# iow-esm/components.flux_calculator

Measured on AMD Instinct MI355X. Metric: exchange-grid Mcells/s per coupling step; achieved HBM GB/s vs MI355X peak, higher is better.
Workload: dtype f64

## Files before the change

### components.flux_calculator_amd/csrc/fcx_engine.hip

```cpp
#include <hip/hip_runtime.h>

#include <algorithm>
#include <atomic>
#include <cctype>
#include <chrono>
#include <condition_variable>
#include <cstdarg>
#include <cstdio>
#include <cstdlib>
#include <cstring>
#include <deque>
#include <map>
#include <memory>
#include <mutex>
#include <set>
#include <string>
#include <thread>
#include <vector>

#include <sched.h>
#include <unistd.h>

#include "fcx_copy_pool.h"
#include "fcx_internal.h"
// ... 108 lines not shown
    return std::max(1, std::min(cpus, 16));
  }();
  return n;
}

}

struct FieldUploader {
  std::thread th;
  std::mutex mu;
  std::condition_variable cv, idle;
  std::deque<int> q;
  int busy = 0;
  bool stop = false;
  bool prepared = false;
  bool dma = false;
  int err = 0;
  std::string msg;
};

struct fcx_engine {
  int device = 0;
  int T = 0;
  int64_t n[3] = {0, 0, 0};
  hipStream_t stream = nullptr;
  bool own_stream = false;
  int8_t method[FCX_NUM_FLUXES][kMaxTypes] = {};
  int slot[kMaxTypes + 1][3][kNumVars];
  bool allocated[kMaxTypes + 1][3][kNumVars] = {};
  uint8_t put_to[kMaxTypes + 1][3][kNumVars] = {};
  std::vector<Buffer> bufs;
  std::map<const double *, int> by_ptr;
  bool committed = false;
  bool any_regrid = false;
  bool aligned16 = true;
  bool f32 = false;
  size_t esize = 8;
  bool lcorr = false;
  int32_t init_date = 0;
  std::vector<double> corr_mm;
  void *corr_dev = nullptr;
  Csr rg[4];
  std::vector<std::pair<int, std::pair<int, int>>> averages;
  std::map<std::pair<uint32_t, int>, Plan> plans;
  void *pool = nullptr;
  hipEvent_t ev0 = nullptr, ev1 = nullptr;
  bool timed = false;
  bool gpu_ready = false;
  bool user_stream = false;
  LaunchConfig launch;
  bool specialize = true;
  struct AtmosField {
    int phase, s, g, var;
    double *out_host = nullptr, *out_dev = nullptr;
    bool external = false;
    StageRef st;
  };
  int64_t n_atmos = -1;
  std::vector<int32_t> atm_row, atm_col;
  std::vector<double> atm_w;
  bool atm_contiguous = true;
  int32_t *d_atm_row = nullptr, *d_atm_col = nullptr, *d_atm_idx = nullptr;
  void *d_atm_seg = nullptr;
  int32_t *d_atm_tile_a0 = nullptr;
  int64_t atm_seg_words = 0, atm_segments = 0;
  std::vector<int32_t> atm_idx;
  std::vector<int32_t> atm_empty;
  int32_t *d_atm_empty = nullptr;
  int32_t atm_maxseg = 0;
  double *d_atm_xrec = nullptr;
  int64_t atm_crossings = 0;
  bool atm_halo = true;
  double *d_atm_w = nullptr;
  std::vector<AtmosField> atm_fields;
  double *atm_shared = nullptr;
  int32_t atm_nb = 0, atm_stride = 0, atm_left = -1, atm_right = -1;
  bool own_shared = false;
  double *atm_shared_own = nullptr;
  struct fcx_comm *comm = nullptr;
  bool atm_done = false;
  bool exchanged = false;
  void *atm_pool = nullptr;
  int64_t atm_out_tpad = 0;
  bool atmos_in_run = true;
  bool atm_done_fused = false;
  int group_members = 0;
  std::unique_ptr<FieldUploader> uploader;
  std::vector<char> field_sent;
  struct RemapField {
    int phase, s, g, var;
    double *out_host = nullptr, *out_dev = nullptr;
    bool external = false;
    StageRef st;
  };
  struct Remap {
    int64_t n_dst = 0, n_links = 0;
    int32_t max_src = -1;
    std::vector<int32_t> row, col;
    std::vector<double> w;
    int32_t *d_row = nullptr, *d_col = nullptr;
    double *d_w = nullptr;
    std::vector<RemapField> fields;
    void *pool = nullptr;
    size_t pool_bytes = 0;
    double scatter = 0.0;
  };
  std::vector<Remap> remaps;
  int remap_pack = 2;
  void *d_rec = nullptr;
  size_t rec_bytes = 0;
  const Plan *rec_plan = nullptr;
  bool rec_written = false;
  int chunks = 8;
  int64_t min_chunk = 256 * 1024;
  int zero_copy = 2;
  bool zc_active = false;
  int64_t zc_bytes = 0;
  bool timing = false;
  hipStream_t s_in = nullptr, s_out = nullptr;
  std::vector<hipEvent_t> ev_in, ev_comp, ev_out;
  bool staging = true;
  bool deferred_scatter = false;
#ifdef FCX_AB_BUILD
  bool ab_fixup_each = false;
  bool ab_no_head = false;
#endif
  int host_threads = 0;
  std::vector<StagePool> spools;
  std::vector<Xfer> pending_out;
  hipEvent_t ev_stage_in = nullptr;
  bool stage_in_live = false;
  size_t pool_bytes = 0, tiled_bytes = 0, atm_pool_bytes = 0;
  bool tiled_opt = true;
  int64_t tpad = 0;
  std::vector<void *> tiled_pools;
  bool plan_dry = false;
  bool lib_spans = true;
  std::vector<Span> spans;
  std::vector<char> written;

  fcx_engine() {
    for (auto &a : slot)
      for (auto &b : a)
        for (auto &c : b) c = -1;
  }
  int buf(int s, int g, int var) const { return slot[s][g - 1][var0(var)]; }
  double *dptr(int s, int g, int var) const {
    int b = buf(s, g, var);
    return b < 0 ? nullptr : bufs[b].dev;
  }
};

static void stage_free(fcx_engine *e);


extern "C" const char *fcx_last_error(void) { return g_err.c_str(); }
extern "C" int fcx_version(void) { return FCX_VERSION; }

static std::atomic<fcx_abort_handler> g_abort{nullptr};

extern "C" int fcx_set_abort_handler(fcx_abort_handler handler) {
  g_abort.store(handler);
  return FCX_OK;
}

extern "C" int fcx_abort(const char *message) {
  fcx_abort_handler h = g_abort.load();
  if (!h) return fail(FCX_E_STATE, "no abort handler registered");
  h(message ? message : "");
  return FCX_OK;
}

extern "C" int fcx_method_from_string(const char *s, size_t len) {
  if (!s) return -1;
  size_t e = len;
  while (e > 0 && (s[e - 1] == ' ' || s[e - 1] == '\0')) --e;
  std::string m(s, e);
  static const char *names[] = {"none", "zero", "copy", "CCLM", "MOM5", "RCO", "water", "ice", "StBo"};
  for (int i = 0; i < 9; ++i)
    if (m == names[i]) return i;
  return -1;
}

static int64_t days_from_civil(int64_t y, int m, int d) {
  y -= m <= 2;
  const int64_t era = (y >= 0 ? y : y - 399) / 400;
  const int64_t yoe = y - era * 400;
  const int64_t doy = (153 * (m + (m > 2 ? -3 : 9)) + 2) / 5 + d - 1;
  const int64_t doe = yoe * 365 + yoe / 4 - yoe / 100 + doy;
  return era * 146097 + doe - 719468;
}

extern "C" int fcx_current_month(int32_t init_date, int64_t seconds, int32_t *month) {
  if (!month) return fail(FCX_E_ARG, "month is NULL");
  const int64_t y = init_date / 10000;
  const int m = (init_date / 100) % 100, d = init_date % 100;
  if (y < 1 || m < 1 || m > 12 || d < 1 || d > 31)
    return fail(FCX_E_ARG, "init_date %d is not YYYYMMDD", (int)init_date);
  int64_t q = seconds / 86400;
  if (seconds % 86400 != 0 && seconds < 0) q -= 1;
  const int64_t z = days_from_civil(y, m, d) + q + 719468;
  const int64_t era = (z >= 0 ? z : z - 146096) / 146097;
  const int64_t doe = z - era * 146097;
  const int64_t yoe = (doe - doe / 1460 + doe / 36524 - doe / 146096) / 365;
  const int64_t doy = doe - (365 * yoe + yoe / 4 - yoe / 100);
  const int64_t mp = (5 * doy + 2) / 153;
  *month = (int32_t)(mp < 10 ? mp + 3 : mp - 9);
  return FCX_OK;
}


extern "C" int fcx_create(int device, int num_surface_types, const int32_t grid_size[3],
                          fcx_engine **out) {
  if (!out || !grid_size) return fail(FCX_E_ARG, "NULL argument");
  *out = nullptr;
  if (num_surface_types < 1 || num_surface_types > kMaxTypes)
    return fail(FCX_E_ARG, "num_surface_types=%d outside 1..%d", num_surface_types, kMaxTypes);
  for (int g = 0; g < 3; ++g)
    if (grid_size[g] < 0) return fail(FCX_E_ARG, "grid_size(%d)=%d < 0", g + 1, grid_size[g]);
  auto *e = new fcx_engine();
  e->device = device;
  e->T = num_surface_types;
  for (int g = 0; g < 3; ++g) e->n[g] = grid_size[g];
  *out = e;
  return FCX_OK;
}

static void uploader_stop(fcx_engine *e);
static int uploader_join(fcx_engine *e);

extern "C" int fcx_destroy(fcx_engine *e) {
  if (!e) return FCX_OK;
  uploader_stop(e);
  if (!e->gpu_ready) {
    delete e;
    return FCX_OK;
  }
  (void)hipSetDevice(e->device);
  if (e->stream) (void)hipStreamSynchronize(e->stream);
  for (auto &kv : e->plans) {
    (void)hipFree(kv.second.dev);
    (void)hipFree(kv.second.host.rec);
  }
  for (auto &r : e->rg) {
    (void)hipFree(r.d_row);
    (void)hipFree(r.d_col);
    (void)hipFree(r.d_w);
  }
  (void)hipFree(e->corr_dev);
  (void)hipFree(e->d_atm_row);
  (void)hipFree(e->d_atm_seg);
  (void)hipFree(e->d_atm_tile_a0);
  (void)hipFree(e->d_atm_idx);
  (void)hipFree(e->d_atm_empty);
  (void)hipFree(e->d_atm_xrec);
  (void)hipFree(e->d_atm_col);
  (void)hipFree(e->d_atm_w);
  (void)hipFree(e->atm_pool);
  (void)hipFree(e->atm_shared_own);
  for (auto &r : e->remaps) {
    (void)hipFree(r.d_row);
    (void)hipFree(r.d_col);
    (void)hipFree(r.d_w);
    (void)hipFree(r.pool);
  }
  (void)hipFree(e->d_rec);
  (void)hipFree(e->pool);
  for (void *p : e->tiled_pools) (void)hipFree(p);
  for (auto &sp : e->spans) (void)hipFree(sp.dev);
  if (e->ev0) (void)hipEventDestroy(e->ev0);
  if (e->ev1) (void)hipEventDestroy(e->ev1);
  for (hipEvent_t ev : e->ev_in) (void)hipEventDestroy(ev);
  for (hipEvent_t ev : e->ev_comp) (void)hipEventDestroy(ev);
  for (hipEvent_t ev : e->ev_out) (void)hipEventDestroy(ev);
  stage_free(e);
  if (e->s_in) (void)hipStreamDestroy(e->s_in);
  if (e->s_out) (void)hipStreamDestroy(e->s_out);
  if (e->own_stream && e->stream) (void)hipStreamDestroy(e->stream);
  delete e;
  return FCX_OK;
}

extern "C" int fcx_set_stream(fcx_engine *e, void *stream) {
  if (!e) return fail(FCX_E_ARG, "NULL engine");
  if (e->committed)
    if (int r = uploader_join(e)) return r;
  if (e->own_stream && e->stream) {
    (void)hipStreamSynchronize(e->stream);
    (void)hipStreamDestroy(e->stream);
  }
  e->stream = reinterpret_cast<hipStream_t>(stream);
  e->own_stream = false;
  e->user_stream = true;
  return FCX_OK;
}

static int gpu_init(fcx_engine *e) {
  if (e->gpu_ready) return FCX_OK;
  HIP_TRY(hipSetDevice(e->device));
  if (!e->user_stream) {
    HIP_TRY(hipStreamCreateWithFlags(&e->stream, hipStreamNonBlocking));
    e->own_stream = true;
  }
  HIP_TRY(hipEventCreate(&e->ev0));
  HIP_TRY(hipEventCreate(&e->ev1));
  e->gpu_ready = true;
  return FCX_OK;
}

extern "C" int fcx_set_method(fcx_engine *e, int flux, int s, int method) {
  if (!e) return fail(FCX_E_ARG, "NULL engine");
  if (e->committed) return fail(FCX_E_STATE, "engine already committed");
  if (flux < 0 || flux >= FCX_NUM_FLUXES) return fail(FCX_E_ARG, "flux %d unknown", flux);
  if (s < 1 || s > e->T) return fail(FCX_E_ARG, "surface_type %d outside 1..%d", s, e->T);
  if (method < FCX_NONE || method > FCX_STBO) return fail(FCX_E_ARG, "method %d unknown", method);
  e->method[flux][s - 1] = (int8_t)method;
  return FCX_OK;
}

extern "C" int fcx_bind_field(fcx_engine *e, int s, int g, int var, double *ptr, int64_t n,
                              int flags) {
  if (!e) return fail(FCX_E_ARG, "NULL engine");
  if (e->committed) return fail(FCX_E_STATE, "engine already committed");
  if (s < 0 || s > kMaxTypes || g < 1 || g > 3 || var < 1 || var > kNumVars)
    return fail(FCX_E_ARG, "slot (%d,%d,%d) out of range", s, g, var);
  if (!ptr) {
    e->slot[s][g - 1][var0(var)] = -1;
    return FCX_OK;
  }
  if (n < e->n[g - 1])
    return fail(FCX_E_ARG, "%s(%d,%s): array of %lld cells shorter than grid_size %lld",
                kVarNames[var0(var)], s, g == 1 ? "t" : g == 2 ? "u" : "v", (long long)n,
                (long long)e->n[g - 1]);
  const bool on_dev = flags & FCX_MEM_DEVICE;
  auto it = e->by_ptr.find(ptr);
  int b;
  if (it == e->by_ptr.end()) {
    Buffer bf;
    bf.n = n;
    if (on_dev) {
      bf.dev = ptr;
// ... 172 lines not shown
}


static bool is_compute(int m) { return m == FCX_ZERO || m == FCX_CCLM || m == FCX_MOM5 || m == FCX_RCO; }

static bool merge_ok(const fcx_engine *e) {
  if (e->n[0] != e->n[1] || e->n[0] != e->n[2]) return false;
  for (int s = 1; s <= e->T; ++s) {
    if (e->method[FCX_SPEC_VAPOR_SURFACE_U][s - 1] != e->method[FCX_SPEC_VAPOR_SURFACE_T][s - 1] ||
        e->method[FCX_SPEC_VAPOR_SURFACE_V][s - 1] != e->method[FCX_SPEC_VAPOR_SURFACE_T][s - 1])
      return false;
    for (int v : {FCX_TSUR, FCX_FICE, FCX_PSUR, FCX_UATM, FCX_VATM, FCX_QSUR})
      for (int g = 2; g <= 3; ++g)
        if (e->buf(s, g, v) >= 0 && e->buf(s, g, v) != e->buf(s, 1, v)) return false;
    for (int v : {FCX_AMOM, FCX_CMOM})
      if (e->buf(s, 3, v) != e->buf(s, 2, v)) return false;
  }
  return true;
}

static void plan_fused_atmos(fcx_engine *e, Plan &pl, uint32_t stages, int phase) {
  pl.atm_fused = false;
  const bool maps = (!compact_map(e->f32, true) || e->d_atm_seg) && (!compact_map(e->f32, false) || e->d_atm_seg) &&
                    (compact_map(e->f32, true) || e->d_atm_idx) && (compact_map(e->f32, false) || e->d_atm_idx);
  if (!pl.variant || !maps || e->atm_maxseg > kTile / 2 || e->any_regrid || phase <= 0 ||
      phase >= 1000 || !e->specialize || (e->f32 && e->T >= 2))
    return;
  const TypeParams &tp = pl.host.type[0];
  AtmosFused af{};
  int nf = 0;
  const bool multi = e->T >= 2;
  if (multi && !pl.host.ravg_on) return;
  for (size_t fi = 0; fi < e->atm_fields.size(); ++fi) {
    const auto &f = e->atm_fields[fi];
    if (!(f.phase & phase)) continue;
    const int b = e->buf(f.s, f.g, f.var);
    int k = -1;
    if (multi) {
      for (int slot = 0; slot < kFusedFields; ++slot)
        if (f.s == 0 && pl.host.ravg.out[slot] && b >= 0 && e->bufs[b].dev == pl.host.ravg.out[slot]) k = slot;
      if (k < 0 || af.out[k]) return;
      af.out[k] = f.out_dev;
      af.x[k] = e->bufs[b].dev;
      af.scol[k] = (int32_t)fi;
      ++nf;
      continue;
    }
    if (f.s == 1 && f.var == FCX_MEVA && (stages & S_MEVA) && b == e->buf(1, 1, FCX_MEVA)) k = 0;
    if (f.s == 1 && f.var == FCX_HLAT && (stages & S_HLAT) && b == e->buf(1, 1, FCX_HLAT) &&
        (tp.m_hlat == FCX_WATER || tp.m_hlat == FCX_ICE || tp.m_hlat == FCX_ZERO))
      k = 1;
    if (f.s == 1 && f.var == FCX_HSEN && (stages & S_HSEN) && b == e->buf(1, 1, FCX_HSEN)) k = 2;
    if (f.s == 1 && f.var == FCX_RBBR && (stages & S_RBBR) && b == e->buf(1, 1, FCX_RBBR) &&
        (tp.m_rbbr == FCX_STBO || tp.m_rbbr == FCX_ZERO))
      k = 3;
    if (f.s == 1 && f.var == FCX_UMOM && (stages & S_UMOM) && b == e->buf(1, 2, FCX_UMOM)) k = 4;
    if (f.s == 1 && f.var == FCX_VMOM && (stages & S_VMOM) && b == e->buf(1, 3, FCX_VMOM)) k = 5;
    if (k < 0 || af.out[k]) return;
    af.out[k] = f.out_dev;
    af.x[k] = e->bufs[b].dev;
    af.scol[k] = (int32_t)fi;
    ++nf;
  }
  if (nf == 0) return;
  if (e->d_atm_seg) {
    af.seg_bits = reinterpret_cast<const uint32_t *>(e->d_atm_seg);
    af.seg_pre = reinterpret_cast<const int32_t *>(af.seg_bits + e->atm_seg_words);
    af.seg_atm = af.seg_pre + e->atm_seg_words + 1;
  }
  af.tile_a0 = e->d_atm_tile_a0;
  af.idx = e->d_atm_idx;
  af.w = e->d_atm_w;
  af.xrec = e->d_atm_xrec;
  af.xrec_on = e->atm_crossings > 0;
#ifdef FCX_AB_BUILD
  if (e->ab_no_head) af.xrec_on = 0;
#endif
  af.n_atmos = e->n_atmos;
  af.shared = e->atm_shared;
  af.stride = e->atm_stride;
  af.left = e->atm_left;
  af.right = e->atm_right;
  af.tpad = e->tpad;
  af.out_tpad = e->atm_out_tpad;
  pl.af = af;
  pl.atm_nf = nf;
  pl.atm_phase = phase;
  pl.atm_fused = true;
}

static bool remap_packs(const fcx_engine *e, const fcx_engine::Remap &rm, int nf);
static int rec_width(const fcx_engine *e, int nf);

static int plan_fused_records(fcx_engine *e, Plan &pl, uint32_t stages, int phase) {
  pl.rec_remap = pl.rec_group = -1;
  Params &P = pl.host;
  for (int k = 0; k < 6; ++k) P.rec_pos[k] = -1;
#ifndef FCX_FUSE_RECORDS
#define FCX_FUSE_RECORDS 1
#endif
  if (!FCX_FUSE_RECORDS || !pl.variant || e->T != 1 || e->f32 || !e->specialize || e->any_regrid || phase <= 0 || phase >= 1000 ||
      e->remap_pack == 0 || e->launch.cells_per_thread != 2 || !e->aligned16 || !P.merged_uv || P.n_max <= 0)
    return FCX_OK;
  const TypeParams &tp = P.type[0];
  auto slot_of = [&](const fcx_engine::RemapField &f) -> int {
    const int b = e->buf(f.s, f.g, f.var);
    if (f.s != 1 || b < 0) return -1;
    if (f.var == FCX_MEVA && (stages & S_MEVA) && b == e->buf(1, 1, FCX_MEVA) && is_compute(tp.m_meva)) return 0;
    if (f.var == FCX_HLAT && (stages & S_HLAT) && b == e->buf(1, 1, FCX_HLAT) && tp.t.hlat &&
        (tp.m_hlat == FCX_WATER || tp.m_hlat == FCX_ICE || tp.m_hlat == FCX_ZERO))
      return 1;
    if (f.var == FCX_HSEN && (stages & S_HSEN) && b == e->buf(1, 1, FCX_HSEN) && tp.t.hsen && is_compute(tp.m_hsen))
      return 2;
    if (f.var == FCX_RBBR && (stages & S_RBBR) && b == e->buf(1, 1, FCX_RBBR) && tp.t.rbbr &&
        (tp.m_rbbr == FCX_STBO || tp.m_rbbr == FCX_ZERO))
      return 3;
    if (f.var == FCX_UMOM && (stages & S_UMOM) && b == e->buf(1, 2, FCX_UMOM) && tp.uv[0].mom && is_compute(tp.m_mom))
      return 4;
    if (f.var == FCX_VMOM && (stages & S_VMOM) && b == e->buf(1, 3, FCX_VMOM) && tp.uv[1].mom && is_compute(tp.m_mom))
      return 5;
    return -1;
  };
  for (size_t ri = 0; ri < e->remaps.size(); ++ri) {
    const auto &rm = e->remaps[ri];
    std::vector<const fcx_engine::RemapField *> grp;
    int gi = 0;
    auto try_group = [&]() -> bool {
      const int nf = (int)grp.size();
      if (!remap_packs(e, rm, nf) || nf > 6) return false;
      int8_t pos[6] = {-1, -1, -1, -1, -1, -1};
      for (int i = 0; i < nf; ++i) {
        const int k = slot_of(*grp[(size_t)i]);
        if (k < 0 || pos[k] >= 0) return false;
        pos[k] = (int8_t)i;
      }
      const int p = rec_width(e, nf);
      HIP_TRY(hipMalloc(&P.rec, (size_t)P.n_max * p * sizeof(double)));
      P.rec_p = p;
      for (int k = 0; k < 6; ++k) P.rec_pos[k] = pos[k];
      pl.rec_remap = (int)ri;
      pl.rec_group = gi;
      return true;
    };
    for (auto &f : rm.fields) {
      if (!(f.phase & phase)) continue;
      grp.push_back(&f);
      if ((int)grp.size() == kMaxAtmosFields) {
        if (try_group()) return FCX_OK;
        grp.clear();
        ++gi;
      }
    }
    if (!grp.empty() && try_group()) return FCX_OK;
  }
  return FCX_OK;
}

static int ravg_slot(const fcx_engine *e, const Params &P, uint32_t stages, int g, int var) {
  if (e->T < 2) return -1;
  int slot = -1;
  if (g == 1 && var == FCX_MEVA) slot = A_MEVA;
  if (g == 1 && var == FCX_HLAT) slot = A_HLAT;
  if (g == 1 && var == FCX_HSEN) slot = A_HSEN;
  if (g == 1 && var == FCX_RBBR) slot = A_RBBR;
  if (g == 1 && var == FCX_TSUR) slot = A_TSUR;
  if (P.merged_uv && g == 2 && var == FCX_UMOM) slot = A_UMOM;
  if (P.merged_uv && g == 3 && var == FCX_VMOM) slot = A_VMOM;
// ... 710 lines not shown
      at[b] = {cold_pool, fill[kCold]++};
    }
  }
  for (int k = 0; k < npools; ++k) {
    void *p = nullptr;
    hipError_t err = hipMalloc(&p, bytes);
    if (err != hipSuccess)
      return fail(FCX_E_NOMEM, "hipMalloc(%zu) for the tiled field mirrors: %s", bytes, hipGetErrorString(err));
    e->tiled_pools.push_back(p);
  }
  for (size_t b = 0; b < e->bufs.size(); ++b)
    e->bufs[b].dev = reinterpret_cast<double *>((char *)e->tiled_pools[at[b].first] +
                                                (size_t)at[b].second * kLayoutTile * e->esize);
  e->tpad = (S - 1) * kLayoutTile;
  return FCX_OK;
}

constexpr hipMemcpyKind kH2D = hipMemcpyDefault, kD2H = hipMemcpyDefault;

static hipError_t copy_cells(const fcx_engine *e, const Buffer &bf, int64_t a, int64_t z, bool h2d,
                             hipStream_t s) {
  const size_t es = e->esize;
  auto one = [&](int64_t lo, int64_t hi) {
    if (hi <= lo) return hipSuccess;
    char *dev = reinterpret_cast<char *>(bf.dev) + (size_t)tiled(lo, e->tpad) * es;
    char *host = reinterpret_cast<char *>(bf.host) + (size_t)lo * es;
    const size_t bytes = (size_t)(hi - lo) * es;
    return h2d ? hipMemcpyAsync(dev, host, bytes, kH2D, s) : hipMemcpyAsync(host, dev, bytes, kD2H, s);
  };
  if (z <= a) return hipSuccess;
  if (e->tpad == 0) return one(a, z);
  const int64_t t0 = (a + kLayoutTile - 1) / kLayoutTile, t1 = z / kLayoutTile;
  if (t1 <= t0) {
    const int64_t m = std::min(z, t0 * kLayoutTile);
    hipError_t r = one(a, m);
    return (r != hipSuccess || m >= z) ? r : one(m, z);
  }
  if (a < t0 * kLayoutTile)
    if (hipError_t r = one(a, t0 * kLayoutTile)) return r;
  const size_t row = (size_t)kLayoutTile * es, pitch = (size_t)(kLayoutTile + e->tpad) * es;
  char *dev = reinterpret_cast<char *>(bf.dev) + (size_t)t0 * pitch;
  char *host = reinterpret_cast<char *>(bf.host) + (size_t)t0 * row;
  hipError_t r = h2d ? hipMemcpy2DAsync(dev, pitch, host, row, row, (size_t)(t1 - t0), kH2D, s)
                     : hipMemcpy2DAsync(host, row, dev, pitch, row, (size_t)(t1 - t0), kD2H, s);
  if (r != hipSuccess || z == t1 * kLayoutTile) return r;
  return one(t1 * kLayoutTile, z);
}

static hipError_t zero_cells(const fcx_engine *e, double *dev, int64_t n, hipStream_t s) {
  if (n <= 0) return hipSuccess;
  if (e->tpad == 0) return hipMemsetAsync(dev, 0, (size_t)n * e->esize, s);
  const size_t row = (size_t)kLayoutTile * e->esize, pitch = (size_t)(kLayoutTile + e->tpad) * e->esize;
  const int64_t full = n / kLayoutTile;
  if (full)
    if (hipError_t r = hipMemset2DAsync(dev, pitch, 0, row, (size_t)full, s)) return r;
  if (n > full * kLayoutTile)
    return hipMemsetAsync(reinterpret_cast<char *>(dev) + full * pitch, 0, (size_t)(n - full * kLayoutTile) * e->esize, s);
  return hipSuccess;
}


static StageRef stage_ref(fcx_engine *e, const void *d) {
  StageRef r;
  const char *p = reinterpret_cast<const char *>(d);
  for (size_t i = 0; i < e->spools.size(); ++i) {
    const StagePool &q = e->spools[i];
    if (p >= q.dev && p < q.dev + q.bytes) {
      r.sp = (int)i;
      r.soff = (size_t)(p - q.dev);
      return r;
    }
  }
  return r;
}

static void stage_setup(fcx_engine *e) {
  if (!e->staging) return;
  const size_t es = e->esize;
  std::vector<StagePool> cand;
  for (void *p : e->tiled_pools)
    cand.push_back(StagePool{(char *)p, nullptr, e->tiled_bytes, true, (size_t)kLayoutTile * es,
                             (size_t)(kLayoutTile + e->tpad) * es});
  if (e->pool) cand.push_back(StagePool{(char *)e->pool, nullptr, e->pool_bytes, false, 0, 0});
  if (e->atm_pool) {
    const bool t = e->atm_out_tpad != 0;
    cand.push_back(StagePool{(char *)e->atm_pool, nullptr, e->atm_pool_bytes, t, t ? (size_t)kLayoutTile * es : 0,
                             t ? (size_t)(kLayoutTile + e->atm_out_tpad) * es : 0});
  }
  for (auto &rm : e->remaps)
    if (rm.pool) cand.push_back(StagePool{(char *)rm.pool, nullptr, rm.pool_bytes, false, 0, 0});
  auto heap = [&](const void *host, int64_t n) { return host && !lib_block_device_ptr(host, (size_t)std::max<int64_t>(n, 1) * es); };
  std::vector<char> used(cand.size(), 0);
  auto mark = [&](const void *dev) {
    for (size_t i = 0; i < cand.size(); ++i)
      if ((const char *)dev >= cand[i].dev && (const char *)dev < cand[i].dev + cand[i].bytes) used[i] = 1;
  };
  for (auto &bf : e->bufs)
    if (!bf.external && heap(bf.host, bf.n)) mark(bf.dev);
  for (auto &f : e->atm_fields)
    if (!f.external && heap(f.out_host, e->n_atmos)) mark(f.out_dev);
  for (auto &rm : e->remaps)
    for (auto &f : rm.fields)
      if (!f.external && heap(f.out_host, rm.n_dst)) mark(f.out_dev);
  for (size_t i = 0; i < cand.size(); ++i)
    if (used[i]) e->spools.push_back(cand[i]);
  for (auto &bf : e->bufs)
    if (!bf.external && heap(bf.host, bf.n)) bf.st = stage_ref(e, bf.dev);
  for (auto &f : e->atm_fields)
    if (!f.external && heap(f.out_host, e->n_atmos)) f.st = stage_ref(e, f.out_dev);
  for (auto &rm : e->remaps)
    for (auto &f : rm.fields)
      if (!f.external && heap(f.out_host, rm.n_dst)) f.st = stage_ref(e, f.out_dev);
}

static void stage_disable(fcx_engine *e, size_t i) {
  StagePool &p = e->spools[i];
  p.host = nullptr;
  p.disabled = true;
  auto drop = [&](StageRef &st) {
    if (st.sp == (int)i) st.sp = -1;
  };
  for (auto &bf : e->bufs) drop(bf.st);
  for (auto &f : e->atm_fields) drop(f.st);
  for (auto &rm : e->remaps)
    for (auto &f : rm.fields) drop(f.st);
}

static int pin_fail_mode() {
  const char *v = std::getenv("FCX_TEST_PIN_FAIL");
  return v && (*v == '1' || *v == '2') ? *v - '0' : 0;
}

static bool stage_pin(fcx_engine *e, size_t i, bool lazy) {
  StagePool &p = e->spools[i];
  if (p.host) return true;
  if (p.disabled) return false;
  const int inject = pin_fail_mode();
  if (!(inject == 1 || (inject == 2 && lazy)) &&
      hipHostMalloc((void **)&p.host, std::max<size_t>(p.bytes, 1), kHostPinFlags) == hipSuccess)
    return true;
  (void)hipGetLastError();
  stage_disable(e, i);
  return false;
}

static void stage_alloc_all(fcx_engine *e, const std::vector<char> &eager) {
  const bool fail_all = pin_fail_mode() == 1;
  for (size_t i = 0; i < e->spools.size(); ++i) {
    if (e->spools[i].host) continue;
    if (i < eager.size() && !eager[i] && !fail_all) continue;
    (void)stage_pin(e, i, false);
  }
}

static void stage_prepare_bufs(fcx_engine *e, const std::vector<int> &ids) {
  for (int b : ids) {
    const int sp = e->bufs[(size_t)b].st.sp;
    if (sp >= 0) (void)stage_pin(e, (size_t)sp, true);
  }
}
static void stage_prepare_outputs(fcx_engine *e) {
  for (auto &f : e->atm_fields)
    if (f.st.sp >= 0) (void)stage_pin(e, (size_t)f.st.sp, true);
  for (auto &rm : e->remaps)
    for (auto &f : rm.fields)
      if (f.st.sp >= 0) (void)stage_pin(e, (size_t)f.st.sp, true);
}

static int stage_alloc(fcx_engine *e, const std::vector<Xfer> &xs) {
  for (const Xfer &x : xs) {
    StagePool &p = e->spools[(size_t)x.sp];
    if (!p.host) return fail(FCX_E_STATE, "staging pool %d has no host image", x.sp);
  }
  return FCX_OK;
}

static void stage_free(fcx_engine *e) {
  for (auto &p : e->spools)
    if (p.host) (void)hipHostFree(p.host);
  e->spools.clear();
  if (e->ev_stage_in) (void)hipEventDestroy(e->ev_stage_in);
  e->ev_stage_in = nullptr;
}

static void stage_copy(fcx_engine *e, const std::vector<Xfer> &xs, int64_t a, int64_t z, bool gather) {
  constexpr size_t kPiece = size_t(64) << 10;
  const size_t es = e->esize;
  std::vector<CopyJob> jobs;
  auto add = [&](char *img, char *host, size_t bytes) {
    for (size_t o = 0; o < bytes; o += kPiece) {
      const size_t b = std::min(kPiece, bytes - o);
      jobs.push_back(gather ? CopyJob{img + o, host + o, b} : CopyJob{host + o, img + o, b});
// ... 265 lines not shown
  for (auto &c : e->rg) {
    if (!c.set) continue;
    HIP_TRY(hipMalloc(&c.d_row, c.row_ptr.size() * sizeof(int32_t)));
    HIP_TRY(hipMalloc(&c.d_col, std::max<size_t>(c.col.size(), 1) * sizeof(int32_t)));
    HIP_TRY(hipMalloc(&c.d_w, std::max<size_t>(c.w.size(), 1) * sizeof(double)));
    HIP_TRY(hipMemcpy(c.d_row, c.row_ptr.data(), c.row_ptr.size() * sizeof(int32_t), hipMemcpyHostToDevice));
    if (!c.col.empty()) {
      HIP_TRY(hipMemcpy(c.d_col, c.col.data(), c.col.size() * sizeof(int32_t), hipMemcpyHostToDevice));
      if (e->f32) {
        std::vector<float> wf(c.w.begin(), c.w.end());
        HIP_TRY(hipMemcpy(c.d_w, wf.data(), wf.size() * sizeof(float), hipMemcpyHostToDevice));
      } else {
        HIP_TRY(hipMemcpy(c.d_w, c.w.data(), c.w.size() * sizeof(double), hipMemcpyHostToDevice));
      }
    }
  }
  if (e->n_atmos >= 0) {
    HIP_TRY(hipMalloc(&e->d_atm_row, e->atm_row.size() * sizeof(int32_t)));
    HIP_TRY(hipMemcpy(e->d_atm_row, e->atm_row.data(), e->atm_row.size() * sizeof(int32_t),
                      hipMemcpyHostToDevice));
    HIP_TRY(hipMalloc(&e->d_atm_w, std::max<size_t>(e->atm_w.size(), 1) * sizeof(double)));
    if (!e->atm_w.empty())
      HIP_TRY(hipMemcpy(e->d_atm_w, e->atm_w.data(), e->atm_w.size() * sizeof(double), hipMemcpyHostToDevice));
    if (e->atm_contiguous && !e->atm_idx.empty() && !(compact_map(e->f32, true) && compact_map(e->f32, false))) {
      HIP_TRY(hipMalloc(&e->d_atm_idx, e->atm_idx.size() * sizeof(int32_t)));
      HIP_TRY(hipMemcpy(e->d_atm_idx, e->atm_idx.data(), e->atm_idx.size() * sizeof(int32_t),
                        hipMemcpyHostToDevice));
    }
    if (e->atm_contiguous && !e->atm_idx.empty() && (compact_map(e->f32, true) || compact_map(e->f32, false))) {
      const int64_t nx = (int64_t)e->atm_idx.size(), nw = (nx + 31) / 32;
      std::vector<uint32_t> seg((size_t)(2 * nw + 1), 0u);
      std::vector<int32_t> atm;
      for (int64_t x = 0; x < nx; ++x)
        if (x == 0 || e->atm_idx[(size_t)x] != e->atm_idx[(size_t)x - 1]) {
          seg[(size_t)(x >> 5)] |= 1u << (x & 31);
          atm.push_back(e->atm_idx[(size_t)x]);
        }
      int32_t run = 0;
      for (int64_t w = 0; w <= nw; ++w) {
        seg[(size_t)(nw + w)] = (uint32_t)run;
        if (w < nw) run += __builtin_popcount(seg[(size_t)w]);
      }
      e->atm_seg_words = nw;
      e->atm_segments = (int64_t)atm.size();
      const size_t head = seg.size() * sizeof(uint32_t);
      HIP_TRY(hipMalloc(&e->d_atm_seg, head + std::max<size_t>(atm.size(), 1) * sizeof(int32_t)));
      HIP_TRY(hipMemcpy(e->d_atm_seg, seg.data(), head, hipMemcpyHostToDevice));
      if (!atm.empty())
        HIP_TRY(hipMemcpy((char *)e->d_atm_seg + head, atm.data(), atm.size() * sizeof(int32_t), hipMemcpyHostToDevice));
      if (compact_map(e->f32, false)) {
        const int64_t tc = (int64_t)(e->f32 ? kF32Cpl : 2) * 64, nt = (nx + tc - 1) / tc;
        std::vector<int32_t> a0((size_t)nt);
        for (int64_t t = 0; t < nt; ++t) a0[(size_t)t] = e->atm_idx[(size_t)(t * tc)];
        HIP_TRY(hipMalloc(&e->d_atm_tile_a0, (size_t)std::max<int64_t>(nt, 1) * sizeof(int32_t)));
        if (nt) HIP_TRY(hipMemcpy(e->d_atm_tile_a0, a0.data(), a0.size() * sizeof(int32_t), hipMemcpyHostToDevice));
      }
    }
    if (e->atm_contiguous && !e->atm_idx.empty()) {
      const int64_t tiles = (e->n[0] + kTile - 1) / kTile;
      HIP_TRY(hipMalloc(&e->d_atm_xrec, (size_t)std::max<int64_t>(tiles, 1) * kXRec * sizeof(double)));
      e->atm_crossings = 0;
      for (size_t b = kTile; b < e->atm_idx.size(); b += kTile) e->atm_crossings += e->atm_idx[b - 1] == e->atm_idx[b];
      if (!e->atm_empty.empty()) {
        HIP_TRY(hipMalloc(&e->d_atm_empty, e->atm_empty.size() * sizeof(int32_t)));
        HIP_TRY(hipMemcpy(e->d_atm_empty, e->atm_empty.data(), e->atm_empty.size() * sizeof(int32_t),
                          hipMemcpyHostToDevice));
      }
    }
    if (!e->atm_contiguous) {
      HIP_TRY(hipMalloc(&e->d_atm_col, std::max<size_t>(e->atm_col.size(), 1) * sizeof(int32_t)));
      if (!e->atm_col.empty())
        HIP_TRY(hipMemcpy(e->d_atm_col, e->atm_col.data(), e->atm_col.size() * sizeof(int32_t),
                          hipMemcpyHostToDevice));
    }
    size_t need = 0;
    bool atm_ext = false;
    for (auto &f : e->atm_fields) {
      atm_ext = atm_ext || f.external;
      if (!f.external) need += ((size_t)std::max<int64_t>(e->n_atmos, 1) * e->esize + 255) / 256 * 256;
    }
    const int64_t nfa = (int64_t)e->atm_fields.size();
    if (FCX_TILED_ATM && e->tpad && !atm_ext && nfa >= 2 && e->n_atmos > 0) {
      const int64_t tiles = (e->n_atmos + kLayoutTile - 1) / kLayoutTile;
      e->atm_pool_bytes = (size_t)tiles * nfa * kLayoutTile * e->esize;
      HIP_TRY(hipMalloc(&e->atm_pool, e->atm_pool_bytes));
      for (int64_t k = 0; k < nfa; ++k)
        e->atm_fields[k].out_dev = reinterpret_cast<double *>((char *)e->atm_pool + (size_t)k * kLayoutTile * e->esize);
      e->atm_out_tpad = (nfa - 1) * kLayoutTile;
      need = 0;
    }
    if (need) {
      e->atm_pool_bytes = need;
      HIP_TRY(hipMalloc(&e->atm_pool, need));
      size_t off = 0;
      for (auto &f : e->atm_fields)
        if (!f.external) {
          f.out_dev = reinterpret_cast<double *>((char *)e->atm_pool + off);
          off += ((size_t)std::max<int64_t>(e->n_atmos, 1) * e->esize + 255) / 256 * 256;
        }
    }
  }
  if (e->own_shared && e->n_atmos >= 0) {
    const size_t stride = std::max<size_t>(e->atm_fields.size(), 1);
    const size_t cnt = std::max<size_t>((size_t)e->atm_nb * stride, 1);
    HIP_TRY(hipMalloc(&e->atm_shared_own, cnt * sizeof(double)));
    HIP_TRY(hipMemset(e->atm_shared_own, 0, cnt * sizeof(double)));
    if (e->atm_left >= 0 && e->atm_right >= 0 && e->n_atmos < 2 && e->atm_left != e->atm_right)
      return fail(FCX_E_ARG, "the one atmosphere cell is shared on both sides: it needs one boundary slot for all "
                             "its ranks (left == right), not %d and %d", e->atm_left, e->atm_right);
    e->atm_shared = e->atm_nb > 0 ? e->atm_shared_own : nullptr;
    e->atm_stride = (int32_t)stride;
  }
  for (auto &rm : e->remaps) {
    for (auto &f : rm.fields)
      if (rm.max_src >= e->n[f.g - 1])
        return fail(FCX_E_ARG, "remap link source %d outside the %lld cells of grid %d", rm.max_src,
                    (long long)e->n[f.g - 1], f.g);
    HIP_TRY(hipMalloc(&rm.d_row, rm.row.size() * sizeof(int32_t)));
    HIP_TRY(hipMemcpy(rm.d_row, rm.row.data(), rm.row.size() * sizeof(int32_t), hipMemcpyHostToDevice));
    HIP_TRY(hipMalloc(&rm.d_col, std::max<size_t>(rm.col.size(), 1) * sizeof(int32_t)));
    HIP_TRY(hipMalloc(&rm.d_w, std::max<size_t>(rm.w.size(), 1) * sizeof(double)));
    if (!rm.col.empty()) {
      HIP_TRY(hipMemcpy(rm.d_col, rm.col.data(), rm.col.size() * sizeof(int32_t), hipMemcpyHostToDevice));
      HIP_TRY(hipMemcpy(rm.d_w, rm.w.data(), rm.w.size() * sizeof(double), hipMemcpyHostToDevice));
    }
    const size_t one = ((size_t)std::max<int64_t>(rm.n_dst, 1) * e->esize + 255) / 256 * 256;
    size_t need = 0;
    for (auto &f : rm.fields) need += f.external ? 0 : one;
    if (need) {
      rm.pool_bytes = need;
      HIP_TRY(hipMalloc(&rm.pool, need));
      size_t off = 0;
      for (auto &f : rm.fields)
        if (!f.external) {
          f.out_dev = reinterpret_cast<double *>((char *)rm.pool + off);
          off += one;
        }
    }
    size_t nf_max = 0;
    for (int ph = 1; ph <= 3; ++ph) {
      size_t c = 0;
      for (auto &f : rm.fields) c += (f.phase & ph) ? 1 : 0;
      nf_max = std::max(nf_max, std::min<size_t>(c, kMaxAtmosFields));
    }
    rm.scatter = remap_scatter(rm);
    if (remap_packs(e, rm, (int)nf_max))
      e->rec_bytes = std::max(e->rec_bytes, (size_t)(rm.max_src + 1) * rec_width(e, (int)nf_max) * e->esize);
  }
  if (e->rec_bytes) HIP_TRY(hipMalloc(&e->d_rec, e->rec_bytes));
  stage_setup(e);
  e->committed = true;
  std::vector<char> eager(e->spools.size(), e->any_regrid ? 1 : 0);
  if (!e->any_regrid) {
    Plan *pl = nullptr;
    if (get_plan(e, phase_stages(FCX_PHASE_ALL), FCX_PHASE_ALL, &pl) == FCX_OK && pl) {
      for (const std::vector<int> *ids : {&pl->reads, &pl->writes})
        for (int b : *ids)
          if (e->bufs[(size_t)b].st.sp >= 0) eager[(size_t)e->bufs[(size_t)b].st.sp] = 1;
    } else {
      std::fill(eager.begin(), eager.end(), 1);
    }
    for (auto &f : e->atm_fields)
      if (f.st.sp >= 0) eager[(size_t)f.st.sp] = 1;
    for (auto &rm : e->remaps)
      for (auto &f : rm.fields)
        if (f.st.sp >= 0) eager[(size_t)f.st.sp] = 1;
  }
  stage_alloc_all(e, eager);
  return FCX_OK;
}


// ... 40 lines not shown
    direct = true;
  }
  if (!spanned.empty()) {
    if (int r = span_copy(e, spanned, h2d, e->stream)) return r;
    direct = true;
  }
  if (h2d) return stage_in(e, xs, e->stream);
  if (xs.empty() && direct && !e->deferred_scatter) {
    HIP_TRY(hipStreamSynchronize(e->stream));
    return stage_flush(e);
  }
  return stage_out(e, xs, e->stream);
}

#ifndef FCX_ZC_ONE_CELL
#define FCX_ZC_ONE_CELL 1
#endif

static int full_range_halo(const fcx_engine *e, const Plan *pl) {
  const int cpl = e->f32 ? kF32Cpl : 2;
  const int h = (e->atm_maxseg - 1 + cpl - 1) / cpl;
  if (e->atm_halo && e->atm_crossings > 0 &&
      (pl->host.num_types == 1 || (FCX_HALO_RAVG && pl->host.ravg_on)) && h >= 1 && h <= (cpl == 4 ? 2 : 4))
    return h;
  return 0;
}

static LaunchConfig plan_launch(fcx_engine *e, Plan *pl, int64_t lo, int64_t hi, bool *fused) {
  LaunchConfig lc = e->launch;
  lc.lo = lo;
  lc.hi = hi;
  if (e->zc_active) lc.nontemporal = false;
  if (!e->aligned16) lc.cells_per_thread = 1;
  if (FCX_ZC_ONE_CELL && e->zc_active && !pl->atm_fused && pl->host.rec == nullptr) lc.cells_per_thread = 1;
  lc.merged = pl->host.merged_uv != 0;
  lc.variant = (e->specialize && lc.merged) ? pl->variant : 0;
  lc.f32 = e->f32;
  lc.ravg = pl->host.ravg_on != 0;
  lc.rec = pl->host.rec != nullptr && lc.variant && lc.cells_per_thread == 2 && !lc.f32;
  *fused = pl->atm_fused && lc.variant && lc.cells_per_thread == 2;
  if (*fused) {
    pl->af.shared = e->atm_shared;
    pl->af.stride = e->atm_stride;
    pl->af.left = e->atm_left;
    pl->af.right = e->atm_right;
    lc.halo = lo == 0 && (hi < 0 || hi >= pl->host.n_max) ? full_range_halo(e, pl) : 0;
    pl->af.halo = lc.halo;
  }
  return lc;
}

static int launch_empty_cells(fcx_engine *e, Plan *pl, const LaunchConfig &lc) {
  if (e->atm_empty.empty()) return FCX_OK;
  const int r = launch_atmos_zero(pl->af, e->d_atm_empty, (int64_t)e->atm_empty.size(), lc.f32, e->stream);
  if (r) return fail(FCX_E_HIP, "atmos_zero launch: %s", hipGetErrorString((hipError_t)r));
  return FCX_OK;
}

static int launch_fixup(fcx_engine *e, Plan *pl, const LaunchConfig &lc) {
  if (int r = launch_empty_cells(e, pl, lc)) return r;
  if (e->atm_crossings <= 0 || lc.halo) return FCX_OK;
  const int r = launch_atmos_fixup(pl->af, pl->host.n_max, lc.f32, e->stream);
  if (r) return fail(FCX_E_HIP, "atmos_fixup launch: %s", hipGetErrorString((hipError_t)r));
  return FCX_OK;
}

static int launch_plan(fcx_engine *e, Plan *pl, const double *corr_m, int64_t lo = 0, int64_t hi = -1,
                       bool fixup = true) {
  if (pl->host.n_max <= 0) return FCX_OK;
  bool fused = false;
  const LaunchConfig lc = plan_launch(e, pl, lo, hi, &fused);
  e->rec_written = lc.rec;
  const int r = launch_cells(&pl->host, pl->dev, corr_m, lc, e->stream, fused ? &pl->af : nullptr);
  if (r) return fail(FCX_E_HIP, "cells_kernel launch: %s", hipGetErrorString((hipError_t)r));
  if (fused && fixup)
    if (int r2 = launch_fixup(e, pl, lc)) return r2;
  if (fused) e->atm_done_fused = true;
  return FCX_OK;
}

static int regrid_var(fcx_engine *e, int var, int surface_type);
static int comm_exchange(fcx_engine *e);
static hipError_t get_atm(const fcx_engine *e, double *host, const double *dev, hipStream_t s);
static int run_remaps(fcx_engine *e, int phase);
static int download_remaps(fcx_engine *e, int phase, hipStream_t s, std::vector<Xfer> *xs);

static int staged_sequence(int phase, std::vector<std::pair<uint32_t, int>> &seq) {
  if (phase & FCX_PHASE_EARLY) seq.push_back({S_RBBR, FCX_RBBR});
  if (phase & FCX_PHASE_NORMAL) {
    seq.push_back({S_QSUR_T | S_QSUR_U | S_QSUR_V, FCX_QSUR});
    seq.push_back({S_MEVA, FCX_MEVA});
    seq.push_back({S_HLAT, FCX_HLAT});
    seq.push_back({S_HSEN, FCX_HSEN});
    seq.push_back({S_UMOM, FCX_UMOM});
    seq.push_back({S_VMOM, FCX_VMOM});
    seq.push_back({S_RSDR, 0});
  }
  return FCX_OK;
}

static uint32_t phase_stages(int phase) {
  uint32_t st = S_AVG;
  if (phase & FCX_PHASE_EARLY) st |= kEarly;
  if (phase & FCX_PHASE_NORMAL) st |= kNormal;
  return st;
}


static int upload_one(fcx_engine *e, int b) {
  FieldUploader &u = *e->uploader;
  const Buffer &bf = e->bufs[(size_t)b];
  if (bf.n == 0) return FCX_OK;
  if (bf.st.sp >= 0) (void)stage_pin(e, (size_t)bf.st.sp, true);
  if (bf.st.sp >= 0) {
    if (!u.prepared) {
      bool mapped = false;
      for (const StagePool &p : e->spools) mapped = mapped || p.mapped;
      if (!e->pending_out.empty() || mapped) {
        HIP_TRY(hipStreamSynchronize(e->stream));
        if (int r = stage_flush(e)) return r;
      }
      if (e->stage_in_live) HIP_TRY(hipEventSynchronize(e->ev_stage_in));
      u.prepared = true;
    }
    const std::vector<Xfer> xs{xfer_of(bf.st, bf.host, bf.n)};
    if (int r = stage_alloc(e, xs)) return r;
    stage_copy(e, xs, 0, -1, true);
    if (!e->spools[(size_t)bf.st.sp].mapped) {
      HIP_TRY(stage_dma(e, xs, 0, -1, true, e->stream));
      u.dma = true;
    }
  } else if (!bf.external || bf.span >= 0) {
    HIP_TRY(copy_cells(e, bf, 0, bf.n, true, e->stream));
  }
  return FCX_OK;
}

static void uploader_loop(fcx_engine *e) {
  FieldUploader &u = *e->uploader;
  (void)hipSetDevice(e->device);
  std::unique_lock<std::mutex> lk(u.mu);
  for (;;) {
    u.cv.wait(lk, [&] { return u.stop || !u.q.empty(); });
    if (u.q.empty()) return;
    const int b = u.q.front();
    u.q.pop_front();
    u.busy = 1;
    lk.unlock();
    const int r = upload_one(e, b);
    lk.lock();
    if (r && !u.err) {
      u.err = r;
      u.msg = g_err;
    }
    u.busy = 0;
    if (u.q.empty()) u.idle.notify_all();
  }
}

static int uploader_join(fcx_engine *e) {
  if (!e->uploader) return FCX_OK;
  FieldUploader &u = *e->uploader;
  std::unique_lock<std::mutex> lk(u.mu);
  u.idle.wait(lk, [&] { return u.q.empty() && u.busy == 0; });
  if (u.dma) {
    u.dma = false;
    if (!e->ev_stage_in) HIP_TRY(hipEventCreateWithFlags(&e->ev_stage_in, hipEventDisableTiming));
    HIP_TRY(hipEventRecord(e->ev_stage_in, e->stream));
    e->stage_in_live = true;
  }
  if (u.err) {
    const int r = u.err;
    u.err = 0;
    std::fill(e->field_sent.begin(), e->field_sent.end(), 0);
    u.prepared = false;
    return fail(r, "fcx_upload_field: %s", u.msg.c_str());
  }
  return FCX_OK;
}

static void uploader_stop(fcx_engine *e) {
  if (!e->uploader) return;
  {
    std::lock_guard<std::mutex> lk(e->uploader->mu);
    e->uploader->stop = true;
  }
  e->uploader->cv.notify_all();
  if (e->uploader->th.joinable()) e->uploader->th.join();
  e->uploader.reset();
}

static void fields_taken(fcx_engine *e) {
  std::fill(e->field_sent.begin(), e->field_sent.end(), 0);
  if (e->uploader) e->uploader->prepared = false;
}

extern "C" int fcx_upload_field(fcx_engine *e, int s, int g, int var) {
  if (!e) return fail(FCX_E_ARG, "NULL engine");
  if (!e->committed) return fail(FCX_E_STATE, "fcx_commit has not been called");
  if (s < 0 || s > kMaxTypes || g < 1 || g > 3 || var < 1 || var > kNumVars)
    return fail(FCX_E_ARG, "field (%d, %d, %d) outside the data model", s, g, var);
  const int b = e->buf(s, g, var);
  if (b < 0) return fail(FCX_E_ARG, "local_field(%d,%d)%%var(%s) is not bound", s, g, kVarNames[var - 1]);
  if (e->field_sent.size() != e->bufs.size()) e->field_sent.assign(e->bufs.size(), 0);
  if (e->field_sent[(size_t)b]) return FCX_OK;
  e->field_sent[(size_t)b] = 1;
  if (!e->uploader) {
    e->uploader.reset(new FieldUploader());
    e->uploader->th = std::thread(uploader_loop, e);
  }
  {
    std::lock_guard<std::mutex> lk(e->uploader->mu);
    e->uploader->q.push_back(b);
  }
  e->uploader->cv.notify_one();
  return FCX_OK;
}

extern "C" int fcx_upload(fcx_engine *e, int phase) {
  if (int r = check(e)) return r;
  if (phase < 1 || phase > 3) return fail(FCX_E_ARG, "phase %d unknown", phase);
  Plan *pl;
  if (int r = get_plan(e, phase_stages(phase), phase, &pl)) return r;
  return copy_bufs(e, pl->reads, true);
}

extern "C" int fcx_download(fcx_engine *e, int phase) {
  if (int r = check(e)) return r;
  if (phase < 1 || phase > 3) return fail(FCX_E_ARG, "phase %d unknown", phase);
  Plan *pl;
  if (int r = get_plan(e, phase_stages(phase), phase, &pl)) return r;
  stage_prepare_outputs(e);
  std::vector<Xfer> xs;
  std::vector<int> ids = pl->writes;
  for (auto &f : e->atm_fields)
    if ((f.phase & phase) && e->n_atmos > 0) {
      if (f.st.sp >= 0)
        xs.push_back(xfer_of(f.st, f.out_host, e->n_atmos));
      else if (!f.external)
        HIP_TRY(get_atm(e, f.out_host, f.out_dev, e->stream));
    }
  if (int r = download_remaps(e, phase, e->stream, &xs)) return r;
  if (e->any_regrid) {
    std::vector<int> extra;
    std::vector<int> vars;
    if (phase & FCX_PHASE_EARLY) vars = {FCX_RBBR};
    if (phase & FCX_PHASE_NORMAL)
      for (int v : {FCX_QSUR, FCX_MEVA, FCX_HLAT, FCX_HSEN, FCX_UMOM, FCX_VMOM}) vars.push_back(v);
    for (int s = 1; s <= e->T; ++s)
      for (int g = 1; g <= 3; ++g)
        for (int v : vars)
          if (e->put_to[s][g - 1][v - 1])
            for (int k = 0; k < 3; ++k)
              if ((e->put_to[s][g - 1][v - 1] >> k) & 1)
                if (e->buf(s, k + 1, v) >= 0) extra.push_back(e->buf(s, k + 1, v));
    ids.insert(ids.end(), extra.begin(), extra.end());
  }
  std::sort(ids.begin(), ids.end());
  ids.erase(std::unique(ids.begin(), ids.end()), ids.end());
  return copy_bufs(e, ids, false, &xs);
}

static hipError_t get_atm(const fcx_engine *e, double *host, const double *dev, hipStream_t s) {
  const size_t es = e->esize, n = (size_t)e->n_atmos;
  if (!e->atm_out_tpad) return hipMemcpyAsync(host, dev, n * es, kD2H, s);
  const size_t row = (size_t)kLayoutTile * es, pitch = (size_t)(kLayoutTile + e->atm_out_tpad) * es;
  const size_t full = n / kLayoutTile;
  if (full)
    if (hipError_t r = hipMemcpy2DAsync(host, row, dev, pitch, row, full, kD2H, s)) return r;
  if (n > full * kLayoutTile)
    return hipMemcpyAsync((char *)host + full * row, (const char *)dev + full * pitch, (n - full * kLayoutTile) * es,
                          kD2H, s);
  return hipSuccess;
}

static AtmosArgs atmos_args(fcx_engine *e, int phase) {
  AtmosArgs a{};
  a.f32 = e->f32 ? 1 : 0;
  a.row_ptr = e->d_atm_row;
  a.col = e->atm_contiguous ? nullptr : e->d_atm_col;
  a.w = e->d_atm_w;
  a.n_atmos = e->n_atmos;
  a.stride = e->atm_stride;
  a.left = e->atm_left;
  a.right = e->atm_right;
  a.shared = e->atm_shared;
  a.tpad = e->tpad;
  a.out_tpad = e->atm_out_tpad;
  a.vec = a.col == nullptr && e->aligned16;
  for (size_t i = 0; i < e->atm_fields.size(); ++i) {
    const auto &f = e->atm_fields[i];
    if (!(f.phase & phase) || a.nf >= kMaxAtmosFields) continue;
    a.x[a.nf] = e->dptr(f.s, f.g, f.var);
    a.out[a.nf] = f.out_dev;
    a.scol[a.nf] = (int32_t)i;
    ++a.nf;
  }
  return a;
}

static int run_atmos(fcx_engine *e, int phase) {
  if (e->n_atmos < 0 || e->atm_fields.empty()) return FCX_OK;
  const AtmosArgs a = atmos_args(e, phase);
  if (a.nf == 0) return FCX_OK;
  const int r = launch_atmos(a, e->stream);
  if (r) return fail(FCX_E_HIP, "atmos_kernel launch: %s", hipGetErrorString((hipError_t)r));
  return FCX_OK;
}

static int run_remaps(fcx_engine *e, int phase) {
  for (size_t ri = 0; ri < e->remaps.size(); ++ri) {
    auto &rm = e->remaps[ri];
    int gi = 0;
    AtmosArgs a{};
    a.f32 = e->f32 ? 1 : 0;
    a.row_ptr = rm.d_row;
    a.col = rm.d_col;
    a.w = rm.d_w;
    a.n_atmos = rm.n_dst;
    a.left = a.right = -1;
    a.tpad = e->tpad;
    auto flush = [&]() -> int {
      if (!a.nf) return FCX_OK;
      a.rec = nullptr;
      a.rec_p = 0;
      const Plan *rp = e->rec_plan;
      if (rp && rp->rec_remap == (int)ri && rp->rec_group == gi) {
        a.rec = rp->host.rec;
        a.rec_p = rp->host.rec_p;
      } else if (e->d_rec && remap_packs(e, rm, a.nf)) {
        a.rec_p = rec_width(e, a.nf);
        const int r = launch_pack_records(a, (int64_t)rm.max_src + 1, e->aligned16, !e->zc_active && e->launch.nontemporal,
                                          e->d_rec, e->stream);
        if (r) return fail(FCX_E_HIP, "remap pack launch: %s", hipGetErrorString((hipError_t)r));
        a.rec = e->d_rec;
      }
      const int r = launch_atmos(a, e->stream);
      if (r) return fail(FCX_E_HIP, "remap launch: %s", hipGetErrorString((hipError_t)r));
      a.nf = 0;
      ++gi;
      return FCX_OK;
    };
    for (auto &f : rm.fields) {
      if (!(f.phase & phase)) continue;
      a.x[a.nf] = e->dptr(f.s, f.g, f.var);
      a.out[a.nf] = f.out_dev;
      if (!a.x[a.nf]) return fail(FCX_E_MISSING, "remap field %s(%d) is not bound", kVarNames[var0(f.var)], f.s);
      if (++a.nf == kMaxAtmosFields)
        if (int r = flush()) return r;
    }
    if (int r = flush()) return r;
  }
  return FCX_OK;
}

static int download_remaps(fcx_engine *e, int phase, hipStream_t s, std::vector<Xfer> *xs) {
  for (auto &rm : e->remaps)
    for (auto &f : rm.fields)
      if ((f.phase & phase) && rm.n_dst > 0) {
        if (f.st.sp >= 0)
          xs->push_back(xfer_of(f.st, f.out_host, rm.n_dst));
        else if (!f.external)
          HIP_TRY(hipMemcpyAsync(f.out_host, f.out_dev, rm.n_dst * e->esize, kD2H, s));
      }
  return FCX_OK;
}

static int run_tail(fcx_engine *e, int phase) {
  if (e->atmos_in_run && !e->atm_done_fused)
    if (int r = run_atmos(e, phase)) return r;
  e->atm_done = e->atmos_in_run || e->atm_done_fused;
  if (e->atm_done)
    if (int r = comm_exchange(e)) return r;
  if (int r = run_remaps(e, phase)) return r;
  if (e->timing) HIP_TRY(hipEventRecord(e->ev1, e->stream));
  e->timed = e->timing;
  return FCX_OK;
}

extern "C" int fcx_run(fcx_engine *e, int phase, int32_t t) {
  if (int r = check(e)) return r;
  if (phase < 1 || phase > 3) return fail(FCX_E_ARG, "phase %d unknown", phase);
  int rc;
  const double *corr_m = month_slice(e, t, &rc);
  if (rc) return rc;
  if (e->timing) HIP_TRY(hipEventRecord(e->ev0, e->stream));
  e->atm_done_fused = false;
  e->atm_done = e->exchanged = false;
  e->rec_plan = nullptr;
  e->group_members = 0;
  fields_taken(e);
  if (!e->any_regrid) {
    Plan *pl;
    if (int r = get_plan(e, phase_stages(phase), phase, &pl)) return r;
    if (int r = launch_plan(e, pl, corr_m)) return r;
    e->rec_plan = e->rec_written ? pl : nullptr;
  } else {
    std::vector<std::pair<uint32_t, int>> seq;
    staged_sequence(phase, seq);
    for (auto &st : seq) {
      Plan *pl;
      if (int r = get_plan(e, st.first, 0, &pl)) return r;
      if (int r = launch_plan(e, pl, corr_m)) return r;
      if (st.second)
// ... 145 lines not shown
    HIP_TRY(hipEventCreateWithFlags(&b, hipEventDisableTiming));
    HIP_TRY(hipEventCreateWithFlags(&c, hipEventDisableTiming));
    e->ev_in.push_back(a);
    e->ev_comp.push_back(b);
    e->ev_out.push_back(c);
  }
  stage_prepare_bufs(e, pl->reads);
  stage_prepare_bufs(e, pl->writes);
  stage_prepare_outputs(e);
  std::vector<Xfer> xin, xout;
  std::vector<int> din, dout;
  for (int b : pl->reads) {
    const Buffer &bf = e->bufs[b];
    if (bf.n == 0) continue;
    if (bf.st.sp >= 0) xin.push_back(xfer_of(bf.st, bf.host, bf.n));
    else if (!bf.external || bf.span >= 0) din.push_back(b);
  }
  for (int b : pl->writes) {
    const Buffer &bf = e->bufs[b];
    if (bf.n == 0) continue;
    if (bf.st.sp >= 0) xout.push_back(xfer_of(bf.st, bf.host, bf.n));
    else if (!bf.external || bf.span >= 0) dout.push_back(b);
  }
  if (!xin.empty() || !xout.empty()) {
    if (int r = stage_alloc(e, xin)) return r;
    if (int r = stage_alloc(e, xout)) return r;
    bool mapped = false;
    for (const Xfer &x : xin) mapped = mapped || e->spools[(size_t)x.sp].mapped;
    if (!e->pending_out.empty() || mapped) {
      HIP_TRY(hipStreamSynchronize(e->stream));
      if (int r = stage_flush(e)) return r;
    }
    if (e->stage_in_live) HIP_TRY(hipEventSynchronize(e->ev_stage_in));
  }
  auto range = [&](int k, int64_t *lo, int64_t *hi) {
    *lo = k * per;
    *hi = k == K - 1 ? -1 : std::min(n, *lo + per);
  };
  int scattered = 0;
  auto scatter_upto = [&](int k_end) -> int {
    for (; scattered < k_end; ++scattered) {
      int64_t lo, hi;
      range(scattered, &lo, &hi);
      HIP_TRY(hipEventSynchronize(e->ev_out[scattered]));
      stage_copy(e, xout, lo, hi, false);
    }
    return FCX_OK;
  };
  if (e->timing) HIP_TRY(hipEventRecord(e->ev0, e->s_in));
  e->atm_done_fused = false;
  e->atm_done = e->exchanged = false;
  e->rec_plan = pl;
  for (int k = 0; k < K; ++k) {
    const int64_t lo = k * per, hi = std::min(n, lo + per);
    const bool last = k == K - 1;
    if (!xin.empty()) {
      stage_copy(e, xin, lo, last ? -1 : hi, true);
      HIP_TRY(stage_dma(e, xin, lo, last ? -1 : hi, true, e->s_in));
    }
    for (int b : din)
      if (int r = copy_slice(e, e->bufs[b], lo, hi, last, true, e->s_in)) return r;
    HIP_TRY(hipEventRecord(e->ev_in[k], e->s_in));
    HIP_TRY(hipStreamWaitEvent(e->stream, e->ev_in[k], 0));
    if (int r = launch_plan(e, pl, corr_m, lo, hi, last)) return r;
    if (!e->rec_written) e->rec_plan = nullptr;
    HIP_TRY(hipEventRecord(e->ev_comp[k], e->stream));
    HIP_TRY(hipStreamWaitEvent(e->s_out, e->ev_comp[k], 0));
    if (!xout.empty()) HIP_TRY(stage_dma(e, xout, lo, last ? -1 : hi, false, e->s_out));
    for (int b : dout)
      if (int r = copy_slice(e, e->bufs[b], lo, hi, last, false, e->s_out)) return r;
    HIP_TRY(hipEventRecord(e->ev_out[k], e->s_out));
    if (!xout.empty() && k >= 2)
      if (int r = scatter_upto(k - 1)) return r;
  }
  if (e->atmos_in_run && !e->atm_done_fused)
    if (int r = run_atmos(e, phase)) return r;
  e->atm_done = e->atmos_in_run || e->atm_done_fused;
  if (e->atm_done)
    if (int r = comm_exchange(e)) return r;
  if (int r = run_remaps(e, phase)) return r;
  HIP_TRY(hipEventRecord(e->ev_comp[K - 1], e->stream));
  HIP_TRY(hipStreamWaitEvent(e->s_out, e->ev_comp[K - 1], 0));
  std::vector<Xfer> xa;
  if (e->atmos_in_run || e->atm_done_fused)
    for (auto &f : e->atm_fields)
      if ((f.phase & phase) && e->n_atmos > 0) {
        if (f.st.sp >= 0)
          xa.push_back(xfer_of(f.st, f.out_host, e->n_atmos));
        else if (!f.external)
          HIP_TRY(get_atm(e, f.out_host, f.out_dev, e->s_out));
      }
  if (int r = download_remaps(e, phase, e->s_out, &xa)) return r;
  if (!xa.empty()) {
    if (int r = stage_alloc(e, xa)) return r;
    HIP_TRY(stage_dma(e, xa, 0, -1, false, e->s_out));
  }
  if (e->timing) HIP_TRY(hipEventRecord(e->ev1, e->s_out));
  e->timed = e->timing;
  if (!xout.empty())
    if (int r = scatter_upto(K)) return r;
  HIP_TRY(hipStreamSynchronize(e->s_out));
  HIP_TRY(hipStreamSynchronize(e->stream));
  if (!xa.empty()) stage_copy(e, xa, 0, -1, false);
  return FCX_OK;
}

static bool host_bound(const fcx_engine *e, const Plan *pl) {
  for (int b : pl->reads)
    if (!e->bufs[b].external || e->bufs[b].st.sp >= 0 || e->bufs[b].span >= 0) return true;
  for (int b : pl->writes)
    if (!e->bufs[b].external || e->bufs[b].st.sp >= 0 || e->bufs[b].span >= 0) return true;
  return false;
}

extern "C" int fcx_step(fcx_engine *e, int phase, int32_t t) {
  if (int r = check(e)) return r;
  if (phase < 1 || phase > 3) return fail(FCX_E_ARG, "phase %d unknown", phase);
  const bool handed = std::find(e->field_sent.begin(), e->field_sent.end(), 1) != e->field_sent.end();
  if (e->chunks > 1 && !e->any_regrid && !handed) {
    Plan *pl;
    if (int r = get_plan(e, phase_stages(phase), phase, &pl)) return r;
    if (host_bound(e, pl) && pl->host.n_max >= 2 * e->min_chunk) return step_pipelined(e, phase, t, pl);
  }
  if (int r = fcx_upload(e, phase)) return r;
  if (int r = fcx_run(e, phase, t)) return r;
  if (int r = fcx_download(e, phase)) return r;
  return fcx_synchronize(e);
}

extern "C" int fcx_step_async(fcx_engine *e, int phase, int32_t t) {
  if (int r = check(e)) return r;
  if (phase < 1 || phase > 3) return fail(FCX_E_ARG, "phase %d unknown", phase);
  const bool handed = std::find(e->field_sent.begin(), e->field_sent.end(), 1) != e->field_sent.end();
  if (e->chunks > 1 && !e->any_regrid && !handed) {
    Plan *pl;
    if (int r = get_plan(e, phase_stages(phase), phase, &pl)) return r;
    if (host_bound(e, pl) && pl->host.n_max >= 2 * e->min_chunk) return step_pipelined(e, phase, t, pl);
  }
  if (int r = fcx_upload(e, phase)) return r;
  if (int r = fcx_run(e, phase, t)) return r;
  const bool keep = e->deferred_scatter;
  e->deferred_scatter = true;
  const int r = fcx_download(e, phase);
  e->deferred_scatter = keep;
  return r;
}

extern "C" int fcx_synchronize(fcx_engine *e) {
  if (!e) return fail(FCX_E_ARG, "NULL engine");
  if (e->committed)
    if (int r = uploader_join(e)) return r;
  HIP_TRY(hipStreamSynchronize(e->stream));
  return stage_flush(e);
}

static int per_call(fcx_engine *e, uint32_t stages, int avg_phases, int32_t t) {
  if (int r = check(e)) return r;
  Plan *pl;
  if (int r = get_plan(e, stages, avg_phases, &pl)) return r;
  int rc;
  const double *corr_m = (stages & S_MEVA) ? month_slice(e, t, &rc) : nullptr;
  if ((stages & S_MEVA) && rc) return rc;
  if (int r = copy_bufs(e, pl->reads, true)) return r;
  fields_taken(e);
  if (e->timing) HIP_TRY(hipEventRecord(e->ev0, e->stream));
  if (int r = launch_plan(e, pl, corr_m)) return r;
  if (e->timing) HIP_TRY(hipEventRecord(e->ev1, e->stream));
  e->timed = e->timing;
  if (int r = copy_bufs(e, pl->writes, false)) return r;
  return fcx_synchronize(e);
}

extern "C" int fcx_calc_spec_vapor_surface(fcx_engine *e, int g) {
  if (g < 1 || g > 3) return fail(FCX_E_ARG, "which_grid %d", g);
// ... 184 lines not shown
                                      : hipMemcpyDefault;
  if (kind < 1 || kind > 3) return fail(FCX_E_ARG, "memcpy kind %d", kind);
  HIP_TRY(hipMemcpy(dst, src, bytes, k));
  return FCX_OK;
}


static int drop_plans(fcx_engine *e) {
  if (e->plans.empty()) return FCX_OK;
  if (e->stream) HIP_TRY(hipStreamSynchronize(e->stream));
  for (auto &kv : e->plans) {
    (void)hipFree(kv.second.dev);
    (void)hipFree(kv.second.host.rec);
  }
  e->plans.clear();
  e->rec_plan = nullptr;
  return FCX_OK;
}

extern "C" int fcx_set_option(fcx_engine *e, int option, int64_t value) {
  if (!e) return fail(FCX_E_ARG, "NULL engine");
  switch (option) {
    case FCX_OPT_CELLS_PER_THREAD:
      if (value != 1 && value != 2) return fail(FCX_E_ARG, "cells per thread must be 1 or 2");
      if (e->launch.cells_per_thread != (int)value)
        if (int r = drop_plans(e)) return r;
      e->launch.cells_per_thread = (int)value;
      return FCX_OK;
    case FCX_OPT_MAX_BLOCKS:
      if (value < -1 || value > (1 << 30)) return fail(FCX_E_ARG, "max blocks %lld", (long long)value);
      e->launch.max_blocks = (int)value;
      return FCX_OK;
    case FCX_OPT_NONTEMPORAL:
      e->launch.nontemporal = value != 0;
      return FCX_OK;
    case FCX_OPT_SPECIALIZE:
      if (e->specialize != (value != 0))
        if (int r = drop_plans(e)) return r;
      e->specialize = value != 0;
      return FCX_OK;
    case FCX_OPT_ATMOS_IN_RUN:
      e->atmos_in_run = value != 0;
      return FCX_OK;
    case FCX_OPT_TIMING:
      e->timing = value != 0;
      if (!e->timing) e->timed = false;
      return FCX_OK;
    case FCX_OPT_LIB_SPANS:
      if (e->committed) return fail(FCX_E_STATE, "lib_spans is applied at fcx_commit");
      if (value < 0 || value > 1) return fail(FCX_E_ARG, "lib_spans: 0 or 1");
      e->lib_spans = value != 0;
      return FCX_OK;
    case FCX_OPT_ZERO_COPY:
      if (e->committed) return fail(FCX_E_STATE, "zero_copy is applied at fcx_commit");
      if (value < 0 || value > 2) return fail(FCX_E_ARG, "zero_copy: 0 off, 1 on, 2 auto");
      e->zero_copy = (int)value;
      return FCX_OK;
    case FCX_OPT_PIPELINE_MIN_CHUNK:
      if (value < kChunkAlign || value % kChunkAlign)
        return fail(FCX_E_ARG, "pipeline min chunk %lld: a positive multiple of %lld cells", (long long)value,
                    (long long)kChunkAlign);
      e->min_chunk = value;
      return FCX_OK;
    case FCX_OPT_PIPELINE_CHUNKS:
      if (value < 1 || value > 1024) return fail(FCX_E_ARG, "pipeline chunks %lld outside 1..1024", (long long)value);
      e->chunks = (int)value;
      return FCX_OK;
    case FCX_OPT_ATMOS_HALO:
      e->atm_halo = value != 0;
      return FCX_OK;
    case FCX_OPT_HOST_STAGING:
      if (e->committed) return fail(FCX_E_STATE, "host_staging is applied at fcx_commit");
      e->staging = value != 0;
      return FCX_OK;
    case FCX_OPT_HOST_THREADS:
      if (value < 0 || value > 64) return fail(FCX_E_ARG, "host threads %lld outside 0..64", (long long)value);
      e->host_threads = (int)value;
      return FCX_OK;
    case FCX_OPT_REMAP_PACK:
      if (e->committed) return fail(FCX_E_STATE, "remap_pack is applied at fcx_commit");
      if (value < 0 || value > 2) return fail(FCX_E_ARG, "remap_pack: 0 never, 1 always, 2 auto");
      e->remap_pack = (int)value;
      return FCX_OK;
    case FCX_OPT_TILED_LAYOUT:
      if (e->committed) return fail(FCX_E_STATE, "tiled_layout is applied at fcx_commit");
      e->tiled_opt = value != 0;
      return FCX_OK;
    case FCX_OPT_DEFERRED_SCATTER:
      e->deferred_scatter = value != 0;
      return FCX_OK;
    case FCX_OPT_RETIRED_PIN_HOST:
    case FCX_OPT_RETIRED_12:
    case FCX_OPT_RETIRED_CARRY_HANDOFF:
      return FCX_OK;
#ifdef FCX_AB_BUILD
    case 98:
      e->ab_no_head = value != 0;
      for (auto &kv : e->plans) kv.second.af.xrec_on = !e->ab_no_head && e->atm_crossings > 0;
      return FCX_OK;
    case 99:
      e->ab_fixup_each = value != 0;
      return FCX_OK;
#endif
    default:
      return fail(FCX_E_ARG, "option %d unknown", option);
  }
}


extern "C" int fcx_set_atmos_map(fcx_engine *e, int64_t n_atmos, const int32_t *idx, const double *w) {
  if (!e) return fail(FCX_E_ARG, "NULL engine");
  if (e->committed) return fail(FCX_E_STATE, "engine already committed");
  const int64_t n = e->n[0];
  if (n_atmos < 0 || (n > 0 && (!idx || !w))) return fail(FCX_E_ARG, "bad atmosphere map");
  std::vector<int32_t> count((size_t)n_atmos + 1, 0);
  bool sorted = true;
  for (int64_t x = 0; x < n; ++x) {
    if (idx[x] < 0 || idx[x] >= n_atmos)
      return fail(FCX_E_ARG, "atmosphere index %d of exchange cell %lld outside 0..%lld", idx[x],
                  (long long)x, (long long)n_atmos - 1);
    if (x > 0 && idx[x] < idx[x - 1]) sorted = false;
    count[(size_t)idx[x] + 1]++;
  }
  e->n_atmos = n_atmos;
  e->atm_idx.assign(idx, idx + n);
  e->atm_maxseg = 0;
  e->atm_empty.clear();
  for (int64_t a = 0; a < n_atmos; ++a) {
    e->atm_maxseg = std::max(e->atm_maxseg, count[(size_t)a + 1]);
    if (count[(size_t)a + 1] == 0) e->atm_empty.push_back((int32_t)a);
  }
  e->atm_row.assign((size_t)n_atmos + 1, 0);
  for (int64_t a = 0; a < n_atmos; ++a) e->atm_row[(size_t)a + 1] = e->atm_row[(size_t)a] + count[(size_t)a + 1];
  e->atm_contiguous = sorted;
  e->atm_w.assign((size_t)n, 0.0);
  e->atm_col.clear();
  if (sorted) {
    for (int64_t x = 0; x < n; ++x) e->atm_w[(size_t)x] = w[x];
  } else {
    e->atm_col.assign((size_t)n, 0);
    std::vector<int32_t> fill(e->atm_row.begin(), e->atm_row.end() - 1);
    for (int64_t x = 0; x < n; ++x) {
      const int32_t at = fill[(size_t)idx[x]]++;
      e->atm_col[(size_t)at] = (int32_t)x;
      e->atm_w[(size_t)at] = w[x];
    }
  }
  return FCX_OK;
}

extern "C" int fcx_add_atmos_field(fcx_engine *e, int phase, int s, int g, int var, double *out, int flags) {
  if (!e) return fail(FCX_E_ARG, "NULL engine");
  if (e->committed) return fail(FCX_E_STATE, "engine already committed");
  if (e->n_atmos < 0) return fail(FCX_E_STATE, "fcx_set_atmos_map first");
  if (phase < 1 || phase > 3 || s < 0 || s > kMaxTypes || g < 1 || g > 3 || var < 1 || var > kNumVars || !out)
    return fail(FCX_E_ARG, "bad atmosphere field arguments");
  if (e->n[g - 1] != e->n[0]) return fail(FCX_E_UNSUPPORTED, "atmosphere fields must live on the t grid cells");
  if ((int)e->atm_fields.size() >= kMaxAtmosFields)
    return fail(FCX_E_UNSUPPORTED, "more than %d atmosphere fields", kMaxAtmosFields);
  fcx_engine::AtmosField f;
  f.phase = phase;
  f.s = s;
  f.g = g;
  f.var = var;
  if (flags & FCX_MEM_DEVICE) {
    f.out_dev = out;
    f.external = true;
  } else {
    f.out_host = out;
  }
  e->atm_fields.push_back(f);
  return FCX_OK;
}

extern "C" int fcx_set_atmos_shared(fcx_engine *e, double *shared, int32_t nb, int32_t stride, int32_t left,
                                    int32_t right) {
  if (!e) return fail(FCX_E_ARG, "NULL engine");
  if (nb < 0 || stride < 0 || left >= nb || right >= nb || (nb > 0 && !shared))
    return fail(FCX_E_ARG, "bad shared boundary buffer");
  if ((left >= 0 || right >= 0) && stride < (int32_t)e->atm_fields.size())
    return fail(FCX_E_ARG, "stride %d < %zu atmosphere fields", stride, e->atm_fields.size());
  if (left >= 0 && right >= 0 && e->n_atmos == 1 && left != right)
    return fail(FCX_E_ARG, "the one atmosphere cell is shared on both sides: it needs one boundary slot for all "
                           "its ranks (left == right), not %d and %d", left, right);
  if (e->own_shared) return fail(FCX_E_STATE, "boundary slots already owned by the engine (fcx_set_atmos_boundaries)");
  e->atm_shared = shared;
  e->atm_nb = nb;
  e->atm_stride = stride;
  e->atm_left = left;
  e->atm_right = right;
  return FCX_OK;
}

extern "C" int fcx_atmos_finish(fcx_engine *e) {
  if (int r = check(e)) return r;
  if (!e->atm_shared) return FCX_OK;
  if (e->n_atmos <= 0) {
    if (e->atm_nb > 0 && e->atm_stride > 0)
      HIP_TRY(hipMemsetAsync(e->atm_shared, 0, (size_t)e->atm_nb * e->atm_stride * sizeof(double), e->stream));
    return FCX_OK;
  }
  const AtmosArgs a = atmos_args(e, FCX_PHASE_ALL);
  const int r = launch_atmos_finish(a, e->atm_nb, e->stream);
  if (r) return fail(FCX_E_HIP, "atmos_finish launch: %s", hipGetErrorString((hipError_t)r));
  return FCX_OK;
}

extern "C" int fcx_run_atmos(fcx_engine *e, int phase) {
  if (int r = check(e)) return r;
  if (phase < 1 || phase > 3) return fail(FCX_E_ARG, "phase %d unknown", phase);
  if (!e->atm_done) {
    if (int r = run_atmos(e, phase)) return r;
    e->atm_done = true;
  }
  return comm_exchange(e);
}

extern "C" int fcx_last_group_size(fcx_engine *e, int32_t *members) {
  if (!e || !members) return fail(FCX_E_ARG, "NULL argument");
  *members = e->group_members;
  return FCX_OK;
}


extern "C" int fcx_add_remap(fcx_engine *e, int64_t n_dst, int64_t n_links, const int32_t *src,
                             const int32_t *dst, const double *w, int32_t *remap_id) {
  if (!e || !remap_id) return fail(FCX_E_ARG, "NULL argument");
  if (e->committed) return fail(FCX_E_STATE, "engine already committed");
  if (n_dst < 0 || n_links < 0 || (n_links > 0 && (!src || !dst || !w))) return fail(FCX_E_ARG, "bad remap");
  fcx_engine::Remap rm;
  rm.n_dst = n_dst;
  rm.n_links = n_links;
  rm.row.assign((size_t)n_dst + 1, 0);
  for (int64_t k = 0; k < n_links; ++k) {
    if (dst[k] < 0 || dst[k] >= n_dst || src[k] < 0)
      return fail(FCX_E_ARG, "remap link %lld (%d -> %d) outside the grids", (long long)k, src[k], dst[k]);
    rm.row[(size_t)dst[k] + 1]++;
    rm.max_src = std::max(rm.max_src, src[k]);
  }
  for (int64_t d = 0; d < n_dst; ++d) rm.row[(size_t)d + 1] += rm.row[(size_t)d];
  rm.col.assign((size_t)n_links, 0);
  rm.w.assign((size_t)n_links, 0.0);
  std::vector<int32_t> fill(rm.row.begin(), rm.row.end() - 1);
  for (int64_t k = 0; k < n_links; ++k) {
    const int32_t at = fill[(size_t)dst[k]]++;
    rm.col[(size_t)at] = src[k];
    rm.w[(size_t)at] = w[k];
  }
  *remap_id = (int32_t)e->remaps.size();
  e->remaps.push_back(std::move(rm));
  return FCX_OK;
}

extern "C" int fcx_add_remap_field(fcx_engine *e, int32_t remap_id, int phase, int s, int g, int var, double *out,
                                   int flags) {
  if (!e) return fail(FCX_E_ARG, "NULL engine");
  if (e->committed) return fail(FCX_E_STATE, "engine already committed");
  if (remap_id < 0 || remap_id >= (int32_t)e->remaps.size()) return fail(FCX_E_ARG, "remap %d unknown", remap_id);
  if (phase < 1 || phase > 3 || s < 0 || s > kMaxTypes || g < 1 || g > 3 || var < 1 || var > kNumVars || !out)
    return fail(FCX_E_ARG, "bad remap field arguments");
  fcx_engine::RemapField f;
  f.phase = phase;
  f.s = s;
  f.g = g;
  f.var = var;
  if (flags & FCX_MEM_DEVICE) {
    f.out_dev = out;
    f.external = true;
  } else {
    f.out_host = out;
  }
  e->remaps[(size_t)remap_id].fields.push_back(f);
  return FCX_OK;
}

extern "C" int fcx_remap_info(const fcx_engine *e, int32_t remap_id, double *scatter, int32_t *packed) {
  if (!e || !scatter || !packed) return fail(FCX_E_ARG, "NULL argument");
  if (!e->committed) return fail(FCX_E_STATE, "remap info is known after fcx_commit");
  if (remap_id < 0 || remap_id >= (int32_t)e->remaps.size()) return fail(FCX_E_ARG, "remap %d unknown", remap_id);
  const auto &rm = e->remaps[(size_t)remap_id];
  int nf_max = 0;
  for (int ph = 1; ph <= 3; ++ph) {
    int c = 0;
    for (auto &f : rm.fields) c += (f.phase & ph) ? 1 : 0;
    nf_max = std::max(nf_max, std::min(c, kMaxAtmosFields));
  }
  *scatter = rm.scatter;
  *packed = e->d_rec && remap_packs(e, rm, nf_max) ? 1 : 0;
  if (e->rec_plan && e->rec_plan->rec_remap == remap_id) *packed = 2;
  return FCX_OK;
}

#include <dlfcn.h>
#include <rccl/rccl.h>

namespace {

struct RcclApi {
  bool ok = false;
  std::string why;
// ... 274 lines not shown
```

### components.flux_calculator_amd/csrc/fcx_internal.h

```cpp
#pragma once
#include <cstdint>
#include "../../include/fcx.h"

#if !defined(FCX_AB_BUILD)
#if defined(FCX_TRIVIAL_MATH) || defined(FCX_DBG_ATM_NOLDS) || defined(FCX_DBG_ATM_NOSTORE) || \
    defined(FCX_DBG_NO_HEAD)
#error "FCX_TRIVIAL_MATH / FCX_DBG_*: wrong-result measurement builds need FCX_AB_BUILD"
#endif
#endif
#ifndef FCX_TRIVIAL_MATH
#define FCX_TRIVIAL_MATH 0
#endif
#ifndef FCX_DBG_ATM_NOLDS
#define FCX_DBG_ATM_NOLDS 0
#endif
#ifndef FCX_DBG_ATM_NOSTORE
#define FCX_DBG_ATM_NOSTORE 0
#endif
#ifndef FCX_DBG_NO_HEAD
#define FCX_DBG_NO_HEAD 0
#endif
#if !defined(FCX_AB_BUILD) && defined(FCX_WAVE_TRACE)
#error "FCX_WAVE_TRACE is a measurement build (FCX_AB_BUILD)"
#endif
#ifndef FCX_WAVE_TRACE
#define FCX_WAVE_TRACE 0
#endif
#ifndef FCX_HALO_RAVG
#define FCX_HALO_RAVG 0
#endif
#ifndef FCX_F64_COMPACT
#define FCX_F64_COMPACT 1
#endif

namespace fcx {

constexpr int kMaxTypes = FCX_MAX_SURFACE_TYPES;
constexpr int kNumVars = FCX_NUM_VARS;
constexpr int kMaxAvg = 24;

enum Stage : uint32_t {
  S_RBBR = 1u << 0,
  S_QSUR_T = 1u << 1,
  S_QSUR_U = 1u << 2,
  S_QSUR_V = 1u << 3,
  S_MEVA = 1u << 4,
  S_HLAT = 1u << 5,
  S_HSEN = 1u << 6,
  S_UMOM = 1u << 7,
  S_VMOM = 1u << 8,
  S_RSDR = 1u << 9,
  S_AVG = 1u << 10,
};

struct TGridPtrs {
  const double *tsur, *fice, *psur, *patm, *qatm, *tatm, *uatm, *vatm;
  const double *amoi, *cmoi, *chea;
  const double *qsur_in;
  const double *meva_in;
  double *qsur, *meva, *hlat, *hsen, *rbbr, *rsdr;
};
struct UVGridPtrs {
  const double *tsur, *fice, *psur, *uatm, *vatm, *amom, *cmom;
  const double *qsur_in;
  double *qsur, *mom;
};
struct TypeParams {
  TGridPtrs t;
  UVGridPtrs uv[2];
  int8_t m_qsur[3], m_meva, m_hlat, m_hsen, m_mom, m_rbbr;
  int8_t bias_adds;
  int8_t pad[7];
};
struct AvgEntry {
  double *x0;
  int32_t grid;
  int32_t pad;
  const double *x[kMaxTypes];
  const double *fare[kMaxTypes];
};
enum AvgSlot : int { A_MEVA = 0, A_HLAT = 1, A_HSEN = 2, A_RBBR = 3, A_UMOM = 4, A_VMOM = 5, A_TSUR = 6 };
constexpr int kAvgSlots = 7;
struct AvgRegs {
  double *out[kAvgSlots];
  const double *fare[kMaxTypes];
};

#ifndef FCX_LAYOUT_SHIFT
#define FCX_LAYOUT_SHIFT 12
#endif
constexpr int kLayoutShift = FCX_LAYOUT_SHIFT;
constexpr int64_t kLayoutTile = int64_t(1) << kLayoutShift;
__host__ __device__ inline int64_t tiled(int64_t j, int64_t tpad) { return j + (j >> kLayoutShift) * tpad; }

struct Params {
  int64_t n[3];
  int64_t n_max;
  int32_t num_types;
  uint32_t stages;
  const double *rsdd0;
  int32_t merged_uv;
  int32_t num_avg;
  TypeParams type[kMaxTypes];
  AvgEntry avg[kMaxAvg];
  AvgRegs ravg;
  int32_t ravg_on;
  int32_t pad2;
  int64_t tpad;
  double *rec;
  int32_t rec_p;
  int8_t rec_pos[6];
  int8_t pad3[2];
};

struct LaunchConfig {
  int cells_per_thread = 2;
  int max_blocks = -1;
  bool nontemporal = true;
  bool merged = false;
  int variant = 0;
  bool f32 = false;
  bool ravg = false;
  int64_t lo = 0, hi = -1;
  bool rec = false;
  int halo = 0;
};
constexpr int64_t kChunkAlign = 1024;

struct AtmosFused;
int launch_cells(const Params *host_params, const Params *dev_params, const double *corr_m,
                 const LaunchConfig &lc, void *stream, const AtmosFused *atm = nullptr);
constexpr int kMaxAtmosFields = 16;
struct AtmosArgs {
  const int32_t *row_ptr;
  const int32_t *col;
  const double *w;
  int64_t n_atmos;
  int32_t nf;
  int32_t stride;
  int32_t left, right;
  double *shared;
  const double *x[kMaxAtmosFields];
  double *out[kMaxAtmosFields];
  int32_t f32;
  int64_t tpad;
  int64_t out_tpad;
  int32_t vec;
  int32_t rec_p;
  const void *rec;
  int32_t scol[kMaxAtmosFields];
};
int launch_atmos(const AtmosArgs &a, void *stream);
struct FinishGroup;
int launch_atmos_finish_group(const AtmosArgs *as, const int32_t *n_boundaries, int n, void *stream);
int launch_pack_records(const AtmosArgs &a, int64_t n, bool aligned16, bool nontemporal, void *rec, void *stream);

constexpr int kFusedFields = 6;
constexpr int kRecHead = 4;
constexpr int kXRec = 32;
constexpr int kTile = 128;
constexpr bool compact_map(bool f32, bool halo) {
  return f32 || FCX_F64_COMPACT == 2 || (FCX_F64_COMPACT == 1 && halo);
}
struct AtmosFused {
  const uint32_t *seg_bits;
  const int32_t *seg_pre;
  const int32_t *seg_atm;
  const int32_t *tile_a0;
  const int32_t *idx;
  const double *w;
  double *out[kFusedFields];
  const double *x[kFusedFields];
  double *xrec;
  int32_t xrec_on;
  int32_t halo;
  int64_t n_atmos;
  double *shared;
  int32_t stride, left, right;
  int64_t tpad;
  int64_t out_tpad;
  int32_t scol[kFusedFields];
  int64_t n_tiles;
#if FCX_WAVE_TRACE
  uint64_t *trace;
#endif
};
constexpr int kMaxGroup = 4;
struct FinishGroup {
  int32_t n;
  int32_t nb[kMaxGroup];
  AtmosArgs a[kMaxGroup];
};
#ifndef FCX_F32_CPL
#define FCX_F32_CPL 4
#endif
constexpr int kF32Cpl = FCX_F32_CPL;
struct GroupMember {
  const Params *P;
  const double *corr_m;
  int64_t tile0;
  int32_t var;
  int32_t pad;
  AtmosFused af;
};
constexpr int kMaxGroupRanges = kMaxGroup;
struct GroupRange {
  int64_t t0;
  int64_t first;
  int32_t member;
  int32_t pad;
};
struct GroupArgs {
  int32_t n;
  int32_t n_ranges;
  int64_t total_tiles;
  GroupMember m[kMaxGroup];
  GroupRange r[kMaxGroupRanges];
};
int launch_cells_group(GroupMember *members, int n, const LaunchConfig &lc, void *stream);

int launch_atmos_fixup(const AtmosFused &af, int64_t n_cells, bool f32, void *stream);
int launch_atmos_zero(const AtmosFused &af, const int32_t *cells, int64_t n, bool f32, void *stream);
struct FixupGroup {
  int32_t n;
  int32_t pad;
  int64_t first[kMaxGroup + 1];
  AtmosFused af[kMaxGroup];
};
int launch_atmos_fixup_group(const AtmosFused *afs, const int64_t *n_cells, int n, bool f32, void *stream);
int launch_atmos_finish(const AtmosArgs &a, int32_t n_boundaries, void *stream);

int launch_regrid_csr(const int32_t *row_ptr, const int32_t *col, const double *w,
                      const double *src, double *dst, int64_t n_dst, void *stream, bool f32 = false,
                      int64_t tpad = 0);
int launch_zero(double *x, int64_t n, void *stream);

}
```

### components.flux_calculator_amd/csrc/fcx_kernels.hip

```cpp
#include <hip/hip_runtime.h>

#include <algorithm>
#include <type_traits>
#include "fcx_internal.h"
#include "fcx_physics.h"

#pragma clang fp contract(off)

namespace fcx {

template <int C, class R = double>
struct Vec {
  R v[C];
};

typedef double d2 __attribute__((ext_vector_type(2)));
#if FCX_WAVE_TRACE
typedef unsigned long long u64x2 __attribute__((ext_vector_type(2)));
#endif
typedef float f4 __attribute__((ext_vector_type(4)));
typedef float f2v __attribute__((ext_vector_type(2)));
typedef int i2v __attribute__((ext_vector_type(2)));
typedef int i4v __attribute__((ext_vector_type(4)));

// ... 557 lines not shown
constexpr int tile_cells() { return 64 * C; }
template <int C>
constexpr int row_len() { return tile_cells<C>() + 2 * (tile_cells<C>() / 16); }
__device__ __forceinline__ int lds_slot(int e) { return e + 2 * (e >> 4); }

template <int C>
constexpr int xrows_doubles() { return kFusedFields * tile_cells<C>() / 2; }
#ifndef FCX_F32_SEG_ORDINAL
#define FCX_F32_SEG_ORDINAL 1
#endif
constexpr int kSegCap = 192;
template <class R, int C>
constexpr bool seg_ordinal() { return FCX_F32_SEG_ORDINAL && sizeof(R) == 4 && C == 4; }
template <class R, int C>
constexpr int wave_lds_doubles(int rows) {
  return sizeof(R) == 4 ? xrows_doubles<C>() + row_len<C>() + (seg_ordinal<R, C>() ? kSegCap : 0)
                        : rows * row_len<C>();
}

template <int C>
struct LdsEmitT {
  double *p;
  double w[C];
  int s;
  template <int CC, class R>
  __device__ __forceinline__ void operator()(int k, const Vec<CC, R> &x) const {
    static_assert(CC == C, "one emitter per cell width");
    if (FCX_DBG_ATM_NOLDS) return;
    if constexpr (sizeof(R) == 4 && C == 4) {
      const int lane = threadIdx.x & 63;
      *reinterpret_cast<f4 *>(reinterpret_cast<float *>(p) + k * tile_cells<C>() + C * lane) =
          f4{x.v[0], x.v[1], x.v[2], x.v[3]};
      return;
    } else if constexpr (sizeof(R) == 4 && C == 2) {
      const int lane = threadIdx.x & 63;
      *reinterpret_cast<f2v *>(reinterpret_cast<float *>(p) + k * tile_cells<C>() + C * lane) = f2v{x.v[0], x.v[1]};
      return;
    }
#pragma unroll
    for (int h = 0; h < C / 2; ++h) {
      const d2 q = {w[2 * h] * (double)x.v[2 * h], w[2 * h + 1] * (double)x.v[2 * h + 1]};
      *reinterpret_cast<d2 *>(p + k * row_len<C>() + s + 2 * h) = q;
    }
  }
};

__device__ __forceinline__ void wave_sync() {
  __builtin_amdgcn_fence(__ATOMIC_RELEASE, "wavefront");
  __builtin_amdgcn_wave_barrier();
  __builtin_amdgcn_fence(__ATOMIC_ACQUIRE, "wavefront");
}

__device__ __forceinline__ int first_bit(uint64_t m) { return m ? __builtin_ctzll(m) : 64; }

constexpr uint32_t kXcds = 8;
#ifndef FCX_XCD_CHUNK
#define FCX_XCD_CHUNK 64
#endif
#ifndef FCX_XCD_CHUNK_F32
#define FCX_XCD_CHUNK_F32 32
#endif
template <uint32_t K>
__device__ __forceinline__ uint32_t xcd_block(uint32_t b, uint32_t nb) {
  constexpr uint32_t row = K * kXcds;
  const uint32_t full = nb / row * row;
  if (b >= full) return b;
  const uint32_t x = b % kXcds, i = b / kXcds;
  return i / K * row + x * K + i % K;
}

template <class R>
__device__ __forceinline__ void segment_done(const AtmosFused &af, int64_t tile, int32_t a, const double *acc,
                                             bool cont) {
  if (cont) {
#pragma unroll
    for (int q = 0; q < kFusedFields / 2; ++q)
      gptr(reinterpret_cast<d2 *>(af.xrec + (tile + 1) * kXRec))[q] = d2{acc[2 * q], acc[2 * q + 1]};
    return;
  }
  if (FCX_DBG_ATM_NOSTORE) return;
#pragma unroll
  for (int k = 0; k < kFusedFields; ++k) {
    if (!af.out[k]) continue;
    FCX_GLOBAL R *o = gptr(reinterpret_cast<R *>(af.out[k]) + tiled(a, af.out_tpad));
    if constexpr (sizeof(R) == 8)
      __builtin_nontemporal_store((R)acc[k], o);
    else
      *o = (R)acc[k];
    if (a == 0 && af.left >= 0) gptr(af.shared)[(int64_t)af.left * af.stride + af.scol[k]] = acc[k];
    if (a == af.n_atmos - 1 && af.right >= 0) gptr(af.shared)[(int64_t)af.right * af.stride + af.scol[k]] = acc[k];
  }
}

#ifndef FCX_RAVG_ATMOS_BLOCKS
#define FCX_RAVG_ATMOS_BLOCKS 3
#endif
#ifndef FCX_T1_ATMOS_BLOCKS
#define FCX_T1_ATMOS_BLOCKS 1
#endif
#ifndef FCX_F32_ATMOS_BLOCKS
#define FCX_F32_ATMOS_BLOCKS 4
#endif
#ifndef FCX_ATMOS_WAVES
#define FCX_ATMOS_WAVES 4
#endif
#ifndef FCX_F32_ATMOS_WAVES
#define FCX_F32_ATMOS_WAVES 4
#endif
template <int C>
constexpr int atmos_waves() { return C == 4 ? FCX_F32_ATMOS_WAVES : FCX_ATMOS_WAVES; }
template <int C, class R, int VAR, bool NT, int TM, bool RAVG, bool REC, bool HALO>
__device__ __forceinline__ void atmos_tile(const Params *__restrict__ P, const double *__restrict__ corr_m,
                                           const AtmosFused &af, int64_t tile, double *wp) {
  constexpr int kT = tile_cells<C>();
  constexpr int kR = row_len<C>();
  constexpr bool kXF = sizeof(R) == 4;
  const int64_t n = P->n_max;
  const int own_lanes = HALO ? 64 - af.halo : 64;
  const int64_t kO = (int64_t)C * own_lanes;
  const int lane = threadIdx.x & 63;
  const uint64_t at_or_above = ~0ull << lane;
  const uint64_t above = lane == 63 ? 0ull : (~0ull << (lane + 1));
    const int64_t t0 = tile * kO;
    const int64_t j0 = t0 + C * lane;
    LdsEmitT<C> emit{wp, {}, lds_slot(C * lane)};
    constexpr bool kCompact = compact_map(sizeof(R) == 4, HALO);
    const int sh = (int)(j0 & 31);
    uint32_t word = 0;
    int32_t before = 0;
    int32_t a[C];
#pragma unroll
    for (int i = 0; i < C; ++i) a[i] = -1;
    int32_t a0_tile = 0;
    if constexpr (kCompact) {
      if (j0 < n) {
        word = gptr(af.seg_bits)[j0 >> 5];
        before = gptr(af.seg_pre)[j0 >> 5];
      }
      if (!HALO && af.xrec_on) a0_tile = gptr(af.tile_a0)[tile];
    } else if (j0 + C <= n) {
      const i2v ii = *gptr(reinterpret_cast<const i2v *>(af.idx + j0));
      a[0] = ii.x;
      a[1] = ii.y;
    } else {
#pragma unroll
      for (int i = 0; i < C; ++i)
        if (j0 + i < n) a[i] = gptr(af.idx)[j0 + i];
    }
    if (j0 + C <= n) {
#pragma unroll
      for (int h = 0; h < C / 2; ++h) {
        const d2 ww = __builtin_nontemporal_load(gptr(reinterpret_cast<const d2 *>(af.w + j0) + h));
        emit.w[2 * h] = ww[0];
        emit.w[2 * h + 1] = ww[1];
      }
    } else {
#pragma unroll
      for (int i = 0; i < C; ++i)
        if (j0 + i < n) emit.w[i] = gptr(af.w)[j0 + i];
    }
    const int64_t tend = t0 + kT;
    bool next_cont;
    int32_t prev_tile = -2;
    if constexpr (kCompact) {
      next_cont = tend < n && !((gptr(af.seg_bits)[tend >> 5] >> (tend & 31)) & 1u);
    } else {
      prev_tile = t0 > 0 ? gptr(af.idx)[t0 - 1] : -2;
      next_cont = tend < n && gptr(af.idx)[tend] == gptr(af.idx)[tend - 1];
    }
    if (j0 < n)
      process<C, true, VAR, NT, R, TM, RAVG, LdsEmitT<C>, REC, HALO>(
          P, corr_m, j0, emit, AccLds<C, R>{reinterpret_cast<R *>(wp + emit.s), kR}, t0 + kO);
    if constexpr (kXF) {
#pragma unroll
      for (int h = 0; h < C / 2; ++h)
        *reinterpret_cast<d2 *>(wp + xrows_doubles<C>() + emit.s + 2 * h) = d2{emit.w[2 * h], emit.w[2 * h + 1]};
    }
    auto add_cell = [&](double *acc, int e) {
      if constexpr (kXF) {
        const float *xr = reinterpret_cast<const float *>(wp);
        const double we = wp[xrows_doubles<C>() + lds_slot(e)];
#pragma unroll
        for (int k = 0; k < kFusedFields; ++k) acc[k] = acc[k] + we * (double)xr[k * kT + e];
      } else {
        const double *q = wp + lds_slot(e);
#pragma unroll
        for (int k = 0; k < kFusedFields; ++k) acc[k] = acc[k] + q[k * kR];
      }
    };
    bool st[C];
    uint64_t m[C];
    if constexpr (kCompact) {
      before += __builtin_popcount(word & ((1u << sh) - 1u));
      int32_t ord = before;
#pragma unroll
      for (int i = 0; i < C; ++i) {
        const bool valid = j0 + i < n;
        st[i] = !valid || ((word >> (sh + i)) & 1u);
        if (valid && st[i]) a[i] = gptr(af.seg_atm)[ord++];
        m[i] = __ballot(st[i]);
      }
    } else {
      int32_t prev = __shfl_up(a[C - 1], 1);
      if (lane == 0) prev = prev_tile;
#pragma unroll
      for (int i = 0; i < C; ++i) {
        st[i] = a[i] != (i ? a[i - 1] : prev);
        m[i] = __ballot(st[i]);
      }
    }
    wave_sync();
    uint32_t rem = 0;
#pragma unroll
    for (int i = 0; i < C; ++i)
      if (st[i] && j0 + i < n && (!HALO || lane < own_lanes)) rem |= 1u << i;
    auto seg_end = [&](int i) {
      int e_end = kT;
#pragma unroll
      for (int q = 0; q < C; ++q) e_end = min(e_end, C * first_bit(m[q] & (q > i ? at_or_above : above)) + q);
      return min(e_end, kT);
    };
    auto seg_end_of = [&](int c) {
      const int l = c / C, i = c % C;
      const uint64_t ge = ~0ull << l, gt = l == 63 ? 0ull : (~0ull << (l + 1));
      int e_end = kT;
#pragma unroll
      for (int q = 0; q < C; ++q) e_end = min(e_end, C * first_bit(m[q] & (q > i ? ge : gt)) + q);
      return min(e_end, kT);
    };
    if constexpr (seg_ordinal<R, C>()) {
      static_assert(kT == 256 && kSegCap * 8 == kT * 6, "one list entry per cell of the tile");
      uint16_t *seg = reinterpret_cast<uint16_t *>(wp + xrows_doubles<C>() + row_len<C>());
      int32_t *seg_a = reinterpret_cast<int32_t *>(seg + kT);
      const uint64_t lower = (1ull << lane) - 1;
      int total = 0, o = 0;
#pragma unroll
      for (int q = 0; q < C; ++q) {
        const uint64_t b = __ballot((rem >> q) & 1u);
        total += __popcll(b);
        o += __popcll(b & lower);
      }
#pragma unroll
      for (int i = 0; i < C; ++i)
        if ((rem >> i) & 1u) {
          seg[o] = (uint16_t)(C * lane + i);
          seg_a[o] = a[i];
          ++o;
        }
      wave_sync();
      for (int base = 0; base < total; base += 64) {
        const int sg = base + lane;
        if (sg < total) {
          const int c = seg[sg];
          const int end = seg_end_of(c);
          const int32_t ai = seg_a[sg];
          double acc[kFusedFields];
#pragma unroll
          for (int k = 0; k < kFusedFields; ++k) acc[k] = 0.0;
          for (int e = c; e < end; ++e) add_cell(acc, e);
          segment_done<R>(af, tile, ai, acc, !HALO && end == kT && next_cont);
        }
      }
      rem = 0;
    }
    while (__ballot(rem != 0)) {
      if (rem) {
        const int i = __builtin_ctz(rem);
        rem &= rem - 1;
        int32_t ai = a[0];
#pragma unroll
        for (int q = 1; q < C; ++q)
          if (q == i) ai = a[q];
        const int c = C * lane + i;
        const int end = seg_end(i);
        double acc[kFusedFields];
#pragma unroll
        for (int k = 0; k < kFusedFields; ++k) acc[k] = 0.0;
        for (int e = c; e < end; ++e) add_cell(acc, e);
        segment_done<R>(af, tile, ai, acc, !HALO && end == kT && next_cont);
      }
    }
    if (!HALO && af.xrec_on) {
      int head = kT;
#pragma unroll
      for (int q = 0; q < C; ++q) head = min(head, C * first_bit(m[q]) + q);
      if (FCX_DBG_NO_HEAD >= 2) head = 0;
      double *xr0 = af.xrec + tile * kXRec;
      if (lane == 0 && FCX_DBG_NO_HEAD < 2) {
        const int32_t a0 = kCompact ? a0_tile : a[0];
        *gptr(reinterpret_cast<i2v *>(xr0 + 30)) = i2v{head, a0};
      }
      if (FCX_DBG_NO_HEAD) head = 0;
      if (lane < min(head, kRecHead)) {
        double hp[kFusedFields];
        if constexpr (kXF) {
          const float *xr = reinterpret_cast<const float *>(wp);
          const double we = wp[xrows_doubles<C>() + lds_slot(lane)];
#pragma unroll
          for (int k = 0; k < kFusedFields; ++k) hp[k] = we * (double)xr[k * kT + lane];
        } else {
#pragma unroll
          for (int k = 0; k < kFusedFields; ++k) hp[k] = wp[k * kR + lds_slot(lane)];
        }
#pragma unroll
        for (int q = 0; q < kFusedFields / 2; ++q)
          gptr(reinterpret_cast<d2 *>(xr0 + kFusedFields + lane * kFusedFields))[q] = d2{hp[2 * q], hp[2 * q + 1]};
      }
    }
    wave_sync();
}

template <int C, class R, int VAR, bool NT, int TM, bool RAVG, bool REC = false, bool HALO = false>
__global__ __launch_bounds__(64 * atmos_waves<C>(), RAVG  ? FCX_RAVG_ATMOS_BLOCKS
                                                  : REC ? 4
                                                  : (C == 4 && VAR != 3) ? FCX_F32_ATMOS_BLOCKS
                                                                         : FCX_T1_ATMOS_BLOCKS) void cells_atmos_kernel(const Params *__restrict__ P,
                                                          const double *__restrict__ corr_m,
                                                          const AtmosFused af, int64_t lo, int64_t hi) {
  static_assert(!RAVG || (C == 2 && sizeof(R) == 8), "register averages: fp64 engine only");
  static_assert(sizeof(R) == 8 || C == 4 || C == 2, "fp32 flux rows: 4 or 2 cells per lane");
  constexpr int kRows = RAVG ? kAvgSlots : kFusedFields;
  __shared__ double s_p[atmos_waves<C>()][wave_lds_doubles<R, C>(kRows)];
  static_assert(!HALO || (TM == 1 && !RAVG) || (FCX_HALO_RAVG && RAVG), "halo tiles: the T=1 launch");
  const int own_lanes = HALO ? 64 - af.halo : 64;
  const int64_t kO = (int64_t)C * own_lanes;
  const int64_t n_tiles = af.n_tiles;
  const int wv = threadIdx.x >> 6;
  double *wp = s_p[wv];
  const int64_t waves = (int64_t)gridDim.x * (blockDim.x >> 6);
  const int64_t wave0 =
      (int64_t)xcd_block<C == 4 ? FCX_XCD_CHUNK_F32 : FCX_XCD_CHUNK>(blockIdx.x, gridDim.x) * (blockDim.x >> 6) + wv;
#if FCX_WAVE_TRACE
  const int lane = threadIdx.x & 63;
  const uint64_t trace_start = (uint64_t)wall_clock64();
  uint64_t trace_loop = 0;
#endif
  for (int64_t tile = lo / kO + wave0; tile < n_tiles; tile += waves) {
#if FCX_WAVE_TRACE
    if (!trace_loop) trace_loop = (uint64_t)wall_clock64();
#endif
    atmos_tile<C, R, VAR, NT, TM, RAVG, REC, HALO>(P, corr_m, af, tile, wp);
  }
#if FCX_WAVE_TRACE
  if (af.trace) {
    __builtin_amdgcn_s_waitcnt(0);
    const uint64_t trace_end = (uint64_t)wall_clock64();
    if (lane == 0) {
      const uint64_t hw = __builtin_amdgcn_s_getreg((31 << 11) | 4);
      const uint64_t xcc = __builtin_amdgcn_s_getreg((31 << 11) | 20);
      u64x2 *t = reinterpret_cast<u64x2 *>(af.trace + ((int64_t)blockIdx.x * (blockDim.x >> 6) + wv) * 4);
      t[0] = u64x2{trace_start, trace_end};
      t[1] = u64x2{hw | (xcc << 32), trace_loop};
    }
  }
#endif
}


#ifndef FCX_GROUP_BLOCKS
#define FCX_GROUP_BLOCKS 4
#endif
template <int C, class R, bool NT, bool HALO, int TM = 1, bool RAVG = false>
__global__ __launch_bounds__(64 * atmos_waves<C>(), RAVG ? FCX_RAVG_ATMOS_BLOCKS
                                                    : C == 4 ? FCX_F32_ATMOS_BLOCKS : FCX_GROUP_BLOCKS) void
cells_atmos_group_kernel(const GroupArgs g, const Params *__restrict__ P0, const Params *__restrict__ P1,
                         const Params *__restrict__ P2, const Params *__restrict__ P3) {
  constexpr int kRows = RAVG ? kAvgSlots : kFusedFields;
  __shared__ double s_p[atmos_waves<C>()][wave_lds_doubles<R, C>(kRows)];
  const int wv = threadIdx.x >> 6;
  double *wp = s_p[wv];
  const int64_t waves = (int64_t)gridDim.x * (blockDim.x >> 6);
  const int64_t wave0 =
      (int64_t)xcd_block<C == 4 ? FCX_XCD_CHUNK_F32 : FCX_XCD_CHUNK>(blockIdx.x, gridDim.x) * (blockDim.x >> 6) + wv;
  for (int64_t t = wave0; t < g.total_tiles; t += waves) {
    int q = 0;
    for (int j = 1; j < g.n_ranges; ++j)
      if (t >= g.r[j].t0) q = j;
    q = __builtin_amdgcn_readfirstlane(q);
    const GroupRange &rg = g.r[q];
    const int k = __builtin_amdgcn_readfirstlane(rg.member);
    const GroupMember &m = g.m[k];
    const Params *__restrict__ P = k == 0 ? P0 : k == 1 ? P1 : k == 2 ? P2 : P3;
    const int64_t tile = t - rg.t0 + rg.first;
    switch (m.var) {
      case 1: atmos_tile<C, R, 1, NT, TM, RAVG, false, HALO>(P, m.corr_m, m.af, tile, wp); break;
      case 2: atmos_tile<C, R, 2, NT, TM, RAVG, false, HALO>(P, m.corr_m, m.af, tile, wp); break;
      default: atmos_tile<C, R, 3, NT, TM, RAVG, false, HALO>(P, m.corr_m, m.af, tile, wp); break;
    }
  }
}

template <class R, int kT>
__device__ __forceinline__ void fixup_one(const AtmosFused &af, int64_t t, int k) {
  const int64_t x0 = t * kT;
  const double *rec = af.xrec + t * kXRec;
  const int2 ha = *reinterpret_cast<const int2 *>(rec + 30);
  double acc = rec[k];
  double p[kRecHead];
#pragma unroll
  for (int e = 0; e < kRecHead; ++e) p[e] = rec[kFusedFields + e * kFusedFields + k];
  const int h = ha.x;
  const int32_t a = ha.y;
  if (h == 0) return;
#pragma unroll
  for (int e = 0; e < kRecHead; ++e)
    if (e < h) acc = acc + p[e];
  const R *xk = reinterpret_cast<const R *>(af.x[k]);
  for (int e = kRecHead; e < h; ++e) acc = acc + af.w[x0 + e] * (double)xk[tiled(x0 + e, af.tpad)];
  reinterpret_cast<R *>(af.out[k])[tiled(a, af.out_tpad)] = (R)acc;
  if (a == 0 && af.left >= 0) af.shared[(int64_t)af.left * af.stride + af.scol[k]] = acc;
  if (a == af.n_atmos - 1 && af.right >= 0) af.shared[(int64_t)af.right * af.stride + af.scol[k]] = acc;
}

template <class R, int kT>
__global__ __launch_bounds__(256) void atmos_fixup_kernel(const AtmosFused af, int64_t n_tiles) {
  const int64_t i = (int64_t)blockIdx.x * blockDim.x + threadIdx.x;
  const int64_t t = 1 + i / kFusedFields;
  const int k = (int)(i % kFusedFields);
  if (t >= n_tiles || !af.out[k]) return;
  fixup_one<R, kT>(af, t, k);
}

template <class R, int kT>
__global__ __launch_bounds__(256) void atmos_fixup_group_kernel(const FixupGroup g) {
  const int64_t i = (int64_t)blockIdx.x * blockDim.x + threadIdx.x;
  if (i >= g.first[g.n]) return;
  int m = 0;
  for (int q = 1; q < g.n; ++q)
    if (i >= g.first[q]) m = q;
  const int64_t j = i - g.first[m];
  const int64_t t = 1 + j / kFusedFields;
  const int k = (int)(j % kFusedFields);
  if (!g.af[m].out[k]) return;
  fixup_one<R, kT>(g.af[m], t, k);
}

template <class R>
__global__ __launch_bounds__(256) void regrid_csr_kernel(const int32_t *__restrict__ row_ptr,
                                                         const int32_t *__restrict__ col,
                                                         const R *__restrict__ w,
                                                         const R *__restrict__ src,
                                                         R *__restrict__ dst, int64_t n_dst, int64_t tpad) {
  const int64_t d = (int64_t)blockIdx.x * blockDim.x + threadIdx.x;
  if (d >= n_dst) return;
  R acc = R(0);
  for (int32_t k = row_ptr[d]; k < row_ptr[d + 1]; ++k) acc = acc + src[tiled(col[k], tpad)] * w[k];
  dst[tiled(d, tpad)] = acc;
}

#ifndef FCX_ATM_CHUNK
#define FCX_ATM_CHUNK 512
#endif
constexpr int kAtmChunk = FCX_ATM_CHUNK;

template <class R>
__global__ __launch_bounds__(256) void atmos_kernel(const AtmosArgs a) {
  extern __shared__ double lds[];
  const int64_t a0 = (int64_t)blockIdx.x * blockDim.x;
  const int64_t c = a0 + threadIdx.x;
  const int64_t a_end = min(a0 + (int64_t)blockDim.x, a.n_atmos);
  const int32_t K0 = a.row_ptr[a0], K1 = a.row_ptr[a_end];
  constexpr int V = 16 / sizeof(R);
  using VecT = typename std::conditional<sizeof(R) == 8, d2, f4>::type;
  const int32_t n_links = a.vec ? a.row_ptr[a.n_atmos] : 0;
  const bool mine = c < a.n_atmos;
  const int32_t k_lo = mine ? a.row_ptr[c] : 0, k_hi = mine ? a.row_ptr[c + 1] : 0;
  double acc[kMaxAtmosFields];
#pragma unroll
  for (int f = 0; f < kMaxAtmosFields; ++f) acc[f] = 0.0;
  for (int32_t C0 = K0; C0 < K1; C0 += kAtmChunk) {
    const int32_t len = min(kAtmChunk, K1 - C0);
    __syncthreads();
    if (a.vec) {
      const int32_t hi_k = C0 + len;
      for (int32_t v = (C0 & ~(V - 1)) + (int32_t)threadIdx.x * V; v < hi_k; v += (int32_t)blockDim.x * V) {
        const bool full = v + V <= n_links;
        double wv[V];
        if (full) {
#pragma unroll
          for (int h = 0; h < V / 2; ++h) {
            const d2 t = __builtin_nontemporal_load(reinterpret_cast<const d2 *>(a.w + v) + h);
            wv[2 * h] = t[0];
            wv[2 * h + 1] = t[1];
          }
        } else {
#pragma unroll
          for (int i = 0; i < V; ++i) wv[i] = v + i < n_links ? a.w[v + i] : 0.0;
        }
        const int64_t xo = tiled(v, a.tpad);
        for (int f = 0; f < a.nf; ++f) {
          const R *xf = reinterpret_cast<const R *>(a.x[f]) + xo;
          R xv[V];
          if (full) {
            const VecT t = __builtin_nontemporal_load(reinterpret_cast<const VecT *>(xf));
#pragma unroll
            for (int i = 0; i < V; ++i) xv[i] = t[i];
          } else {
#pragma unroll
            for (int i = 0; i < V; ++i) xv[i] = v + i < n_links ? xf[i] : R(0);
          }
#pragma unroll
          for (int i = 0; i < V; ++i)
            if (v + i >= C0 && v + i < hi_k) lds[f * kAtmChunk + (v + i - C0)] = wv[i] * (double)xv[i];
        }
      }
    } else if (a.rec) {
      for (int32_t i = threadIdx.x; i < len; i += blockDim.x) {
        const int32_t k = C0 + i;
        const int32_t xi = __builtin_nontemporal_load(a.col + k);
        const double wk = __builtin_nontemporal_load(a.w + k);
        const VecT *r = reinterpret_cast<const VecT *>(reinterpret_cast<const R *>(a.rec) + (int64_t)xi * a.rec_p);
#pragma unroll
        for (int q = 0; q < kMaxAtmosFields / V; ++q) {
          if (q * V >= a.nf) break;
          const VecT t = r[q];
#pragma unroll
          for (int h = 0; h < V; ++h)
            if (q * V + h < a.nf) lds[(q * V + h) * kAtmChunk + i] = wk * (double)t[h];
        }
      }
    } else {
      for (int32_t i = threadIdx.x; i < len; i += blockDim.x) {
        const int32_t k = C0 + i;
        const int32_t xi = a.col ? a.col[k] : k;
        const double wk = __builtin_nontemporal_load(a.w + k);
#pragma unroll
        for (int f = 0; f < kMaxAtmosFields; ++f)
          if (f < a.nf) lds[f * kAtmChunk + i] = wk * (double)reinterpret_cast<const R *>(a.x[f])[tiled(xi, a.tpad)];
      }
    }
    __syncthreads();
    const int32_t lo = max(k_lo, C0), hi = min(k_hi, C0 + len);
    for (int32_t k = lo; k < hi; ++k) {
#pragma unroll
      for (int f = 0; f < kMaxAtmosFields; ++f)
        if (f < a.nf) acc[f] = acc[f] + lds[f * kAtmChunk + (k - C0)];
    }
  }
  if (!mine) return;
#pragma unroll
  for (int f = 0; f < kMaxAtmosFields; ++f) {
    if (f >= a.nf) break;
    reinterpret_cast<R *>(a.out[f])[tiled(c, a.out_tpad)] = (R)acc[f];
    if (c == 0 && a.left >= 0) a.shared[(int64_t)a.left * a.stride + a.scol[f]] = acc[f];
    if (c == a.n_atmos - 1 && a.right >= 0) a.shared[(int64_t)a.right * a.stride + a.scol[f]] = acc[f];
  }
}

template <class R>
__global__ __launch_bounds__(256) void pack_records_kernel(const AtmosArgs a, int64_t n, int32_t flags, R *rec) {
  constexpr int V = 16 / sizeof(R);
  constexpr int CB = 256 * V;
  using VecT = typename std::conditional<sizeof(R) == 8, d2, f4>::type;
  extern __shared__ unsigned char lds_raw[];
  R *lds = reinterpret_cast<R *>(lds_raw);
  const int64_t c0 = (int64_t)blockIdx.x * CB;
  const int64_t cn = min((int64_t)CB, n - c0);
  const int t = threadIdx.x;
  for (int f = 0; f < a.nf; ++f) {
    const R *x = reinterpret_cast<const R *>(a.x[f]) + tiled(c0, a.tpad);
    const int64_t j = (int64_t)t * V;
    if ((flags & 1) && j + V <= cn) {
      const VecT *p = reinterpret_cast<const VecT *>(x + j);
      const VecT v = (flags & 2) ? __builtin_nontemporal_load(p) : *p;
#pragma unroll
      for (int h = 0; h < V; ++h) lds[f * CB + j + h] = v[h];
    } else {
#pragma unroll
      for (int h = 0; h < V; ++h)
        if (j + h < cn) lds[f * CB + j + h] = x[j + h];
    }
  }
  __syncthreads();
  const int P = a.rec_p;
  const int64_t nvec = cn * P / V;
  VecT *out = reinterpret_cast<VecT *>(rec + c0 * P);
  for (int64_t q = t; q < nvec; q += 256) {
    const int64_t e = q * V;
    const int64_t cell = e / P;
    const int f0 = (int)(e - cell * P);
    VecT v;
#pragma unroll
    for (int h = 0; h < V; ++h) v[h] = f0 + h < a.nf ? lds[(f0 + h) * CB + cell] : R(0);
    __builtin_nontemporal_store(v, out + q);
  }
}

template <class R>
__global__ void atmos_finish_kernel(const AtmosArgs a, int32_t n_boundaries) {
  const int t = threadIdx.x;
  if (t < a.nf) {
    R *out = reinterpret_cast<R *>(a.out[t]);
    if (a.left >= 0) out[0] = (R)a.shared[(int64_t)a.left * a.stride + a.scol[t]];
    if (a.right >= 0) out[tiled(a.n_atmos - 1, a.out_tpad)] = (R)a.shared[(int64_t)a.right * a.stride + a.scol[t]];
  }
  __syncthreads();
  for (int64_t i = t; i < (int64_t)n_boundaries * a.stride; i += blockDim.x) a.shared[i] = 0.0;
}

template <class R>
__global__ void atmos_finish_group_kernel(const FinishGroup g) {
  const AtmosArgs &a = g.a[blockIdx.x];
  const int32_t n_boundaries = g.nb[blockIdx.x];
  const int t = threadIdx.x;
  if (t < a.nf) {
    R *out = reinterpret_cast<R *>(a.out[t]);
    if (a.left >= 0) out[0] = (R)a.shared[(int64_t)a.left * a.stride + a.scol[t]];
    if (a.right >= 0) out[tiled(a.n_atmos - 1, a.out_tpad)] = (R)a.shared[(int64_t)a.right * a.stride + a.scol[t]];
  }
  __syncthreads();
  for (int64_t i = t; i < (int64_t)n_boundaries * a.stride; i += blockDim.x) a.shared[i] = 0.0;
}

__global__ void zero_kernel(double *x, int64_t n) {
  const int64_t stride = (int64_t)gridDim.x * blockDim.x;
  for (int64_t j = (int64_t)blockIdx.x * blockDim.x + threadIdx.x; j < n; j += stride) x[j] = 0.0;
}

static int grid_for(int64_t units, int max_blocks = 256 * 8) {
  int64_t blocks = (units + 255) / 256;
  if (max_blocks > 0 && blocks > max_blocks) blocks = max_blocks;
  if (blocks < 1) blocks = 1;
  return (int)blocks;
}

template <int C, bool MERGED, int VAR, bool NT, class R, int TM, bool RAVG>
static void launch_one(int blocks, hipStream_t s, const Params *dp, const double *corr_m, int64_t lo,
                       int64_t hi) {
  hipLaunchKernelGGL((cells_kernel<C, MERGED, VAR, NT, R, TM, RAVG>), dim3(blocks), dim3(256), 0, s, dp,
                     corr_m, lo, hi);
}

template <int C, bool MERGED, int VAR, class R, int TM, bool RAVG>
static void launch_nt(bool nt, int blocks, hipStream_t s, const Params *dp, const double *corr_m,
                      int64_t lo, int64_t hi) {
  if (nt)
    launch_one<C, MERGED, VAR, true, R, TM, RAVG>(blocks, s, dp, corr_m, lo, hi);
  else
    launch_one<C, MERGED, VAR, false, R, TM, RAVG>(blocks, s, dp, corr_m, lo, hi);
}

template <int C, class R, int TM, bool RAVG>
static void launch_c(const LaunchConfig &lc, int blocks, hipStream_t s, const Params *dp,
                     const double *corr_m, int64_t lo, int64_t hi) {
  if (!lc.merged) {
    launch_nt<C, false, 0, R, TM, RAVG>(lc.nontemporal, blocks, s, dp, corr_m, lo, hi);
    return;
  }
  switch (lc.variant) {
    case 1: launch_nt<C, true, 1, R, TM, RAVG>(lc.nontemporal, blocks, s, dp, corr_m, lo, hi); break;
    case 2: launch_nt<C, true, 2, R, TM, RAVG>(lc.nontemporal, blocks, s, dp, corr_m, lo, hi); break;
    case 3: launch_nt<C, true, 3, R, TM, RAVG>(lc.nontemporal, blocks, s, dp, corr_m, lo, hi); break;
    default: launch_nt<C, true, 0, R, TM, RAVG>(lc.nontemporal, blocks, s, dp, corr_m, lo, hi); break;
  }
}

template <int VAR>
static void launch_rec(bool nt, int blocks, hipStream_t s, const Params *dp, const double *corr_m, int64_t lo,
                       int64_t hi) {
  if (nt)
    hipLaunchKernelGGL((cells_kernel<2, true, VAR, true, double, 1, false, true>), dim3(blocks), dim3(256), 0, s, dp,
                       corr_m, lo, hi);
  else
    hipLaunchKernelGGL((cells_kernel<2, true, VAR, false, double, 1, false, true>), dim3(blocks), dim3(256), 0, s, dp,
                       corr_m, lo, hi);
}

template <int C, class R>
static void launch_r(const Params *hp, const LaunchConfig &lc, int blocks, hipStream_t s, const Params *dp,
                     const double *corr_m, int64_t lo, int64_t hi) {
  if (hp->num_types == 1)
    launch_c<C, R, 1, false>(lc, blocks, s, dp, corr_m, lo, hi);
  else if (lc.ravg)
    launch_c<C, R, 0, true>(lc, blocks, s, dp, corr_m, lo, hi);
  else
    launch_c<C, R, 0, false>(lc, blocks, s, dp, corr_m, lo, hi);
}

template <int C, class R, int VAR, int TM, bool RAVG, bool REC = false, bool HALO = false>
static void launch_atm(bool nt, int blocks, hipStream_t s, const Params *dp, const double *corr_m,
                       const AtmosFused &af, int64_t lo, int64_t hi) {
  if (nt)
    hipLaunchKernelGGL((cells_atmos_kernel<C, R, VAR, true, TM, RAVG, REC, HALO>), dim3(blocks),
                       dim3(64 * atmos_waves<C>()), 0, s, dp, corr_m, af, lo, hi);
  else
    hipLaunchKernelGGL((cells_atmos_kernel<C, R, VAR, false, TM, RAVG, REC, HALO>), dim3(blocks),
                       dim3(64 * atmos_waves<C>()), 0, s, dp, corr_m, af, lo, hi);
}

template <int VAR>
static int launch_atm_r(const Params *hp, const LaunchConfig &lc, int blocks, hipStream_t s, const Params *dp,
                        const double *corr_m, const AtmosFused &af, int64_t lo, int64_t hi) {
  const bool halo = lc.halo > 0;
  if (halo && ((hp->num_types != 1 && !(FCX_HALO_RAVG && lc.ravg)) || lo != 0)) return (int)hipErrorInvalidValue;
  if (hp->num_types == 1 && lc.f32) {
    if (halo)
      launch_atm<kF32Cpl, float, VAR, 1, false, false, true>(lc.nontemporal, blocks, s, dp, corr_m, af, lo, hi);
    else
      launch_atm<kF32Cpl, float, VAR, 1, false>(lc.nontemporal, blocks, s, dp, corr_m, af, lo, hi);
  } else if (lc.f32) {
    return (int)hipErrorInvalidValue;
  } else if (hp->num_types == 1 && lc.rec) {
    if (halo)
      launch_atm<2, double, VAR, 1, false, true, true>(lc.nontemporal, blocks, s, dp, corr_m, af, lo, hi);
    else
      launch_atm<2, double, VAR, 1, false, true>(lc.nontemporal, blocks, s, dp, corr_m, af, lo, hi);
  } else if (hp->num_types == 1) {
    if (halo)
      launch_atm<2, double, VAR, 1, false, false, true>(lc.nontemporal, blocks, s, dp, corr_m, af, lo, hi);
    else
      launch_atm<2, double, VAR, 1, false>(lc.nontemporal, blocks, s, dp, corr_m, af, lo, hi);
  }
  else if (lc.ravg) {
    if constexpr (FCX_HALO_RAVG) {
      if (halo) {
        launch_atm<2, double, VAR, 0, true, false, true>(lc.nontemporal, blocks, s, dp, corr_m, af, lo, hi);
        return 0;
      }
    }
    launch_atm<2, double, VAR, 0, true>(lc.nontemporal, blocks, s, dp, corr_m, af, lo, hi);
  } else
    return (int)hipErrorInvalidValue;
  return 0;
}

#if FCX_WAVE_TRACE
static struct {
  uint64_t *base = nullptr;
  int64_t stride = 0;
  int64_t slots = 1;
  int64_t launches = 0;
} g_trace;
}
extern "C" int fcx_debug_wave_trace(uint64_t *base, int64_t stride_words, int64_t slots, int64_t *wall_khz) {
  fcx::g_trace.base = base;
  fcx::g_trace.stride = stride_words;
  fcx::g_trace.slots = slots > 0 ? slots : 1;
  fcx::g_trace.launches = 0;
  int rate = 0, dev = 0;
  if (hipGetDevice(&dev) != hipSuccess || hipDeviceGetAttribute(&rate, hipDeviceAttributeWallClockRate, dev) != hipSuccess)
    return 1;
  if (wall_khz) *wall_khz = rate;
  return 0;
}
namespace fcx {
#endif

int launch_cells(const Params *hp, const Params *dp, const double *corr_m, const LaunchConfig &lc,
                 void *stream, const AtmosFused *atm) {
  hipStream_t s = reinterpret_cast<hipStream_t>(stream);
  const int64_t lo = lc.lo, hi = lc.hi < 0 ? hp->n_max : std::min<int64_t>(lc.hi, hp->n_max);
  if (lo % kChunkAlign || lo < 0) return (int)hipErrorInvalidValue;
  if (hi <= lo) return 0;
  AtmosFused afl;
  if (atm) {
    afl = *atm;
    const int64_t own = (lc.f32 ? kF32Cpl : 2) * (64 - lc.halo);
    afl.n_tiles = (hi + own - 1) / own;
#if FCX_WAVE_TRACE
    afl.trace = g_trace.base ? g_trace.base + (g_trace.launches++ % g_trace.slots) * g_trace.stride : nullptr;
#endif
    atm = &afl;
  }
  if (atm) {
    const int64_t kt = (lc.f32 ? kF32Cpl : 2) * (64 - lc.halo);
    const int64_t kw = lc.f32 ? atmos_waves<kF32Cpl>() : atmos_waves<2>();
    const int64_t tiles = (hi - lo + kt - 1) / kt;
    const int64_t full = (tiles + kw - 1) / kw;
    const int blocks = (int)std::max<int64_t>(1, lc.max_blocks > 0 ? std::min<int64_t>(full, lc.max_blocks) : full);
    int r = 0;
    switch (lc.variant) {
      case 1: r = launch_atm_r<1>(hp, lc, blocks, s, dp, corr_m, *atm, lo, hi); break;
      case 2: r = launch_atm_r<2>(hp, lc, blocks, s, dp, corr_m, *atm, lo, hi); break;
      case 3: r = launch_atm_r<3>(hp, lc, blocks, s, dp, corr_m, *atm, lo, hi); break;
      default: return (int)hipErrorInvalidValue;
    }
    if (r) return r;
    return (int)hipGetLastError();
  }
  const int c = lc.cells_per_thread == 1 ? 1 : lc.f32 ? 4 : 2;
  const int64_t units = (hi - lo + c - 1) / c;
  const int blocks = grid_for(units, lc.max_blocks < 0 ? 8192 : lc.max_blocks);
  if (lc.rec) {
    if (lc.f32 || c != 2 || hp->num_types != 1 || !lc.merged || lc.variant < 1 || lc.variant > 3)
      return (int)hipErrorInvalidValue;
    switch (lc.variant) {
      case 1: launch_rec<1>(lc.nontemporal, blocks, s, dp, corr_m, lo, hi); break;
      case 2: launch_rec<2>(lc.nontemporal, blocks, s, dp, corr_m, lo, hi); break;
      default: launch_rec<3>(lc.nontemporal, blocks, s, dp, corr_m, lo, hi); break;
    }
    return (int)hipGetLastError();
  }
  if (lc.f32) {
    if (c == 4)
      launch_r<4, float>(hp, lc, blocks, s, dp, corr_m, lo, hi);
    else
      launch_r<1, float>(hp, lc, blocks, s, dp, corr_m, lo, hi);
  } else if (c == 2) {
    launch_r<2, double>(hp, lc, blocks, s, dp, corr_m, lo, hi);
  } else {
    launch_r<1, double>(hp, lc, blocks, s, dp, corr_m, lo, hi);
  }
  return (int)hipGetLastError();
}

template <int C, class R, bool NT>
static void launch_group_h(bool halo, bool ravg, int blocks, hipStream_t s, const GroupArgs &g) {
  const Params *p[kMaxGroup];
  for (int k = 0; k < kMaxGroup; ++k) p[k] = g.m[k < g.n ? k : 0].P;
  if constexpr (C == 2 && sizeof(R) == 8) {
    if (ravg) {
      hipLaunchKernelGGL((cells_atmos_group_kernel<C, R, NT, false, 0, true>), dim3(blocks),
                         dim3(64 * atmos_waves<C>()), 0, s, g, p[0], p[1], p[2], p[3]);
      return;
    }
  }
  if (halo)
    hipLaunchKernelGGL((cells_atmos_group_kernel<C, R, NT, true>), dim3(blocks), dim3(64 * atmos_waves<C>()), 0, s, g,
                       p[0], p[1], p[2], p[3]);
  else
    hipLaunchKernelGGL((cells_atmos_group_kernel<C, R, NT, false>), dim3(blocks), dim3(64 * atmos_waves<C>()), 0, s,
                       g, p[0], p[1], p[2], p[3]);
}

int launch_cells_group(GroupMember *members, int n, const LaunchConfig &lc, void *stream) {
  if (n < 1 || n > kMaxGroup) return (int)hipErrorInvalidValue;
  hipStream_t s = reinterpret_cast<hipStream_t>(stream);
  GroupArgs g{};
  g.n = n;
  int64_t total = 0;
  for (int k = 0; k < n; ++k) {
    GroupMember &m = members[k];
    if (m.var < 1 || m.var > 3 || (m.af.halo > 0) != (lc.halo > 0) || m.af.n_tiles < 0)
      return (int)hipErrorInvalidValue;
    m.tile0 = total;
    g.m[k] = m;
    g.r[k] = GroupRange{total, 0, k, 0};
    total += m.af.n_tiles;
  }
  g.n_ranges = n;
  g.total_tiles = total;
  if (total == 0) return 0;
  const int64_t kw = lc.f32 ? atmos_waves<kF32Cpl>() : atmos_waves<2>();
  const int blocks = (int)std::max<int64_t>(1, (total + kw - 1) / kw);
  if (lc.ravg && (lc.f32 || lc.halo > 0)) return (int)hipErrorInvalidValue;
  if (lc.f32) {
    if (lc.nontemporal) launch_group_h<kF32Cpl, float, true>(lc.halo > 0, false, blocks, s, g);
    else launch_group_h<kF32Cpl, float, false>(lc.halo > 0, false, blocks, s, g);
  } else {
    if (lc.nontemporal) launch_group_h<2, double, true>(lc.halo > 0, lc.ravg, blocks, s, g);
    else launch_group_h<2, double, false>(lc.halo > 0, lc.ravg, blocks, s, g);
  }
  return (int)hipGetLastError();
}

int launch_regrid_csr(const int32_t *row_ptr, const int32_t *col, const double *w,
                      const double *src, double *dst, int64_t n_dst, void *stream, bool f32, int64_t tpad) {
  if (n_dst <= 0) return 0;
  const int blocks = (int)((n_dst + 255) / 256);
  hipStream_t s = reinterpret_cast<hipStream_t>(stream);
  if (f32)
    hipLaunchKernelGGL(regrid_csr_kernel<float>, dim3(blocks), dim3(256), 0, s, row_ptr, col,
                       reinterpret_cast<const float *>(w), reinterpret_cast<const float *>(src),
                       reinterpret_cast<float *>(dst), n_dst, tpad);
  else
    hipLaunchKernelGGL(regrid_csr_kernel<double>, dim3(blocks), dim3(256), 0, s, row_ptr, col, w, src, dst, n_dst, tpad);
  return (int)hipGetLastError();
}

int launch_atmos(const AtmosArgs &a, void *stream) {
  if (a.n_atmos <= 0 || a.nf <= 0) return 0;
  const int blocks = (int)((a.n_atmos + 255) / 256);
  const size_t lds = (size_t)a.nf * kAtmChunk * sizeof(double);
  if (a.f32)
    hipLaunchKernelGGL(atmos_kernel<float>, dim3(blocks), dim3(256), lds, reinterpret_cast<hipStream_t>(stream), a);
  else
    hipLaunchKernelGGL(atmos_kernel<double>, dim3(blocks), dim3(256), lds, reinterpret_cast<hipStream_t>(stream), a);
  return (int)hipGetLastError();
}

int launch_pack_records(const AtmosArgs &a, int64_t n, bool aligned16, bool nontemporal, void *rec, void *stream) {
  if (n <= 0 || a.nf <= 0) return 0;
  const int V = a.f32 ? 4 : 2;
  if (a.rec_p < a.nf || a.rec_p % V || a.nf > kMaxAtmosFields) return (int)hipErrorInvalidValue;
  const int64_t cb = 256 * V;
  const int blocks = (int)((n + cb - 1) / cb);
  const size_t lds = (size_t)a.nf * cb * (a.f32 ? 4 : 8);
  const int32_t flags = (aligned16 ? 1 : 0) | (nontemporal ? 2 : 0);
  hipStream_t s = reinterpret_cast<hipStream_t>(stream);
  if (a.f32)
    hipLaunchKernelGGL(pack_records_kernel<float>, dim3(blocks), dim3(256), lds, s, a, n, flags,
                       reinterpret_cast<float *>(rec));
  else
    hipLaunchKernelGGL(pack_records_kernel<double>, dim3(blocks), dim3(256), lds, s, a, n, flags,
                       reinterpret_cast<double *>(rec));
  return (int)hipGetLastError();
}

int launch_atmos_finish(const AtmosArgs &a, int32_t n_boundaries, void *stream) {
  if (!a.shared) return 0;
  if (a.f32)
    hipLaunchKernelGGL(atmos_finish_kernel<float>, dim3(1), dim3(256), 0, reinterpret_cast<hipStream_t>(stream),
                       a, n_boundaries);
  else
    hipLaunchKernelGGL(atmos_finish_kernel<double>, dim3(1), dim3(256), 0, reinterpret_cast<hipStream_t>(stream),
                       a, n_boundaries);
  return (int)hipGetLastError();
}

int launch_atmos_finish_group(const AtmosArgs *as, const int32_t *nbs, int n, void *stream) {
  if (n < 1 || n > kMaxGroup) return (int)hipErrorInvalidValue;
  FinishGroup g{};
  g.n = n;
  for (int k = 0; k < n; ++k) {
    if (!as[k].shared || as[k].f32 != as[0].f32) return (int)hipErrorInvalidValue;
    g.a[k] = as[k];
    g.nb[k] = nbs[k];
  }
  hipStream_t s = reinterpret_cast<hipStream_t>(stream);
  if (as[0].f32)
    hipLaunchKernelGGL(atmos_finish_group_kernel<float>, dim3(n), dim3(256), 0, s, g);
  else
    hipLaunchKernelGGL(atmos_finish_group_kernel<double>, dim3(n), dim3(256), 0, s, g);
  return (int)hipGetLastError();
}

int launch_atmos_fixup(const AtmosFused &af, int64_t n, bool f32, void *stream) {
  const int64_t kt = f32 ? tile_cells<kF32Cpl>() : tile_cells<2>();
  const int64_t tiles = (n + kt - 1) / kt;
  if (tiles < 2) return 0;
  const int blocks = (int)(((tiles - 1) * kFusedFields + 255) / 256);
  hipStream_t s = reinterpret_cast<hipStream_t>(stream);
  if (f32)
    hipLaunchKernelGGL((atmos_fixup_kernel<float, tile_cells<kF32Cpl>()>), dim3(blocks), dim3(256), 0, s, af, tiles);
  else
    hipLaunchKernelGGL((atmos_fixup_kernel<double, tile_cells<2>()>), dim3(blocks), dim3(256), 0, s, af, tiles);
  return (int)hipGetLastError();
}

template <class R>
__global__ __launch_bounds__(256) void atmos_zero_kernel(const AtmosFused af, const int32_t *cells, int64_t n) {
  const int64_t i = (int64_t)blockIdx.x * blockDim.x + threadIdx.x;
  if (i >= n) return;
  const int32_t a = cells[i];
#pragma unroll
  for (int k = 0; k < kFusedFields; ++k)
    if (af.out[k]) reinterpret_cast<R *>(af.out[k])[tiled(a, af.out_tpad)] = R(0);
}

int launch_atmos_zero(const AtmosFused &af, const int32_t *cells, int64_t n, bool f32, void *stream) {
  if (n <= 0) return 0;
  const int blocks = (int)((n + 255) / 256);
  hipStream_t s = reinterpret_cast<hipStream_t>(stream);
  if (f32)
    hipLaunchKernelGGL(atmos_zero_kernel<float>, dim3(blocks), dim3(256), 0, s, af, cells, n);
  else
    hipLaunchKernelGGL(atmos_zero_kernel<double>, dim3(blocks), dim3(256), 0, s, af, cells, n);
  return (int)hipGetLastError();
}

int launch_atmos_fixup_group(const AtmosFused *afs, const int64_t *n_cells, int n, bool f32, void *stream) {
  if (n < 1 || n > kMaxGroup) return (int)hipErrorInvalidValue;
  const int64_t kt = f32 ? tile_cells<kF32Cpl>() : tile_cells<2>();
  FixupGroup g{};
  g.n = n;
  for (int m = 0; m < n; ++m) {
    g.af[m] = afs[m];
    const int64_t tiles = (n_cells[m] + kt - 1) / kt;
    g.first[m + 1] = g.first[m] + std::max<int64_t>(tiles - 1, 0) * kFusedFields;
  }
  if (g.first[n] == 0) return 0;
  const int blocks = (int)((g.first[n] + 255) / 256);
  hipStream_t s = reinterpret_cast<hipStream_t>(stream);
  if (f32)
    hipLaunchKernelGGL((atmos_fixup_group_kernel<float, tile_cells<kF32Cpl>()>), dim3(blocks), dim3(256), 0, s, g);
  else
    hipLaunchKernelGGL((atmos_fixup_group_kernel<double, tile_cells<2>()>), dim3(blocks), dim3(256), 0, s, g);
  return (int)hipGetLastError();
}

int launch_zero(double *x, int64_t n, void *stream) {
  if (n <= 0) return 0;
  hipLaunchKernelGGL(zero_kernel, dim3(grid_for(n)), dim3(256), 0,
                     reinterpret_cast<hipStream_t>(stream), x, n);
  return (int)hipGetLastError();
}

}
```

### components.flux_calculator_amd/python/fcx/_lib.py

```python
import ctypes
import os

_HERE = os.path.dirname(os.path.abspath(__file__))
LIB_PATH = os.path.normpath(os.path.join(_HERE, "..", "..", "lib", "libfcx.so"))
if os.environ.get("FCX_LIBRARY"):
    LIB_PATH = os.path.abspath(os.environ["FCX_LIBRARY"])

FCX_OK = 0
FCX_MEM_HOST = 0x0
FCX_MEM_DEVICE = 0x1
FCX_ALLOCATED = 0x2
FCX_CORR_CELL_MAJOR = 0
FCX_CORR_MONTH_MAJOR = 1
FCX_PRECISION_F64 = 0
FCX_PRECISION_F32 = 1
FCX_COMM_ID_BYTES = 128

_c = ctypes
_P = _c.c_void_p
_I = _c.c_int
_I32 = _c.c_int32
_I64 = _c.c_int64
_DP = _c.POINTER(_c.c_double)
SIGNATURES = [
    ("fcx_last_error", _c.c_char_p, []),
    ("fcx_version", _I, []),
    ("fcx_method_from_string", _I, [_c.c_char_p, _c.c_size_t]),
    ("fcx_current_month", _I, [_I32, _I64, _c.POINTER(_I32)]),
    ("fcx_create", _I, [_I, _I, _c.POINTER(_I32), _c.POINTER(_P)]),
    ("fcx_destroy", _I, [_P]),
    ("fcx_set_stream", _I, [_P, _P]),
    ("fcx_set_method", _I, [_P, _I, _I, _I]),
    ("fcx_bind_field", _I, [_P, _I, _I, _I, _P, _I64, _I]),
    ("fcx_set_corrections", _I, [_P, _I, _I32, _P, _I64, _I]),
    ("fcx_set_regrid_matrix", _I, [_P, _I, _I64, _P, _P, _P]),
    ("fcx_set_put_to", _I, [_P, _I, _I, _I, _I]),
    ("fcx_add_average", _I, [_P, _I, _I, _I]),
    ("fcx_set_precision", _I, [_P, _I]),
    ("fcx_commit", _I, [_P]),
    ("fcx_plan_check", _I, [_P]),
    ("fcx_upload", _I, [_P, _I]),
    ("fcx_run", _I, [_P, _I, _I32]),
    ("fcx_download", _I, [_P, _I]),
    ("fcx_step", _I, [_P, _I, _I32]),
    ("fcx_synchronize", _I, [_P]),
    ("fcx_calc_spec_vapor_surface", _I, [_P, _I]),
    ("fcx_calc_flux_mass_evap", _I, [_P, _I32]),
    ("fcx_calc_flux_heat_latent", _I, [_P]),
    ("fcx_calc_flux_heat_sensible", _I, [_P]),
    ("fcx_calc_flux_momentum_east", _I, [_P, _I]),
    ("fcx_calc_flux_momentum_north", _I, [_P, _I]),
    ("fcx_calc_flux_radiation_blackbody", _I, [_P]),
    ("fcx_distribute_shortwave_radiation_flux", _I, [_P]),
    ("fcx_average_across_surface_types", _I, [_P, _I, _I]),
    ("fcx_do_regridding", _I, [_P, _I, _I]),
    ("fcx_device_ptr", _I, [_P, _I, _I, _I, _c.POINTER(_DP)]),
    ("fcx_device_layout", _I, [_P, _c.POINTER(_I64), _c.POINTER(_I64)]),
    ("fcx_last_kernel_ms", _I, [_P, _c.POINTER(_c.c_float)]),
    ("fcx_staging_bytes", _I, [_P, _c.POINTER(_I64)]),
    ("fcx_algorithmic_bytes", _I, [_P, _I, _c.POINTER(_I64)]),
    ("fcx_span_runs", _I, [_P, _I, _c.POINTER(_I32), _c.POINTER(_I32)]),
    ("fcx_zero_copy_bytes", _I, [_P, _c.POINTER(_I64)]),
    ("fcx_run_group", _I, [_P, _I, _I, _I32]),
    ("fcx_pinned_bytes", _I, [_P, _c.POINTER(_I64)]),
    ("fcx_handoff_recoveries", _I, [_P, _c.POINTER(_I64)]),
    ("fcx_host_malloc", _I, [_c.c_size_t, _c.POINTER(_P)]),
    ("fcx_set_atmos_boundaries", _I, [_P, _I32, _I32, _I32]),
    ("fcx_comm_unique_id", _I, [_P]),
    ("fcx_comm_create", _I, [_I, _I, _I, _P, _c.POINTER(_P)]),
    ("fcx_comm_destroy", _I, [_P]),
    ("fcx_comm_allreduce_sum", _I, [_P, _P, _c.c_size_t, _P]),
    ("fcx_set_comm", _I, [_P, _P]),
    ("fcx_atmos_allreduce", _I, [_P, _c.POINTER(_P), _I]),
    ("fcx_host_free", _I, [_P]),
    ("fcx_add_remap", _I, [_P, _I64, _I64, _P, _P, _P, _P]),
    ("fcx_add_remap_field", _I, [_P, _I32, _I, _I, _I, _I, _P, _I]),
    ("fcx_remap_info", _I, [_P, _I32, _c.POINTER(_c.c_double), _c.POINTER(_I32)]),
    ("fcx_set_option", _I, [_P, _I, _I64]),
    ("fcx_set_atmos_map", _I, [_P, _I64, _P, _P]),
    ("fcx_add_atmos_field", _I, [_P, _I, _I, _I, _I, _P, _I]),
    ("fcx_set_atmos_shared", _I, [_P, _P, _I32, _I32, _I32, _I32]),
    ("fcx_atmos_finish", _I, [_P]),
    ("fcx_run_atmos", _I, [_P, _I]),
    ("fcx_device_malloc", _I, [_I, _c.c_size_t, _c.POINTER(_P)]),
    ("fcx_device_free", _I, [_P]),
    ("fcx_memcpy", _I, [_P, _P, _c.c_size_t, _I]),
    ("fcx_last_group_size", _I, [_P, _c.POINTER(_I32)]),
    ("fcx_step_async", _I, [_P, _I, _I32]),
    ("fcx_upload_field", _I, [_P, _I, _I, _I]),
    ("fcx_comm_verify", _I, [_P, _I]),
    ("fcx_set_abort_handler", _I, [_P]),
    ("fcx_abort", _I, [_c.c_char_p]),
]


class FcxError(RuntimeError):

    def __init__(self, status, message):
        super().__init__(f"fcx status {status}: {message}")
        self.status = status


_lib = None


def load():
    global _lib
    if _lib is None:
        if not os.environ.get("FCX_NO_TORCH"):
            try:
                import torch
            except ImportError:
                pass
        if not os.path.exists(LIB_PATH):
            raise FcxError(-1, f"{LIB_PATH} is not built (run __graft_entry__.build())")
        lib = ctypes.CDLL(LIB_PATH)
        _bind(lib, strict=not os.environ.get("FCX_LIBRARY"))
        _lib = lib
    return _lib


def load_path(path):
    load()
    lib = ctypes.CDLL(os.path.abspath(path))
    _bind(lib, strict=False)
    return lib


def _bind(lib, strict=True):
    for name, res, args in SIGNATURES:
        try:
            fn = getattr(lib, name)
        except AttributeError:
            if strict:
                raise
            continue
        fn.restype = res
        fn.argtypes = args


def check(status):
    if status != FCX_OK:
        raise FcxError(status, load().fcx_last_error().decode(errors="replace"))
    return status
```

### components.flux_calculator_amd/python/fcx/engine.py

```python
import ctypes

import numpy as np

from . import _lib
from .basic import FLUX_ID, IDX, METHOD_ID, PHASE_ALL, PHASE_EARLY, PHASE_NORMAL
from .local_field import LocalFields, data_ptr, dtype_name, is_device


class Engine:

    def __init__(self, lf: LocalFields, num_surface_types, methods, corrections=None,
                 averages=(), regrid=None, device=0, stream=None, atmos=None, options=None, remaps=None,
                 lib=None, commit=True):
        self.lib = lib if lib is not None else _lib.load()
        self.lf = lf
        self.T = int(num_surface_types)
        self.methods = {k: list(v) for k, v in methods.items()}
        self._keep = []
        h = ctypes.c_void_p()
        gs = (ctypes.c_int32 * 3)(*lf.grid_size)
        _lib.check(self.lib.fcx_create(device, self.T, gs, ctypes.byref(h)))
        self.h = h
        try:
            if stream is not None:
# ... 67 lines not shown
                _lib.check(self.lib.fcx_add_remap(h, int(rm["n_dst"]), src.shape[0], ctypes.c_void_p(src.ctypes.data),
                                                  ctypes.c_void_p(dst.ctypes.data), ctypes.c_void_p(w.ctypes.data),
                                                  ctypes.byref(rid)))
                for phase, s, g, name, out in rm["fields"]:
                    if dtype_name(out) != dtype:
                        raise TypeError(f"remap output {name}: {dtype_name(out)} array in a {dtype} engine")
                    flags = _lib.FCX_MEM_DEVICE if is_device(out) else _lib.FCX_MEM_HOST
                    self._keep.append(out)
                    _lib.check(self.lib.fcx_add_remap_field(h, rid.value, phase, s, g, IDX[name],
                                                            ctypes.c_void_p(data_ptr(out)), flags))
            for name, value in (options or {}).items():
                _lib.check(self.lib.fcx_set_option(h, self._option_id(name), int(value)))
            if commit:
                _lib.check(self.lib.fcx_commit(h))
        except Exception:
            self.lib.fcx_destroy(h)
            self.h = None
            raise

    def plan_check(self):
        _lib.check(self.lib.fcx_plan_check(self.h))

    def commit(self):
        _lib.check(self.lib.fcx_commit(self.h))

    def upload(self, phase=PHASE_ALL):
        _lib.check(self.lib.fcx_upload(self.h, phase))

    def run(self, phase=PHASE_ALL, current_step_time=0):
        _lib.check(self.lib.fcx_run(self.h, phase, int(current_step_time)))

    def download(self, phase=PHASE_ALL):
        _lib.check(self.lib.fcx_download(self.h, phase))

    def step(self, phase=PHASE_ALL, current_step_time=0):
        _lib.check(self.lib.fcx_step(self.h, phase, int(current_step_time)))

    def step_async(self, phase=PHASE_ALL, current_step_time=0):
        _lib.check(self.lib.fcx_step_async(self.h, phase, int(current_step_time)))

    def upload_field(self, surface_type, grid, name):
        _lib.check(self.lib.fcx_upload_field(self.h, int(surface_type), int(grid), IDX[name]))

    def set_stream(self, stream):
        _lib.check(self.lib.fcx_set_stream(self.h, ctypes.c_void_p(stream)))

    def do_regridding(self, name, surface_type=0):
        _lib.check(self.lib.fcx_do_regridding(self.h, IDX[name], int(surface_type)))

    def synchronize(self):
        _lib.check(self.lib.fcx_synchronize(self.h))

    def last_kernel_ms(self):
        ms = ctypes.c_float()
        _lib.check(self.lib.fcx_last_kernel_ms(self.h, ctypes.byref(ms)))
        return ms.value

    def algorithmic_bytes(self, phase=PHASE_ALL):
        b = ctypes.c_int64()
        _lib.check(self.lib.fcx_algorithmic_bytes(self.h, phase, ctypes.byref(b)))
        return b.value

    def staging_bytes(self):
        b = ctypes.c_int64()
        _lib.check(self.lib.fcx_staging_bytes(self.h, ctypes.byref(b)))
        return b.value

    def zero_copy_bytes(self):
        b = ctypes.c_int64()
        _lib.check(self.lib.fcx_zero_copy_bytes(self.h, ctypes.byref(b)))
        return b.value

    def span_runs(self, phase=PHASE_ALL):
        a, b = ctypes.c_int32(), ctypes.c_int32()
        _lib.check(self.lib.fcx_span_runs(self.h, phase, ctypes.byref(a), ctypes.byref(b)))
        return a.value, b.value

    def zero_copy_active(self):
        return self.zero_copy_bytes() > 0

    OPTIONS = {"cells_per_thread": 1, "max_blocks": 2, "nontemporal": 3, "specialize": 4,
               "atmos_in_run": 5, "pipeline_chunks": 7, "pipeline_min_chunk": 8, "zero_copy": 9,
               "timing": 10, "tiled_layout": 11, "remap_pack": 13, "host_staging": 15, "host_threads": 16,
               "atmos_halo": 17, "deferred_scatter": 18, "lib_spans": 19}

    def run_atmos(self, phase=PHASE_ALL):
        _lib.check(self.lib.fcx_run_atmos(self.h, phase))

    def atmos_finish(self):
        _lib.check(self.lib.fcx_atmos_finish(self.h))

    def remap_info(self, remap_id=0):
        sc, pk = ctypes.c_double(), ctypes.c_int32()
        _lib.check(self.lib.fcx_remap_info(self.h, remap_id, ctypes.byref(sc), ctypes.byref(pk)))
        return sc.value, pk.value

    @classmethod
    def _option_id(cls, name):
        if isinstance(name, int) or (isinstance(name, str) and name.isdigit()):
            return int(name)
        return cls.OPTIONS[name]

    def set_option(self, name, value):
        _lib.check(self.lib.fcx_set_option(self.h, self._option_id(name), int(value)))

    def device_ptr(self, s, g, name):
        p = ctypes.POINTER(ctypes.c_double)()
        _lib.check(self.lib.fcx_device_ptr(self.h, s, g, IDX[name], ctypes.byref(p)))
        return ctypes.cast(p, ctypes.c_void_p).value

    def device_layout(self):
        tile, stride = ctypes.c_int64(), ctypes.c_int64()
        _lib.check(self.lib.fcx_device_layout(self.h, ctypes.byref(tile), ctypes.byref(stride)))
        return tile.value, stride.value

    def last_group_size(self):
        m = ctypes.c_int32()
        _lib.check(self.lib.fcx_last_group_size(self.h, ctypes.byref(m)))
        return m.value

    def close(self):
        if self.h is not None:
            self.lib.fcx_destroy(self.h)
            self.h = None

    def __del__(self):
        try:
            self.close()
        except Exception:
            pass


def run_group(engines, phase=PHASE_ALL, current_step_time=0):
    if not engines:
        return
    lib = engines[0].lib
    arr = (ctypes.c_void_p * len(engines))(*[e.h.value for e in engines])
    _lib.check(lib.fcx_run_group(arr, len(engines), phase, int(current_step_time)))


def current_month(init_date, seconds):
    lib = _lib.load()
    m = ctypes.c_int32()
    _lib.check(lib.fcx_current_month(int(init_date), int(seconds), ctypes.byref(m)))
    return m.value


__all__ = ["Engine", "run_group", "current_month", "PHASE_EARLY", "PHASE_NORMAL", "PHASE_ALL"]
```

### include/fcx.h

```cpp
#ifndef FCX_H
#define FCX_H
#include <stddef.h>
#include <stdint.h>

#ifdef __cplusplus
extern "C" {
#endif

#define FCX_VERSION 1
#define FCX_MAX_SURFACE_TYPES 10
#define FCX_NUM_VARS 35

enum fcx_var {
  FCX_ALBE = 1, FCX_ALBA, FCX_AMOI, FCX_AMOM, FCX_FARE, FCX_FICE, FCX_PATM, FCX_PSUR,
  FCX_QATM, FCX_TATM, FCX_TSUR, FCX_UATM, FCX_VATM, FCX_U10M, FCX_V10M,
  FCX_CMOM, FCX_CMOI, FCX_CHEA, FCX_QSUR, FCX_HLAT, FCX_HSEN,
  FCX_MEVA, FCX_MPRE, FCX_MRAI, FCX_MSNO,
  FCX_RBBR, FCX_RLWD, FCX_RLWU, FCX_RSID, FCX_RSIU, FCX_RSIN, FCX_RSDD, FCX_RSDR,
  FCX_UMOM, FCX_VMOM
};

enum fcx_grid { FCX_T_GRID = 1, FCX_U_GRID = 2, FCX_V_GRID = 3 };

enum fcx_method {
  FCX_NONE = 0, FCX_ZERO, FCX_COPY, FCX_CCLM, FCX_MOM5, FCX_RCO, FCX_WATER, FCX_ICE, FCX_STBO
};

enum fcx_flux {
  FCX_SPEC_VAPOR_SURFACE_T = 0, FCX_SPEC_VAPOR_SURFACE_U, FCX_SPEC_VAPOR_SURFACE_V,
  FCX_FLUX_MASS_EVAP, FCX_FLUX_HEAT_LATENT, FCX_FLUX_HEAT_SENSIBLE, FCX_FLUX_MOMENTUM,
  FCX_FLUX_RADIATION_BLACKBODY, FCX_NUM_FLUXES
};

enum fcx_phase { FCX_PHASE_EARLY = 1, FCX_PHASE_NORMAL = 2, FCX_PHASE_ALL = 3 };

enum fcx_regrid { FCX_U_TO_T = 0, FCX_V_TO_T, FCX_T_TO_U, FCX_T_TO_V };

enum fcx_status {
  FCX_OK = 0, FCX_E_ARG = 1, FCX_E_STATE = 2, FCX_E_UNSUPPORTED = 3, FCX_E_HIP = 4,
  FCX_E_MISSING = 5, FCX_E_NOMEM = 6
};

#define FCX_MEM_HOST   0x0
#define FCX_MEM_DEVICE 0x1
#define FCX_ALLOCATED  0x2

#define FCX_CORR_CELL_MAJOR  0
#define FCX_CORR_MONTH_MAJOR 1

typedef struct fcx_engine fcx_engine;

const char *fcx_last_error(void);
int fcx_version(void);

typedef void (*fcx_abort_handler)(const char *message);
int fcx_set_abort_handler(fcx_abort_handler handler);
int fcx_abort(const char *message);

int fcx_method_from_string(const char *s, size_t len);

int fcx_current_month(int32_t init_date, int64_t seconds, int32_t *month);

int fcx_create(int device, int num_surface_types, const int32_t grid_size[3], fcx_engine **out);
int fcx_destroy(fcx_engine *e);
int fcx_set_stream(fcx_engine *e, void *hip_stream);
int fcx_set_method(fcx_engine *e, int flux, int surface_type, int method);
int fcx_bind_field(fcx_engine *e, int surface_type, int grid, int var, double *ptr, int64_t n,
                   int flags);
int fcx_set_corrections(fcx_engine *e, int enabled, int32_t init_date, const double *corr,
                        int64_t n, int layout);
int fcx_set_regrid_matrix(fcx_engine *e, int which, int64_t num_elements, const int32_t *src_index,
                          const int32_t *dst_index, const double *weight);
int fcx_set_put_to(fcx_engine *e, int surface_type, int grid, int var, int mask);
int fcx_add_average(fcx_engine *e, int phase, int grid, int var);
enum fcx_precision { FCX_PRECISION_F64 = 0, FCX_PRECISION_F32 = 1 };
int fcx_set_precision(fcx_engine *e, int precision);
int fcx_commit(fcx_engine *e);
int fcx_plan_check(fcx_engine *e);

int fcx_upload(fcx_engine *e, int phase);
int fcx_run(fcx_engine *e, int phase, int32_t current_step_time);
int fcx_download(fcx_engine *e, int phase);
int fcx_run_group(fcx_engine *const *engines, int n_engines, int phase, int32_t current_step_time);
int fcx_last_group_size(fcx_engine *e, int32_t *members);
int fcx_step(fcx_engine *e, int phase, int32_t current_step_time);
int fcx_synchronize(fcx_engine *e);
int fcx_step_async(fcx_engine *e, int phase, int32_t current_step_time);
int fcx_upload_field(fcx_engine *e, int surface_type, int grid, int var);

int fcx_calc_spec_vapor_surface(fcx_engine *e, int which_grid);
int fcx_calc_flux_mass_evap(fcx_engine *e, int32_t current_step_time);
int fcx_calc_flux_heat_latent(fcx_engine *e);
int fcx_calc_flux_heat_sensible(fcx_engine *e);
int fcx_calc_flux_momentum_east(fcx_engine *e, int which_grid);
int fcx_calc_flux_momentum_north(fcx_engine *e, int which_grid);
int fcx_calc_flux_radiation_blackbody(fcx_engine *e);
int fcx_distribute_shortwave_radiation_flux(fcx_engine *e);
int fcx_average_across_surface_types(fcx_engine *e, int which_grid, int var);
int fcx_do_regridding(fcx_engine *e, int var, int surface_type);

int fcx_device_ptr(fcx_engine *e, int surface_type, int grid, int var, double **dptr);
int fcx_device_layout(fcx_engine *e, int64_t *tile, int64_t *tile_stride);
int fcx_last_kernel_ms(fcx_engine *e, float *ms);
int fcx_staging_bytes(fcx_engine *e, int64_t *bytes);
int fcx_pinned_bytes(fcx_engine *e, int64_t *bytes);
int fcx_handoff_recoveries(fcx_engine *e, int64_t *count);
int fcx_zero_copy_bytes(fcx_engine *e, int64_t *bytes);
int fcx_span_runs(fcx_engine *e, int phase, int32_t *h2d_copies, int32_t *d2h_copies);
int fcx_algorithmic_bytes(fcx_engine *e, int phase, int64_t *bytes);

int fcx_set_atmos_map(fcx_engine *e, int64_t n_atmos, const int32_t *atmos_index,
                      const double *weight);
int fcx_add_atmos_field(fcx_engine *e, int phase, int surface_type, int grid, int var,
                        double *out, int flags);
int fcx_set_atmos_shared(fcx_engine *e, double *shared, int32_t n_boundaries, int32_t stride,
                         int32_t left, int32_t right);
int fcx_set_atmos_boundaries(fcx_engine *e, int32_t n_boundaries, int32_t left, int32_t right);
int fcx_atmos_finish(fcx_engine *e);
int fcx_run_atmos(fcx_engine *e, int phase);

#define FCX_COMM_ID_BYTES 128
typedef struct fcx_comm fcx_comm;
int fcx_comm_unique_id(void *id );
int fcx_comm_create(int device, int nranks, int rank, const void *id, fcx_comm **out);
int fcx_comm_destroy(fcx_comm *c);
int fcx_comm_allreduce_sum(fcx_comm *c, double *buf, size_t count, void *hip_stream);
int fcx_set_comm(fcx_engine *e, fcx_comm *c);
int fcx_atmos_allreduce(fcx_comm *c, fcx_engine *const *engines, int n_engines);
int fcx_comm_verify(fcx_comm *c, int every_exchange);

int fcx_add_remap(fcx_engine *e, int64_t n_dst, int64_t n_links, const int32_t *src_cell,
                  const int32_t *dst_cell, const double *weight, int32_t *remap_id);
int fcx_add_remap_field(fcx_engine *e, int32_t remap_id, int phase, int surface_type, int grid,
                        int var, double *out, int flags);
int fcx_remap_info(const fcx_engine *e, int32_t remap_id, double *scatter, int32_t *packed);

enum fcx_option {
  FCX_OPT_CELLS_PER_THREAD = 1,
  FCX_OPT_MAX_BLOCKS = 2,
  FCX_OPT_NONTEMPORAL = 3,
  FCX_OPT_SPECIALIZE = 4,
  FCX_OPT_ATMOS_IN_RUN = 5,
  FCX_OPT_PIPELINE_CHUNKS = 7,
  FCX_OPT_PIPELINE_MIN_CHUNK = 8,
  FCX_OPT_ZERO_COPY = 9,
  FCX_OPT_LIB_SPANS = 19,
  FCX_OPT_TIMING = 10,
  FCX_OPT_HOST_STAGING = 15,
  FCX_OPT_HOST_THREADS = 16,
  FCX_OPT_DEFERRED_SCATTER = 18,
  FCX_OPT_RETIRED_PIN_HOST = 6,
  FCX_OPT_RETIRED_12 = 12,
  FCX_OPT_RETIRED_CARRY_HANDOFF = 14,
  FCX_OPT_ATMOS_HALO = 17,
  FCX_OPT_REMAP_PACK = 13,
  FCX_OPT_TILED_LAYOUT = 11
};
int fcx_set_option(fcx_engine *e, int option, int64_t value);

int fcx_host_malloc(size_t bytes, void **ptr);
int fcx_host_free(void *ptr);

int fcx_device_malloc(int device, size_t bytes, void **ptr);
int fcx_device_free(void *ptr);
int fcx_memcpy(void *dst, const void *src, size_t bytes, int kind);

#ifdef __cplusplus
}
#endif
#endif
```

Baseline: 39710.

## Store atmosphere outputs as interleaved records and unpack to tiled layout before download

Adds an atmosphere-output record layout in which all fused fields of one atmosphere cell are stored contiguously. A new dense halo kernel variant gathers a wave's finished cells in LDS and writes them as one coalesced nontemporal run. A separate unpack kernel then transposes the records into the tiled per-field layout before the host download. The aim is fewer scattered per-field stores in the fused atmosphere kernel, at the cost of an extra device pass over the outputs and a second buffer. It is enabled automatically only for large fp64 single-type halo configurations.

New measurement: 40130 (median of 6 runs). 1.1% higher.

```diff
diff --git a/components.flux_calculator_amd/csrc/fcx_engine.hip b/components.flux_calculator_amd/csrc/fcx_engine.hip
--- a/components.flux_calculator_amd/csrc/fcx_engine.hip
+++ b/components.flux_calculator_amd/csrc/fcx_engine.hip
@@ -214,6 +214,11 @@
   bool exchanged = false;
   void *atm_pool = nullptr;
   int64_t atm_out_tpad = 0;
+  int atm_records_opt = 2;
+  bool atm_records = false;
+  void *atm_soa = nullptr;
+  size_t atm_soa_bytes = 0;
+  int atm_soa_sp = -1;
   bool atmos_in_run = true;
   bool atm_done_fused = false;
   int group_members = 0;
@@ -354,6 +359,8 @@
   e->device = device;
   e->T = num_surface_types;
   for (int g = 0; g < 3; ++g) e->n[g] = grid_size[g];
+  if (const char *v = std::getenv("FCX_ATM_RECORDS"))
+    if ((*v == '0' || *v == '1' || *v == '2') && !v[1]) e->atm_records_opt = *v - '0';
   *out = e;
   return FCX_OK;
 }
@@ -389,6 +396,7 @@
   (void)hipFree(e->d_atm_col);
   (void)hipFree(e->d_atm_w);
   (void)hipFree(e->atm_pool);
+  (void)hipFree(e->atm_soa);
   (void)hipFree(e->atm_shared_own);
   for (auto &r : e->remaps) {
     (void)hipFree(r.d_row);
@@ -727,7 +735,10 @@
   af.left = e->atm_left;
   af.right = e->atm_right;
   af.tpad = e->tpad;
-  af.out_tpad = e->atm_out_tpad;
+  af.out_tpad = e->atm_records ? 0 : e->atm_out_tpad;
+  af.out_stride = e->atm_records ? (int32_t)e->atm_fields.size() : 1;
+  af.rec_dense = e->atm_records && af.out_stride == kFusedFields && nf == kFusedFields;
+  for (int k = 0; k < kFusedFields && af.rec_dense; ++k) af.rec_dense = af.out[k] == af.out[0] + k;
   pl.af = af;
   pl.atm_nf = nf;
   pl.atm_phase = phase;
@@ -1604,9 +1615,12 @@
     cand.push_back(StagePool{(char *)p, nullptr, e->tiled_bytes, true, (size_t)kLayoutTile * es,
                              (size_t)(kLayoutTile + e->tpad) * es});
   if (e->pool) cand.push_back(StagePool{(char *)e->pool, nullptr, e->pool_bytes, false, 0, 0});
+  int atm_cand = -1;
   if (e->atm_pool) {
     const bool t = e->atm_out_tpad != 0;
-    cand.push_back(StagePool{(char *)e->atm_pool, nullptr, e->atm_pool_bytes, t, t ? (size_t)kLayoutTile * es : 0,
+    if (e->atm_records) atm_cand = (int)cand.size();
+    cand.push_back(StagePool{e->atm_records ? nullptr : (char *)e->atm_pool, nullptr,
+                             e->atm_records ? e->atm_soa_bytes : e->atm_pool_bytes, t, t ? (size_t)kLayoutTile * es : 0,
                              t ? (size_t)(kLayoutTile + e->atm_out_tpad) * es : 0});
   }
   for (auto &rm : e->remaps)
@@ -1620,16 +1634,32 @@
   for (auto &bf : e->bufs)
     if (!bf.external && heap(bf.host, bf.n)) mark(bf.dev);
   for (auto &f : e->atm_fields)
-    if (!f.external && heap(f.out_host, e->n_atmos)) mark(f.out_dev);
+    if (!f.external && heap(f.out_host, e->n_atmos)) {
+      if (atm_cand >= 0)
+        used[(size_t)atm_cand] = 1;
+      else
+        mark(f.out_dev);
+    }
   for (auto &rm : e->remaps)
     for (auto &f : rm.fields)
       if (!f.external && heap(f.out_host, rm.n_dst)) mark(f.out_dev);
   for (size_t i = 0; i < cand.size(); ++i)
-    if (used[i]) e->spools.push_back(cand[i]);
+    if (used[i]) {
+      if ((int)i == atm_cand) e->atm_soa_sp = (int)e->spools.size();
+      e->spools.push_back(cand[i]);
+    }
   for (auto &bf : e->bufs)
     if (!bf.external && heap(bf.host, bf.n)) bf.st = stage_ref(e, bf.dev);
-  for (auto &f : e->atm_fields)
-    if (!f.external && heap(f.out_host, e->n_atmos)) f.st = stage_ref(e, f.out_dev);
+  for (size_t k = 0; k < e->atm_fields.size(); ++k) {
+    auto &f = e->atm_fields[k];
+    if (f.external || !heap(f.out_host, e->n_atmos)) continue;
+    if (e->atm_soa_sp >= 0) {
+      f.st.sp = e->atm_soa_sp;
+      f.st.soff = k * (size_t)kLayoutTile * es;
+    } else {
+      f.st = stage_ref(e, f.out_dev);
+    }
+  }
   for (auto &rm : e->remaps)
     for (auto &f : rm.fields)
       if (!f.external && heap(f.out_host, rm.n_dst)) f.st = stage_ref(e, f.out_dev);
@@ -2061,12 +2091,25 @@
     const int64_t nfa = (int64_t)e->atm_fields.size();
     if (FCX_TILED_ATM && e->tpad && !atm_ext && nfa >= 2 && e->n_atmos > 0) {
       const int64_t tiles = (e->n_atmos + kLayoutTile - 1) / kLayoutTile;
-      e->atm_pool_bytes = (size_t)tiles * nfa * kLayoutTile * e->esize;
-      HIP_TRY(hipMalloc(&e->atm_pool, e->atm_pool_bytes));
-      for (int64_t k = 0; k < nfa; ++k)
-        e->atm_fields[k].out_dev = reinterpret_cast<double *>((char *)e->atm_pool + (size_t)k * kLayoutTile * e->esize);
+      const size_t soa_bytes = (size_t)tiles * nfa * kLayoutTile * e->esize;
       e->atm_out_tpad = (nfa - 1) * kLayoutTile;
       need = 0;
+      const int halo_h = (e->atm_maxseg - 1 + 1) / 2;
+      const bool dense_launch = e->T == 1 && nfa == kFusedFields && e->atm_contiguous && e->atm_halo &&
+                                e->atm_crossings > 0 && halo_h >= 1 && halo_h <= 4;
+      e->atm_records = !e->f32 && (e->atm_records_opt == 1 ||
+                                   (e->atm_records_opt == 2 && dense_launch && e->n[0] >= 2 * e->min_chunk));
+      if (e->atm_records) {
+        e->atm_soa_bytes = soa_bytes;
+        e->atm_pool_bytes = ((size_t)e->n_atmos * nfa * sizeof(double) + 255) / 256 * 256;
+        HIP_TRY(hipMalloc(&e->atm_pool, e->atm_pool_bytes));
+        for (int64_t k = 0; k < nfa; ++k) e->atm_fields[k].out_dev = reinterpret_cast<double *>(e->atm_pool) + k;
+      } else {
+        e->atm_pool_bytes = soa_bytes;
+        HIP_TRY(hipMalloc(&e->atm_pool, e->atm_pool_bytes));
+        for (int64_t k = 0; k < nfa; ++k)
+          e->atm_fields[k].out_dev = reinterpret_cast<double *>((char *)e->atm_pool + (size_t)k * kLayoutTile * e->esize);
+      }
     }
     if (need) {
       e->atm_pool_bytes = need;
@@ -2273,6 +2316,8 @@
 static int regrid_var(fcx_engine *e, int var, int surface_type);
 static int comm_exchange(fcx_engine *e);
 static hipError_t get_atm(const fcx_engine *e, double *host, const double *dev, hipStream_t s);
+static int atm_unpack(fcx_engine *e, hipStream_t s);
+static const double *atm_src(const fcx_engine *e, size_t k);
 static int run_remaps(fcx_engine *e, int phase);
 static int download_remaps(fcx_engine *e, int phase, hipStream_t s, std::vector<Xfer> *xs);
 
@@ -2424,13 +2469,19 @@
   stage_prepare_outputs(e);
   std::vector<Xfer> xs;
   std::vector<int> ids = pl->writes;
-  for (auto &f : e->atm_fields)
+  bool any_atm = false;
+  for (auto &f : e->atm_fields) any_atm = any_atm || (f.phase & phase);
+  if (any_atm)
+    if (int r = atm_unpack(e, e->stream)) return r;
+  for (size_t k = 0; k < e->atm_fields.size(); ++k) {
+    auto &f = e->atm_fields[k];
     if ((f.phase & phase) && e->n_atmos > 0) {
       if (f.st.sp >= 0)
         xs.push_back(xfer_of(f.st, f.out_host, e->n_atmos));
       else if (!f.external)
-        HIP_TRY(get_atm(e, f.out_host, f.out_dev, e->stream));
-    }
+        HIP_TRY(get_atm(e, f.out_host, atm_src(e, k), e->stream));
+    }
+  }
   if (int r = download_remaps(e, phase, e->stream, &xs)) return r;
   if (e->any_regrid) {
     std::vector<int> extra;
@@ -2465,6 +2516,22 @@
   return hipSuccess;
 }
 
+static int atm_unpack(fcx_engine *e, hipStream_t s) {
+  if (!e->atm_records || e->n_atmos <= 0) return FCX_OK;
+  if (!e->atm_soa) {
+    HIP_TRY(hipMalloc(&e->atm_soa, e->atm_soa_bytes));
+    if (e->atm_soa_sp >= 0) e->spools[(size_t)e->atm_soa_sp].dev = reinterpret_cast<char *>(e->atm_soa);
+  }
+  const int r = launch_atm_unpack(reinterpret_cast<const double *>(e->atm_pool), reinterpret_cast<double *>(e->atm_soa),
+                                  e->n_atmos, (int)e->atm_fields.size(), e->atm_out_tpad, s);
+  if (r) return fail(FCX_E_HIP, "atm_unpack launch: %s", hipGetErrorString((hipError_t)r));
+  return FCX_OK;
+}
+static const double *atm_src(const fcx_engine *e, size_t k) {
+  if (!e->atm_records) return e->atm_fields[k].out_dev;
+  return reinterpret_cast<const double *>(reinterpret_cast<const char *>(e->atm_soa) + k * (size_t)kLayoutTile * e->esize);
+}
+
 static AtmosArgs atmos_args(fcx_engine *e, int phase) {
   AtmosArgs a{};
   a.f32 = e->f32 ? 1 : 0;
@@ -2477,7 +2544,8 @@
   a.right = e->atm_right;
   a.shared = e->atm_shared;
   a.tpad = e->tpad;
-  a.out_tpad = e->atm_out_tpad;
+  a.out_tpad = e->atm_records ? 0 : e->atm_out_tpad;
+  a.out_stride = e->atm_records ? (int64_t)e->atm_fields.size() : 1;
   a.vec = a.col == nullptr && e->aligned16;
   for (size_t i = 0; i < e->atm_fields.size(); ++i) {
     const auto &f = e->atm_fields[i];
@@ -2511,6 +2579,7 @@
     a.n_atmos = rm.n_dst;
     a.left = a.right = -1;
     a.tpad = e->tpad;
+    a.out_stride = 1;
     auto flush = [&]() -> int {
       if (!a.nf) return FCX_OK;
       a.rec = nullptr;
@@ -2822,14 +2891,21 @@
   HIP_TRY(hipEventRecord(e->ev_comp[K - 1], e->stream));
   HIP_TRY(hipStreamWaitEvent(e->s_out, e->ev_comp[K - 1], 0));
   std::vector<Xfer> xa;
-  if (e->atmos_in_run || e->atm_done_fused)
-    for (auto &f : e->atm_fields)
+  if (e->atmos_in_run || e->atm_done_fused) {
+    bool any_atm = false;
+    for (auto &f : e->atm_fields) any_atm = any_atm || (f.phase & phase);
+    if (any_atm)
+      if (int r = atm_unpack(e, e->s_out)) return r;
+    for (size_t k = 0; k < e->atm_fields.size(); ++k) {
+      auto &f = e->atm_fields[k];
       if ((f.phase & phase) && e->n_atmos > 0) {
         if (f.st.sp >= 0)
           xa.push_back(xfer_of(f.st, f.out_host, e->n_atmos));
         else if (!f.external)
-          HIP_TRY(get_atm(e, f.out_host, f.out_dev, e->s_out));
+          HIP_TRY(get_atm(e, f.out_host, atm_src(e, k), e->s_out));
       }
+    }
+  }
   if (int r = download_remaps(e, phase, e->s_out, &xa)) return r;
   if (!xa.empty()) {
     if (int r = stage_alloc(e, xa)) return r;
@@ -3180,6 +3256,11 @@
       if (value < 0 || value > 2) return fail(FCX_E_ARG, "remap_pack: 0 never, 1 always, 2 auto");
       e->remap_pack = (int)value;
       return FCX_OK;
+    case FCX_OPT_ATM_RECORDS:
+      if (e->committed) return fail(FCX_E_STATE, "atm_records is applied at fcx_commit");
+      if (value < 0 || value > 2) return fail(FCX_E_ARG, "atm_records: 0 never, 1 always, 2 auto");
+      e->atm_records_opt = (int)value;
+      return FCX_OK;
     case FCX_OPT_TILED_LAYOUT:
       if (e->committed) return fail(FCX_E_STATE, "tiled_layout is applied at fcx_commit");
       e->tiled_opt = value != 0;
@@ -3314,6 +3395,13 @@
   return comm_exchange(e);
 }
 
+extern "C" int fcx_atm_records(const fcx_engine *e, int32_t *on) {
+  if (!e || !on) return fail(FCX_E_ARG, "NULL argument");
+  if (!e->committed) return fail(FCX_E_STATE, "the atmosphere output layout is decided at fcx_commit");
+  *on = e->atm_records ? 1 : 0;
+  return FCX_OK;
+}
+
 extern "C" int fcx_last_group_size(fcx_engine *e, int32_t *members) {
   if (!e || !members) return fail(FCX_E_ARG, "NULL argument");
   *members = e->group_members;
diff --git a/components.flux_calculator_amd/csrc/fcx_internal.h b/components.flux_calculator_amd/csrc/fcx_internal.h
--- a/components.flux_calculator_amd/csrc/fcx_internal.h
+++ b/components.flux_calculator_amd/csrc/fcx_internal.h
@@ -92,6 +92,7 @@
 constexpr int kLayoutShift = FCX_LAYOUT_SHIFT;
 constexpr int64_t kLayoutTile = int64_t(1) << kLayoutShift;
 __host__ __device__ inline int64_t tiled(int64_t j, int64_t tpad) { return j + (j >> kLayoutShift) * tpad; }
+__host__ __device__ inline int64_t atm_at(int64_t a, int64_t stride, int64_t tpad) { return tiled(a, tpad) * stride; }
 
 struct Params {
   int64_t n[3];
@@ -145,6 +146,7 @@
   int32_t f32;
   int64_t tpad;
   int64_t out_tpad;
+  int64_t out_stride = 1;
   int32_t vec;
   int32_t rec_p;
   const void *rec;
@@ -179,6 +181,8 @@
   int32_t stride, left, right;
   int64_t tpad;
   int64_t out_tpad;
+  int32_t out_stride = 1;
+  int32_t rec_dense;
   int32_t scol[kFusedFields];
   int64_t n_tiles;
 #if FCX_WAVE_TRACE
@@ -220,6 +224,7 @@
 int launch_cells_group(GroupMember *members, int n, const LaunchConfig &lc, void *stream);
 
 int launch_atmos_fixup(const AtmosFused &af, int64_t n_cells, bool f32, void *stream);
+int launch_atm_unpack(const double *rec, double *soa, int64_t n_atmos, int nf, int64_t tpad, void *stream);
 int launch_atmos_zero(const AtmosFused &af, const int32_t *cells, int64_t n, bool f32, void *stream);
 struct FixupGroup {
   int32_t n;
diff --git a/components.flux_calculator_amd/csrc/fcx_kernels.hip b/components.flux_calculator_amd/csrc/fcx_kernels.hip
--- a/components.flux_calculator_amd/csrc/fcx_kernels.hip
+++ b/components.flux_calculator_amd/csrc/fcx_kernels.hip
@@ -663,7 +663,7 @@
 #pragma unroll
   for (int k = 0; k < kFusedFields; ++k) {
     if (!af.out[k]) continue;
-    FCX_GLOBAL R *o = gptr(reinterpret_cast<R *>(af.out[k]) + tiled(a, af.out_tpad));
+    FCX_GLOBAL R *o = gptr(reinterpret_cast<R *>(af.out[k]) + atm_at(a, af.out_stride, af.out_tpad));
     if constexpr (sizeof(R) == 8)
       __builtin_nontemporal_store((R)acc[k], o);
     else
@@ -673,6 +673,40 @@
   }
 }
 
+__device__ __forceinline__ void record_round(const AtmosFused &af, int32_t a, const double *acc, bool act, bool last,
+                                             double *wp) {
+  if (FCX_DBG_ATM_NOSTORE) return;
+  const int lane = threadIdx.x & 63;
+  const uint64_t am = __ballot(act);
+  const int ord = (int)__builtin_amdgcn_mbcnt_hi((uint32_t)(am >> 32), __builtin_amdgcn_mbcnt_lo((uint32_t)am, 0u));
+  const int cnt = __popcll(am);
+  const int32_t a_first = __builtin_amdgcn_readlane(a, __builtin_amdgcn_readfirstlane(first_bit(am) & 63));
+  const bool dense = last && __ballot(act && a != a_first + ord) == 0;
+  if (dense) {
+    wave_sync();
+    if (act) {
+#pragma unroll
+      for (int q = 0; q < kFusedFields / 2; ++q)
+        reinterpret_cast<d2 *>(wp)[ord * (kFusedFields / 2) + q] = d2{acc[2 * q], acc[2 * q + 1]};
+    }
+    wave_sync();
+    FCX_GLOBAL d2 *run = gptr(reinterpret_cast<d2 *>(af.out[0] + (int64_t)a_first * kFusedFields));
+    for (int c = lane; c < cnt * (kFusedFields / 2); c += 64)
+      __builtin_nontemporal_store(reinterpret_cast<const d2 *>(wp)[c], run + c);
+  } else if (act) {
+    FCX_GLOBAL d2 *rec = gptr(reinterpret_cast<d2 *>(af.out[0] + (int64_t)a * kFusedFields));
+#pragma unroll
+    for (int q = 0; q < kFusedFields / 2; ++q) __builtin_nontemporal_store(d2{acc[2 * q], acc[2 * q + 1]}, rec + q);
+  }
+  if (act) {
+#pragma unroll
+    for (int k = 0; k < kFusedFields; ++k) {
+      if (a == 0 && af.left >= 0) gptr(af.shared)[(int64_t)af.left * af.stride + af.scol[k]] = acc[k];
+      if (a == af.n_atmos - 1 && af.right >= 0) gptr(af.shared)[(int64_t)af.right * af.stride + af.scol[k]] = acc[k];
+    }
+  }
+}
+
 #ifndef FCX_RAVG_ATMOS_BLOCKS
 #define FCX_RAVG_ATMOS_BLOCKS 3
 #endif
@@ -690,7 +724,7 @@
 #endif
 template <int C>
 constexpr int atmos_waves() { return C == 4 ? FCX_F32_ATMOS_WAVES : FCX_ATMOS_WAVES; }
-template <int C, class R, int VAR, bool NT, int TM, bool RAVG, bool REC, bool HALO>
+template <int C, class R, int VAR, bool NT, int TM, bool RAVG, bool REC, int HALO>
 __device__ __forceinline__ void atmos_tile(const Params *__restrict__ P, const double *__restrict__ corr_m,
                                            const AtmosFused &af, int64_t tile, double *wp) {
   constexpr int kT = tile_cells<C>();
@@ -750,7 +784,7 @@
       next_cont = tend < n && gptr(af.idx)[tend] == gptr(af.idx)[tend - 1];
     }
     if (j0 < n)
-      process<C, true, VAR, NT, R, TM, RAVG, LdsEmitT<C>, REC, HALO>(
+      process<C, true, VAR, NT, R, TM, RAVG, LdsEmitT<C>, REC, (HALO != 0)>(
           P, corr_m, j0, emit, AccLds<C, R>{reinterpret_cast<R *>(wp + emit.s), kR}, t0 + kO);
     if constexpr (kXF) {
 #pragma unroll
@@ -844,8 +878,23 @@
       }
       rem = 0;
     }
+    constexpr bool kDense = HALO == 2;
+    static_assert(!kDense || (sizeof(R) == 8 && C == 2 && !REC && !RAVG), "dense records: the fp64 T = 1 halo launch");
     while (__ballot(rem != 0)) {
-      if (rem) {
+      if constexpr (kDense) {
+        const bool act = rem != 0;
+        const int i = act ? __builtin_ctz(rem) : 0;
+        rem &= rem - 1;
+        const int32_t ai = i ? a[C - 1] : a[0];
+        const int c = C * lane + i;
+        const int end = act ? seg_end(i) : c;
+        double acc[kFusedFields];
+        const double *q0 = wp + lds_slot(c);
+#pragma unroll
+        for (int k = 0; k < kFusedFields; ++k) acc[k] = 0.0 + q0[k * kR];
+        for (int e = c + 1; e < end; ++e) add_cell(acc, e);
+        record_round(af, ai, acc, act, __ballot(rem != 0) == 0, wp);
+      } else if (rem) {
         const int i = __builtin_ctz(rem);
         rem &= rem - 1;
         int32_t ai = a[0];
@@ -891,7 +940,7 @@
     wave_sync();
 }
 
-template <int C, class R, int VAR, bool NT, int TM, bool RAVG, bool REC = false, bool HALO = false>
+template <int C, class R, int VAR, bool NT, int TM, bool RAVG, bool REC = false, int HALO = 0>
 __global__ __launch_bounds__(64 * atmos_waves<C>(), RAVG  ? FCX_RAVG_ATMOS_BLOCKS
                                                   : REC ? 4
                                                   : (C == 4 && VAR != 3) ? FCX_F32_ATMOS_BLOCKS
@@ -941,7 +990,7 @@
 #ifndef FCX_GROUP_BLOCKS
 #define FCX_GROUP_BLOCKS 4
 #endif
-template <int C, class R, bool NT, bool HALO, int TM = 1, bool RAVG = false>
+template <int C, class R, bool NT, int HALO, int TM = 1, bool RAVG = false>
 __global__ __launch_bounds__(64 * atmos_waves<C>(), RAVG ? FCX_RAVG_ATMOS_BLOCKS
                                                     : C == 4 ? FCX_F32_ATMOS_BLOCKS : FCX_GROUP_BLOCKS) void
 cells_atmos_group_kernel(const GroupArgs g, const Params *__restrict__ P0, const Params *__restrict__ P1,
@@ -968,6 +1017,7 @@
       case 2: atmos_tile<C, R, 2, NT, TM, RAVG, false, HALO>(P, m.corr_m, m.af, tile, wp); break;
       default: atmos_tile<C, R, 3, NT, TM, RAVG, false, HALO>(P, m.corr_m, m.af, tile, wp); break;
     }
+    if constexpr (HALO == 2) break;
   }
 }
 
@@ -988,7 +1038,7 @@
     if (e < h) acc = acc + p[e];
   const R *xk = reinterpret_cast<const R *>(af.x[k]);
   for (int e = kRecHead; e < h; ++e) acc = acc + af.w[x0 + e] * (double)xk[tiled(x0 + e, af.tpad)];
-  reinterpret_cast<R *>(af.out[k])[tiled(a, af.out_tpad)] = (R)acc;
+  reinterpret_cast<R *>(af.out[k])[atm_at(a, af.out_stride, af.out_tpad)] = (R)acc;
   if (a == 0 && af.left >= 0) af.shared[(int64_t)af.left * af.stride + af.scol[k]] = acc;
   if (a == af.n_atmos - 1 && af.right >= 0) af.shared[(int64_t)af.right * af.stride + af.scol[k]] = acc;
 }
@@ -1122,7 +1172,7 @@
 #pragma unroll
   for (int f = 0; f < kMaxAtmosFields; ++f) {
     if (f >= a.nf) break;
-    reinterpret_cast<R *>(a.out[f])[tiled(c, a.out_tpad)] = (R)acc[f];
+    reinterpret_cast<R *>(a.out[f])[atm_at(c, a.out_stride, a.out_tpad)] = (R)acc[f];
     if (c == 0 && a.left >= 0) a.shared[(int64_t)a.left * a.stride + a.scol[f]] = acc[f];
     if (c == a.n_atmos - 1 && a.right >= 0) a.shared[(int64_t)a.right * a.stride + a.scol[f]] = acc[f];
   }
@@ -1173,7 +1223,7 @@
   if (t < a.nf) {
     R *out = reinterpret_cast<R *>(a.out[t]);
     if (a.left >= 0) out[0] = (R)a.shared[(int64_t)a.left * a.stride + a.scol[t]];
-    if (a.right >= 0) out[tiled(a.n_atmos - 1, a.out_tpad)] = (R)a.shared[(int64_t)a.right * a.stride + a.scol[t]];
+    if (a.right >= 0) out[atm_at(a.n_atmos - 1, a.out_stride, a.out_tpad)] = (R)a.shared[(int64_t)a.right * a.stride + a.scol[t]];
   }
   __syncthreads();
   for (int64_t i = t; i < (int64_t)n_boundaries * a.stride; i += blockDim.x) a.shared[i] = 0.0;
@@ -1187,7 +1237,7 @@
   if (t < a.nf) {
     R *out = reinterpret_cast<R *>(a.out[t]);
     if (a.left >= 0) out[0] = (R)a.shared[(int64_t)a.left * a.stride + a.scol[t]];
-    if (a.right >= 0) out[tiled(a.n_atmos - 1, a.out_tpad)] = (R)a.shared[(int64_t)a.right * a.stride + a.scol[t]];
+    if (a.right >= 0) out[atm_at(a.n_atmos - 1, a.out_stride, a.out_tpad)] = (R)a.shared[(int64_t)a.right * a.stride + a.scol[t]];
   }
   __syncthreads();
   for (int64_t i = t; i < (int64_t)n_boundaries * a.stride; i += blockDim.x) a.shared[i] = 0.0;
@@ -1258,7 +1308,7 @@
     launch_c<C, R, 0, false>(lc, blocks, s, dp, corr_m, lo, hi);
 }
 
-template <int C, class R, int VAR, int TM, bool RAVG, bool REC = false, bool HALO = false>
+template <int C, class R, int VAR, int TM, bool RAVG, bool REC = false, int HALO = 0>
 static void launch_atm(bool nt, int blocks, hipStream_t s, const Params *dp, const double *corr_m,
                        const AtmosFused &af, int64_t lo, int64_t hi) {
   if (nt)
@@ -1287,7 +1337,9 @@
     else
       launch_atm<2, double, VAR, 1, false, true>(lc.nontemporal, blocks, s, dp, corr_m, af, lo, hi);
   } else if (hp->num_types == 1) {
-    if (halo)
+    if (halo && af.rec_dense)
+      launch_atm<2, double, VAR, 1, false, false, 2>(lc.nontemporal, blocks, s, dp, corr_m, af, lo, hi);
+    else if (halo)
       launch_atm<2, double, VAR, 1, false, false, true>(lc.nontemporal, blocks, s, dp, corr_m, af, lo, hi);
     else
       launch_atm<2, double, VAR, 1, false>(lc.nontemporal, blocks, s, dp, corr_m, af, lo, hi);
@@ -1393,6 +1445,15 @@
     if (ravg) {
       hipLaunchKernelGGL((cells_atmos_group_kernel<C, R, NT, false, 0, true>), dim3(blocks),
                          dim3(64 * atmos_waves<C>()), 0, s, g, p[0], p[1], p[2], p[3]);
+      return;
+    }
+  }
+  if constexpr (C == 2 && sizeof(R) == 8) {
+    bool dense = halo;
+    for (int k = 0; k < g.n; ++k) dense = dense && g.m[k].af.rec_dense;
+    if (dense) {
+      hipLaunchKernelGGL((cells_atmos_group_kernel<C, R, NT, 2>), dim3(blocks), dim3(64 * atmos_waves<C>()), 0, s, g,
+                         p[0], p[1], p[2], p[3]);
       return;
     }
   }
@@ -1519,6 +1580,39 @@
   return (int)hipGetLastError();
 }
 
+__global__ __launch_bounds__(256) void atm_unpack_kernel(const double *__restrict__ rec, double *__restrict__ soa,
+                                                         int64_t n_atmos, int nf, int64_t tpad) {
+  constexpr int CB = 256;
+  extern __shared__ unsigned char lds_raw[];
+  double *lds = reinterpret_cast<double *>(lds_raw);
+  const int64_t c0 = (int64_t)blockIdx.x * CB;
+  const int cn = (int)min((int64_t)CB, n_atmos - c0);
+  const int ne = cn * nf;
+  const double *src = rec + c0 * nf;
+  for (int e = 2 * (int)threadIdx.x; e < ne; e += 2 * CB) {
+    if (e + 1 < ne) {
+      const d2 v = __builtin_nontemporal_load(reinterpret_cast<const d2 *>(src + e));
+      lds[e] = v[0];
+      lds[e + 1] = v[1];
+    } else {
+      lds[e] = src[e];
+    }
+  }
+  __syncthreads();
+  const int t = threadIdx.x;
+  if (t >= cn) return;
+  double *dst = soa + tiled(c0, tpad) + t;
+  for (int f = 0; f < nf; ++f) dst[(int64_t)f * kLayoutTile] = lds[t * nf + f];
+}
+
+int launch_atm_unpack(const double *rec, double *soa, int64_t n_atmos, int nf, int64_t tpad, void *stream) {
+  if (n_atmos <= 0 || nf <= 0) return 0;
+  const unsigned blocks = (unsigned)((n_atmos + 255) / 256);
+  hipLaunchKernelGGL(atm_unpack_kernel, dim3(blocks), dim3(256), (size_t)256 * nf * sizeof(double),
+                     reinterpret_cast<hipStream_t>(stream), rec, soa, n_atmos, nf, tpad);
+  return (int)hipGetLastError();
+}
+
 template <class R>
 __global__ __launch_bounds__(256) void atmos_zero_kernel(const AtmosFused af, const int32_t *cells, int64_t n) {
   const int64_t i = (int64_t)blockIdx.x * blockDim.x + threadIdx.x;
@@ -1526,7 +1620,7 @@
   const int32_t a = cells[i];
 #pragma unroll
   for (int k = 0; k < kFusedFields; ++k)
-    if (af.out[k]) reinterpret_cast<R *>(af.out[k])[tiled(a, af.out_tpad)] = R(0);
+    if (af.out[k]) reinterpret_cast<R *>(af.out[k])[atm_at(a, af.out_stride, af.out_tpad)] = R(0);
 }
 
 int launch_atmos_zero(const AtmosFused &af, const int32_t *cells, int64_t n, bool f32, void *stream) {
diff --git a/components.flux_calculator_amd/python/fcx/_lib.py b/components.flux_calculator_amd/python/fcx/_lib.py
--- a/components.flux_calculator_amd/python/fcx/_lib.py
+++ b/components.flux_calculator_amd/python/fcx/_lib.py
@@ -86,6 +86,7 @@
     ("fcx_device_free", _I, [_P]),
     ("fcx_memcpy", _I, [_P, _P, _c.c_size_t, _I]),
     ("fcx_last_group_size", _I, [_P, _c.POINTER(_I32)]),
+    ("fcx_atm_records", _I, [_P, _c.POINTER(_I32)]),
     ("fcx_step_async", _I, [_P, _I, _I32]),
     ("fcx_upload_field", _I, [_P, _I, _I, _I]),
     ("fcx_comm_verify", _I, [_P, _I]),
diff --git a/components.flux_calculator_amd/python/fcx/engine.py b/components.flux_calculator_amd/python/fcx/engine.py
--- a/components.flux_calculator_amd/python/fcx/engine.py
+++ b/components.flux_calculator_amd/python/fcx/engine.py
@@ -173,7 +173,7 @@
     OPTIONS = {"cells_per_thread": 1, "max_blocks": 2, "nontemporal": 3, "specialize": 4,
                "atmos_in_run": 5, "pipeline_chunks": 7, "pipeline_min_chunk": 8, "zero_copy": 9,
                "timing": 10, "tiled_layout": 11, "remap_pack": 13, "host_staging": 15, "host_threads": 16,
-               "atmos_halo": 17, "deferred_scatter": 18, "lib_spans": 19}
+               "atmos_halo": 17, "deferred_scatter": 18, "lib_spans": 19, "atm_records": 21}
 
     def run_atmos(self, phase=PHASE_ALL):
         _lib.check(self.lib.fcx_run_atmos(self.h, phase))
@@ -209,6 +209,11 @@
         m = ctypes.c_int32()
         _lib.check(self.lib.fcx_last_group_size(self.h, ctypes.byref(m)))
         return m.value
+
+    def atm_records(self):
+        on = ctypes.c_int32()
+        _lib.check(self.lib.fcx_atm_records(self.h, ctypes.byref(on)))
+        return bool(on.value)
 
     def close(self):
         if self.h is not None:
diff --git a/include/fcx.h b/include/fcx.h
--- a/include/fcx.h
+++ b/include/fcx.h
@@ -83,6 +83,7 @@
 int fcx_download(fcx_engine *e, int phase);
 int fcx_run_group(fcx_engine *const *engines, int n_engines, int phase, int32_t current_step_time);
 int fcx_last_group_size(fcx_engine *e, int32_t *members);
+int fcx_atm_records(const fcx_engine *e, int32_t *on);
 int fcx_step(fcx_engine *e, int phase, int32_t current_step_time);
 int fcx_synchronize(fcx_engine *e);
 int fcx_step_async(fcx_engine *e, int phase, int32_t current_step_time);
@@ -154,6 +155,7 @@
   FCX_OPT_RETIRED_CARRY_HANDOFF = 14,
   FCX_OPT_ATMOS_HALO = 17,
   FCX_OPT_REMAP_PACK = 13,
+  FCX_OPT_ATM_RECORDS = 21,
   FCX_OPT_TILED_LAYOUT = 11
 };
 int fcx_set_option(fcx_engine *e, int option, int64_t value);
```
